# SeungheonOh/voxtral.c

Measured on AMD Instinct MI355X. Metric: decoder tokens/sec + encoder RTF, Voxtral-4B bf16 at 1/2/4/8 MI355X, higher is better.
Workload: dtype f32

## Files before the change

include/voxtral_hip.h:

```cpp
#ifndef VOXTRAL_HIP_H
#define VOXTRAL_HIP_H

#include <stddef.h>
#include <stdint.h>

#ifdef __cplusplus
extern "C" {
#endif

int vox_hip_init(void);
int vox_hip_available(void);
void vox_hip_shutdown(void);
size_t vox_hip_memory_used(void);
const char *vox_hip_last_error(void);
void vox_hip_clear_error(void);
int vox_hip_set_device(int device);

typedef struct {
    int enc_dim, enc_layers, enc_heads, enc_kv_heads, enc_head_dim, enc_hidden, enc_window;
    int dec_dim, dec_layers, dec_heads, dec_kv_heads, dec_head_dim, dec_hidden, dec_window;
    int vocab, mel_bins, downsample, ada_dim;
    float rope_theta, enc_eps, dec_eps;
    int gelu_erf;
} vox_hip_config_t;

void vox_hip_config_voxtral_4b(vox_hip_config_t *cfg);

typedef struct {
    const float *conv0_w, *conv0_b, *conv1_w, *conv1_b;
    const uint16_t **enc_wq, **enc_wk, **enc_wv, **enc_wo, **enc_w1, **enc_w2, **enc_w3;
    const float **enc_wq_b, **enc_wv_b, **enc_wo_b, **enc_w2_b, **enc_attn_norm, **enc_ffn_norm;
    const float *enc_norm;
    const uint16_t *ad0, *ad1;
    const uint16_t *tok_emb;
    const uint16_t **dec_wq, **dec_wk, **dec_wv, **dec_wo, **dec_w1, **dec_w2, **dec_w3;
    const float **dec_attn_norm, **dec_ffn_norm, **dec_ada_down, **dec_ada_up;
    const float *dec_norm;
    const float **enc_wq_s, **enc_wk_s, **enc_wv_s, **enc_wo_s, **enc_w1_s, **enc_w2_s, **enc_w3_s;
    const float *ad0_s, *ad1_s, *tok_emb_s;
    const float **dec_wq_s, **dec_wk_s, **dec_wv_s, **dec_wo_s, **dec_w1_s, **dec_w2_s, **dec_w3_s;
} vox_hip_weights_t;

typedef struct vox_hip_model vox_hip_model_t;
typedef struct vox_hip_stream vox_hip_stream_t;

vox_hip_model_t *vox_hip_model_create(const vox_hip_config_t *cfg, const vox_hip_weights_t *w,
                                      int delay_tokens);
void vox_hip_model_free(vox_hip_model_t *m);
int vox_hip_model_set_delay(vox_hip_model_t *m, int delay_tokens);
int vox_hip_model_ada_scale(vox_hip_model_t *m, float *out);
int vox_hip_model_set_kv_fp16(vox_hip_model_t *m, int on);
int vox_hip_model_set_kv_dtype(vox_hip_model_t *m, int dtype);
int vox_hip_model_set_enc_kv_fp16(vox_hip_model_t *m, int on);
int vox_hip_model_set_kv_grow(vox_hip_model_t *m, int slots0);
typedef struct {
    int packed_tensors;
    int raw_tensors;
    long long packed_bytes;
    long long packed_raw_bytes;
    long long raw_bytes;
    double pack_ms;
} vox_hip_wpack_stats_t;
int vox_hip_model_wpack_stats(const vox_hip_model_t *m, vox_hip_wpack_stats_t *out);
int vox_hip_gemv_wpack(int rows, int K, const uint16_t *W, const float *x, float *y, int packed);
int vox_hip_set_wmx4(int mode);
int vox_hip_wmx4(void);
typedef struct {
    int wmx4_tensors;
    int refused_tensors;
    long long plane_bytes;
    long long bf16_bytes;
    double bits_per_weight;
    double scan_ms;
    double round_ms;
    double pack_ms;
} vox_hip_wmx4_stats_t;
int vox_hip_model_wmx4_stats(const vox_hip_model_t *m, vox_hip_wmx4_stats_t *out);
int vox_hip_set_wmx4_batch(int on);
int vox_hip_wmx4_batch(void);
int vox_hip_model_wmx4_batch_stats(const vox_hip_model_t *m, long long out4[4]);
int vox_hip_skinny_wmx4(int N, int K, const uint16_t *W, const float *x, int nb, float *y, int fmt, int head);
int vox_hip_set_gemm_planes(int planes);
int vox_hip_gemm_planes(void);
int vox_hip_set_gemmf_wait(int ticks);
int vox_hip_set_gemmf_q8(int on);
int vox_hip_gemmf_q8(void);
int vox_hip_model_gemmf_q8_stats(const vox_hip_model_t *m, long long out4[4]);
int vox_hip_gemmf_q8_rows(int M, int N, int K, const float *x, const int8_t *Wq, const float *scales, float *y,
                          int fmt);

vox_hip_stream_t *vox_hip_stream_create(vox_hip_model_t *m);
void vox_hip_stream_free(vox_hip_stream_t *s);
int vox_hip_stream_kv_fp16(const vox_hip_stream_t *s);
int vox_hip_stream_kv_dtype(const vox_hip_stream_t *s);
int vox_hip_stream_enc_kv_fp16(const vox_hip_stream_t *s);
int vox_hip_stream_enc_paths(const vox_hip_stream_t *s, long long out5[5]);
long long vox_hip_stream_enc_kv_bytes(const vox_hip_stream_t *s);
int vox_hip_stream_kv_slots(const vox_hip_stream_t *s);
long long vox_hip_stream_kv_bytes(const vox_hip_stream_t *s);
int vox_hip_stream_kv_grow_stats(const vox_hip_stream_t *s, long long out3[3]);
int vox_hip_stream_reserve_kv(vox_hip_stream_t *s, int positions);
int vox_hip_stream_read_kv(vox_hip_stream_t *s, int layer, int first_logical_pos, int n, void *k_out, void *v_out);
int vox_hip_stream_read_enc_kv(vox_hip_stream_t *s, int layer, int first_logical_pos, int n, void *k_out, void *v_out);
int vox_hip_kv8_convert(const float *x, int n, uint8_t *codes, float *back);
int vox_hip_stream_reset(vox_hip_stream_t *s);
int vox_hip_stream_reset_decoder(vox_hip_stream_t *s);
#define VOX_HIP_MAX_DELAY_TOKENS 30
int vox_hip_stream_set_delay(vox_hip_stream_t *s, int delay_tokens);
int vox_hip_stream_delay(const vox_hip_stream_t *s);
int vox_hip_stream_ada_scale(vox_hip_stream_t *s, float *out);

int vox_hip_stream_encode_mel(vox_hip_stream_t *s, const float *mel, int n_frames,
                              int mel_on_device);
int vox_hip_stream_adapter_tokens(vox_hip_stream_t *s);
int vox_hip_set_adapter_rows0(int rows);
int vox_hip_stream_adapter_stats(const vox_hip_stream_t *s, long long out3[3]);
int vox_hip_stream_set_async_encode(vox_hip_stream_t *s, int on);
int vox_hip_stream_encode_mel_batch(vox_hip_stream_t *const *streams, const float *const *mels,
                                    const int *n_frames, int B, int mel_on_device, int *added);

typedef struct vox_hip_mel vox_hip_mel_t;
vox_hip_mel_t *vox_hip_mel_create(vox_hip_stream_t *s, int left_pad_samples);
int vox_hip_mel_feed(vox_hip_mel_t *m, const float *samples, int n_samples);
int vox_hip_mel_finish(vox_hip_mel_t *m, int right_pad_samples);
int vox_hip_mel_frames(const vox_hip_mel_t *m, int *frame_offset);
const float *vox_hip_mel_frame_ptr(const vox_hip_mel_t *m, int global_frame);
int vox_hip_mel_discard_before(vox_hip_mel_t *m, int keep_from_frame);
int vox_hip_mel_read(vox_hip_mel_t *m, int global_first, int n, float *out);
void vox_hip_mel_free(vox_hip_mel_t *m);
int vox_hip_mel_reset(vox_hip_mel_t *m, int left_pad_samples);
int vox_hip_stream_read_adapter(vox_hip_stream_t *s, int first, int n, float *out);

int vox_hip_stream_decode(vox_hip_stream_t *s, int max_steps, int stop_at_eos,
                          int *tokens_out, float *logits_out);
#define VOX_HIP_MAX_ALT 4
int vox_hip_stream_set_alt(vox_hip_stream_t *s, int n_alt, float cutoff);
int vox_hip_stream_read_alts(vox_hip_stream_t *s, int first, int n, int *ids_out, float *probs_out);
#define VOX_HIP_BATCH_MAX_SLOTS 128
typedef struct vox_hip_batch vox_hip_batch_t;
vox_hip_batch_t *vox_hip_batch_create(vox_hip_model_t *m, int max_streams);
void vox_hip_batch_free(vox_hip_batch_t *b);
int vox_hip_batch_decode(vox_hip_batch_t *b, vox_hip_stream_t **streams, int n, int max_steps,
                         int stop_at_eos, int *tokens_out, int *counts_out);
int vox_hip_batch_decode_rows(vox_hip_batch_t *b, vox_hip_stream_t **streams, int n, const int *rows,
                              int max_steps, int stop_at_eos, int *tokens_out, int *counts_out);
int vox_hip_batch_begin_rows(vox_hip_batch_t *b, vox_hip_stream_t **streams, int n, const int *rows,
                             int max_steps, int stop_at_eos, int *tokens_out, int *counts_out);
int vox_hip_batch_finish(vox_hip_batch_t *b);
int vox_hip_batch_read_logits(vox_hip_batch_t *b, vox_hip_stream_t *s, float *out);
int vox_hip_batch_stats(const vox_hip_batch_t *b, long long *out6);
int vox_hip_batch_kv_grow_stats(const vox_hip_batch_t *b, long long out3[3]);
int vox_hip_batch_set_prefill_kv(vox_hip_batch_t *b, int on);
int vox_hip_batch_set_gemv_rows(vox_hip_batch_t *b, int max_rows);
int vox_hip_batch_set_gemv_rows_q8(vox_hip_batch_t *b, int max_rows);
int vox_hip_batch_gemv_stats(const vox_hip_batch_t *b, long long *out4);
int vox_hip_batch_set_gemv_wmx4(vox_hip_batch_t *b, int on);
int vox_hip_batch_gemv_wmx4_stats(const vox_hip_batch_t *b, long long out4[4]);
int vox_hip_batch_set_wmx4(vox_hip_batch_t *b, int on);
int vox_hip_gemv_rows(int rows, int K, const uint16_t *W, const float *x, int R, float *y, int packed);
int vox_hip_gemv_rows_q8(int rows, int K, const int8_t *W, const float *scales, const float *x, int R, float *y);
int vox_hip_gemv_q8(int rows, int K, const int8_t *W, const float *scales, const float *x, float *y);
int vox_hip_stream_state(vox_hip_stream_t *s, int *out6);

void vox_hip_sgemm_bf16(int M, int N, int K, const float *A, const uint16_t *B_bf16, float *C);
void vox_hip_sgemm_q8(int M, int N, int K, const float *A, const int8_t *B_q8, const float *scales,
                      float *C);
void vox_hip_fused_qkv_bf16(int M, int K, const float *input,
                            const uint16_t *wq_bf16, int Nq, const uint16_t *wk_bf16, int Nk,
                            const uint16_t *wv_bf16, int Nv, float *q, float *k, float *v);
void vox_hip_fused_ffn_bf16(int M, int dim, int hidden, const float *input,
                            const uint16_t *w1_bf16, const uint16_t *w3_bf16,
                            const uint16_t *w2_bf16, float *output);
// ... 24 lines not shown
```

voxtral.c_amd/csrc/vox_hip.hip:

```cpp
#include "../../include/voxtral_hip.h"
#include "vox_hip_internal.h"
#include "vox_wmx4.h"
#include "vox_wpack.h"

#include <hip/hip_runtime.h>
#include <math.h>
#include <stdarg.h>
#include <stdio.h>
#include <stdlib.h>
#include <string.h>

#include <stddef.h>
#include <algorithm>
#include <atomic>
#include <chrono>
#include <mutex>
#include <string>
#include <thread>
#include <unordered_map>
#include <vector>

using namespace vox;

#define TOKEN_BOS 1
// ... 1561 lines not shown
            if (l == 0) s->enc_paths[4] += ns > 1;
            SklFused o = f;
            o.x = x;
            o.bias = L.bo;
            o.ssq_out = s->essq;
            o.planes = xa;
            o.nw = L.ffn_norm;
            CK(launch_gemm_sklx(SKX_PRO_PLANES, SKX_EPI_RESID, xq, EQ, F.wo, ED, n, o, st));
            SklFused u = f;
            u.ssq_in = s->essq;
            u.nsl = nsl_wo;
            u.planes = xq;
            CK(launch_gemm_sklx(SKX_PRO_SCALE, SKX_EPI_SWIGLU, xa, ED, F.w13, 2 * EH, n, u, st));
            SklFused d = f;
            d.x = x;
            d.bias = L.b2;
            d.ssq_out = s->essq;
            if (l + 1 < c.enc_layers) {
                d.planes = xa;
                d.nw = m->enc[l + 1].attn_norm;
            }
            CK(launch_gemm_sklx(SKX_PRO_PLANES, SKX_EPI_RESID, xq, EH, F.w2, ED, n, d, st));
        }
        CK(launch_rmsnorm_rows(x, ED, x, ED, m->enc_norm, nullptr, n, ED, c.enc_eps, st));
        return 0;
    }
    s->enc_paths[2]++;
    for (int l = 0; l < c.enc_layers; l++) {
        const EncLayerD& L = m->enc[l];
        const DecFragD& F = m->efrag[l];
        float* Kc = enc_ring(s, s->ek, l);
        float* Vc = enc_ring(s, s->ev, l);
        CK(launch_rmsnorm_fplanes(x, n, ED, L.attn_norm, nullptr, c.enc_eps, xp, l ? sl : nullptr,
                                  l ? skl_splits(EH, ED) : 0, st, l ? m->enc[l - 1].b2 : nullptr));
        CK(launch_gemm_skl(xp, ED, F.wqkv, L.sqkv, NQKV, n, sl, st));
        CK(launch_slabs_rope_kv(sl, skl_splits(ED, NQKV), n, L.bqkv, EQ, EKV, hd, rope, (int)pos0, s->q, Kc, Vc, s->ecap, st,
                                s->ekvt));
        CK(launch_attn_rows_mf(hd, s->q, EQ, Kc, Vc, s->ecap, s->att, EQ, n, H, KVH, (int)pos0, 0, c.enc_window, scale, st,
                             s->gws, s->gws_n, xp, s->ekvt));
        CK(launch_gemm_skl(xp, EQ, F.wo, L.so, ED, n, sl, st));
        CK(launch_rmsnorm_fplanes(x, n, ED, L.ffn_norm, nullptr, c.enc_eps, xp, sl, skl_splits(EQ, ED), st, L.bo));
        CK(launch_gemm_skl(xp, ED, F.w13, L.s13, 2 * EH, n, sl, st));
        CK(launch_swiglu_fplanes(sl, skl_splits(ED, 2 * EH), EH, n, xp, st));
        CK(launch_gemm_skl(xp, EH, F.w2, L.s2, ED, n, sl, st));
    }
    CK(launch_resid_slabs(x, n, ED, sl, skl_splits(EH, ED), m->enc[c.enc_layers - 1].b2, st));
    CK(launch_rmsnorm_rows(x, ED, x, ED, m->enc_norm, nullptr, n, ED, c.enc_eps, st));
    return 0;
}

static int enc_gemmf_env() {
    static const int v = env_on("VOX_HIP_GEMMF");
    return v;
}

template <class Layer>
static bool gemmf_fmt_ok(const vox_hip_model_t* m, const std::vector<Layer>& layers) {
    if (m->gemmf_q8) return true;
    for (const Layer& L : layers)
        if (L.sqkv || L.so || L.s13 || L.s2) return false;
    return true;
}

static bool enc_gemmf_ok(const vox_hip_model_t* m, int n) {
    const vox_hip_config_t& c = m->c;
    const int ED = c.enc_dim, EQ = c.enc_heads * c.enc_head_dim, EKV = c.enc_kv_heads * c.enc_head_dim;
    return enc_gemmf_env() && gemmf_fmt_ok(m, m->enc) && gemmf_ok(n, EQ + 2 * EKV, ED) && gemmf_ok(n, ED, EQ) &&
           gemmf_ok(n, 2 * c.enc_hidden, ED) && gemmf_ok(n, ED, c.enc_hidden) && c.enc_hidden % 64 == 0 &&
           ED <= 4 * 512;
}

struct GemmfQ {
    hipStream_t st;
    float* ws;
    size_t ws_n;
    int* flags;
    int* epoch;
    long long* n_q8;
    const int* epoch_dev;
    int* step_q8;
};

static int gemmf_on(const GemmfQ& q, int epi, const uint16_t* xs, int K, int n, const uint8_t* W, const float* wscale,
                    int N, const float* bias, float* C, int ldc, uint16_t* xo) {
    if (!q.epoch_dev) {
        hipStreamCaptureStatus cs = hipStreamCaptureStatusNone;
        CK(hipStreamIsCapturing(q.st, &cs));
        if (cs != hipStreamCaptureStatusNone) return set_err("k_gemmf launch while the stream is capturing");
    }
    if (++*q.epoch <= 0) *q.epoch = 1;
    if (!gemmf_ok(n, N, K) || !q.ws || !q.flags)
        return set_err("k_gemmf: unsupported shape M %d N %d K %d (ws %p flags %p)", n, N, K, (void*)q.ws, (void*)q.flags);
    if (!q.epoch_dev) {
        const hipError_t pend = hipGetLastError();
        if (pend != hipSuccess) return set_err("k_gemmf: HIP error pending before the launch: %s", hipGetErrorString(pend));
    }
    CK(launch_gemmf(epi, gemm_planes_np(), xs, K, n, W, N, bias, C, ldc, xo, q.ws, q.ws_n, q.flags, *q.epoch, q.st,
                    q.epoch_dev, q.epoch_dev ? gemmf_wide_rb(n, N, K) : 0, wscale));
    if (wscale) {
        ++*q.n_q8;
        if (q.step_q8) ++*q.step_q8;
    }
    return 0;
}

static GemmfQ stream_gemmfq(vox_hip_stream_t* s) {
    return GemmfQ{s->st, s->gws, s->gws_n, s->gflags, &s->gepoch, &s->m->n_gemmf_q8, nullptr, nullptr};
}

struct RowsLayer {
    const uint8_t *wqkv, *wo, *w13, *w2;
    const uint8_t *fqkv, *fo, *f13, *f2;
    const float *sqkv, *so, *s13, *s2;
    const float *bqkv, *bo, *b2;
    const float *attn_norm, *ffn_norm, *ada;
};
struct RowsStack {
    int D, Q, KV, hidden, layers;
    float eps;
    RowsLayer (*layer)(const vox_hip_model_t* m, int l);
};
struct RowsScratch {
    float *x, *qkv, *xn, *att, *hid;
    uint16_t *pa, *pc;
};
struct RowsAda {
    const float* table = nullptr;
    const BatchSlot* slots = nullptr;
};

static RowsLayer enc_rows_layer(const vox_hip_model_t* m, int l) {
    const EncLayerD& L = m->enc[l];
    const DecFragD F = m->efrag.empty() ? DecFragD{} : m->efrag[l];
    return RowsLayer{L.wqkv, L.wo, L.w13, L.w2, F.wqkv, F.wo, F.w13, F.w2, L.sqkv, L.so, L.s13, L.s2,
                     L.bqkv, L.bo, L.b2, L.attn_norm, L.ffn_norm, nullptr};
}
static RowsLayer dec_rows_layer(const vox_hip_model_t* m, int l) {
    const DecLayerD& L = m->dec[l];
    const DecFragD F = m->dfrag.empty() ? DecFragD{} : m->dfrag[l];
    return RowsLayer{L.wqkv, L.wo, L.w13, L.w2, F.wqkv, F.wo, F.w13, F.w2, L.sqkv, L.so, L.s13, L.s2,
                     nullptr, nullptr, nullptr, L.attn_norm, L.ffn_norm, m->ada_scale + (size_t)l * m->c.dec_dim};
}
static RowsStack enc_rows_stack(const vox_hip_config_t& c) {
    return RowsStack{c.enc_dim, c.enc_heads * c.enc_head_dim, c.enc_kv_heads * c.enc_head_dim, c.enc_hidden, c.enc_layers,
                     c.enc_eps, enc_rows_layer};
}
static RowsStack dec_rows_stack(const vox_hip_config_t& c) {
    return RowsStack{c.dec_dim, c.dec_heads * c.dec_head_dim, c.dec_kv_heads * c.dec_head_dim, c.dec_hidden, c.dec_layers,
                     c.dec_eps, dec_rows_layer};
}

template <class Attn>
static int rows_layers(const vox_hip_model_t* m, const RowsStack& S, const RowsScratch& B, const GemmfQ& q, bool gf, int n,
                       Attn attn, const RowsAda& ada = RowsAda{}) {
    const int D = S.D, NQKV = S.Q + 2 * S.KV, HID = S.hidden;
    hipStream_t st = q.st;
    for (int l = 0; l < S.layers; l++) {
        RowsLayer L = S.layer(m, l);
        if (ada.table) L.ada = ada.table + (size_t)l * D;
        if (gf) {
            CK(launch_rmsnorm_fplanes(B.x, n, D, L.attn_norm, nullptr, S.eps, B.pa, nullptr, 0, st));
            if (gemmf_on(q, EPI_STORE, B.pa, D, n, L.fqkv, L.sqkv, NQKV, L.bqkv, B.qkv, NQKV, nullptr)) return -1;
        } else {
            CK(launch_rmsnorm_rows(B.x, D, B.xn, D, L.attn_norm, nullptr, n, D, S.eps, st));
            CK(launch_gemm(EPI_STORE, 3, B.xn, D, L.wqkv, L.sqkv, D, n, NQKV, L.bqkv, B.qkv, NQKV, st, q.ws, q.ws_n));
        }
        if (attn(l, gf ? B.pa : nullptr)) return -1;
        if (gf) {
            if (gemmf_on(q, EPI_RESID, B.pa, S.Q, n, L.fo, L.so, D, L.bo, B.x, D, nullptr)) return -1;
            if (ada.slots) CK(launch_rmsnorm_fplanes_slots(B.x, n, D, L.ffn_norm, ada.slots, (size_t)l * D, S.eps, B.pa, st));
            else CK(launch_rmsnorm_fplanes(B.x, n, D, L.ffn_norm, L.ada, S.eps, B.pa, nullptr, 0, st));
            if (gemmf_on(q, EPI_SWIGLU, B.pa, D, n, L.f13, L.s13, 2 * HID, nullptr, nullptr, HID, B.pc)) return -1;
            if (gemmf_on(q, EPI_RESID, B.pc, HID, n, L.f2, L.s2, D, L.b2, B.x, D, nullptr)) return -1;
        } else {
            CK(launch_gemm(EPI_RESID, 3, B.att, S.Q, L.wo, L.so, S.Q, n, D, L.bo, B.x, D, st, q.ws, q.ws_n));
            if (ada.slots) CK(launch_rmsnorm_rows_slots(B.x, D, B.xn, D, L.ffn_norm, ada.slots, (size_t)l * D, n, D, S.eps, st));
            else CK(launch_rmsnorm_rows(B.x, D, B.xn, D, L.ffn_norm, L.ada, n, D, S.eps, st));
            CK(launch_gemm(EPI_SWIGLU, 3, B.xn, D, L.w13, L.s13, D, n, 2 * HID, nullptr, B.hid, HID, st, q.ws, q.ws_n));
            CK(launch_gemm(EPI_RESID, 3, B.hid, HID, L.w2, L.s2, HID, n, D, L.b2, B.x, D, st, q.ws, q.ws_n));
        }
    }
    return 0;
}

static int stream_enc_planes(vox_hip_stream_t* s) {
    const vox_hip_config_t& c = s->m->c;
    if (model_enc_frag(s->m)) return -1;
    if (!s->gpa) {
        const size_t rb = PLANE_MAX_ROWS / SK_ROWS;
        CK(dalloc(&s->gpa, rb * 3 * SK_ROWS * std::max(c.enc_dim, c.enc_heads * c.enc_head_dim)));
        CK(dalloc(&s->gpc, rb * 3 * SK_ROWS * c.enc_hidden));
    }
    if (!s->gflags) CK(dalloc(&s->gflags, gemmf_flag_ints()));
    return 0;
}
static RowsScratch enc_rows_scratch(vox_hip_stream_t* s, float* x) {
    return RowsScratch{x, s->qkv, s->xn, s->att, s->gate, s->gpa, s->gpc};
}

static bool enc_gemv_ok(const vox_hip_model_t* m) {
    const vox_hip_config_t& c = m->c;
    const int ED = c.enc_dim, EQ = c.enc_heads * c.enc_head_dim, EKV = c.enc_kv_heads * c.enc_head_dim;
    const bool q8 = m->enc[0].sqkv != nullptr;
    return gemv_ok(EQ + 2 * EKV, ED, q8) && gemv_ok(ED, EQ, q8) && gemv_ok(2 * c.enc_hidden, ED, q8) &&
           gemv_ok(ED, c.enc_hidden, q8) && c.enc_head_dim % 2 == 0 && c.enc_hidden % 16 == 0;
}

static int run_encoder_row_gemv(vox_hip_stream_t* s, float* x, long long pos0, const float* rope) {
    vox_hip_model_t* m = s->m;
    const vox_hip_config_t& c = m->c;
    const int ED = c.enc_dim, H = c.enc_heads, KVH = c.enc_kv_heads, hd = c.enc_head_dim;
    const int EQ = H * hd, EKV = KVH * hd, EH = c.enc_hidden;
    const float scale = 1.0f / sqrtf((float)hd);
    hipStream_t st = s->st;
    for (int l = 0; l < c.enc_layers; l++) {
        const EncLayerD& L = m->enc[l];
        float* Kc = enc_ring(s, s->ek, l);
        float* Vc = enc_ring(s, s->ev, l);
        GemvArgs a;
        memset(&a, 0, sizeof a);
        a.x = x; a.K = ED; a.W = L.wqkv; a.wscale = L.sqkv; a.rows = EQ + 2 * EKV; a.bias = L.bqkv;
        a.norm_w = L.attn_norm; a.eps = c.enc_eps; a.y = s->q;
        a.qd = EQ; a.kvd = EKV; a.hd = hd; a.pos = (int)pos0; a.rope = rope - (size_t)pos0 * hd;
        a.Kc = Kc; a.Vc = Vc; a.cap = s->ecap; a.kvt = s->ekvt;
        CK(launch_gemv(PRO_NORM, EPI_QKV_BIAS, a, st));
        CK(launch_attn_rows_mf(hd, s->q, EQ, Kc, Vc, s->ecap, s->att, EQ, 1, H, KVH, (int)pos0, 0, c.enc_window, scale,
                               st, s->gws, s->gws_n, nullptr, s->ekvt));
        memset(&a, 0, sizeof a);
        a.x = s->att; a.K = EQ; a.W = L.wo; a.wscale = L.so; a.rows = ED; a.bias = L.bo; a.y = x;
        CK(launch_gemv(PRO_NONE, EPI_RESID, a, st));
        memset(&a, 0, sizeof a);
        a.x = x; a.K = ED; a.W = L.w13; a.wscale = L.s13; a.rows = 2 * EH; a.norm_w = L.ffn_norm; a.eps = c.enc_eps;
        a.y = s->gate;
        CK(launch_gemv(PRO_NORM, EPI_SWIGLU, a, st));
        memset(&a, 0, sizeof a);
        a.x = s->gate; a.K = EH; a.W = L.w2; a.wscale = L.s2; a.rows = ED; a.bias = L.b2; a.y = x;
        CK(launch_gemv(PRO_NONE, EPI_RESID, a, st));
    }
    CK(launch_rmsnorm_rows(x, ED, x, ED, m->enc_norm, nullptr, 1, ED, c.enc_eps, st));
    return 0;
}

static int enc_skinny_env() {
    static const int v = env_on("VOX_HIP_ENC_SKINNY");
    return v;
}

static int run_encoder_rows(vox_hip_stream_t* s, float* x, int n, long long pos0, const float* rope) {
    vox_hip_model_t* m = s->m;
    const vox_hip_config_t& c = m->c;
    const int ED = c.enc_dim, H = c.enc_heads, KVH = c.enc_kv_heads, hd = c.enc_head_dim;
    const int EQ = H * hd, EKV = KVH * hd;
    const float scale = 1.0f / sqrtf((float)hd);
    hipStream_t st = s->st;
    if (n > ENC_SUB) return set_err("encoder pass of %d rows > %d", n, ENC_SUB);
    if (n == 1 && enc_gemv_ok(m)) {
        s->enc_paths[0]++;
        return run_encoder_row_gemv(s, x, pos0, rope);
    }
    if (n <= enc_skinny_rows() && enc_skinny_env() && enc_skinny_ok(c)) return run_encoder_rows_skinny(s, x, n, pos0, rope);
    s->enc_paths[3]++;
    const bool gf = enc_gemmf_ok(m, n);
    if (gf && stream_enc_planes(s)) return -1;
    if (rows_layers(m, enc_rows_stack(c), enc_rows_scratch(s, x), stream_gemmfq(s), gf, n, [&](int l, uint16_t* planes) -> int {
            float* Kc = enc_ring(s, s->ek, l);
            float* Vc = enc_ring(s, s->ev, l);
            CK(launch_rope_kv(s->qkv, n, EQ, EKV, hd, rope, (int)pos0, s->q, Kc, Vc, s->ecap, st, s->ekvt));
            CK(launch_attn_rows_mf(hd, s->q, EQ, Kc, Vc, s->ecap, s->att, EQ, n, H, KVH, (int)pos0, 0, c.enc_window, scale,
                                   st, s->gws, s->gws_n, planes, s->ekvt));
            return 0;
        }))
        return -1;
    CK(launch_rmsnorm_rows(x, ED, x, ED, m->enc_norm, nullptr, n, ED, c.enc_eps, st));
    return 0;
}

static int ensure_rope(vox_hip_stream_t* s, long long last_pos) {
    vox_hip_model_t* m = s->m;
    if (last_pos < m->rope_positions) return 0;
    int p = m->rope_positions;
    while (p <= last_pos) p *= 2;
    CK(hipDeviceSynchronize());
    if (model_rope_tables(m, p)) return -1;
    s->graph_ready = 0;
    return 0;
}

static int enc_prefix(vox_hip_stream_t* s, const float* mel, int n, int mel_on_device, int* T1o, float** xino) {
    vox_hip_model_t* m = s->m;
    const vox_hip_config_t& c = m->c;
    const int MB = c.mel_bins, ED = c.enc_dim;
    hipStream_t st = s->st;
    *T1o = 0;
    *xino = nullptr;
    if (n <= 0) return 0;
    if (stream_alloc_frames(s, n + 4)) return -1;
    CK(hipMemcpyAsync(s->mel_p, s->mel_tail, (size_t)2 * MB * 4, hipMemcpyDeviceToDevice, st));
    CK(hipMemcpyAsync(s->mel_p + (size_t)2 * MB, mel, (size_t)n * MB * 4,
                      mel_on_device ? hipMemcpyDeviceToDevice : hipMemcpyHostToDevice, st));
    CK(launch_mel_tail(s->mel_p, n, MB, s->mel_tail, st));
    CK(hipMemcpyAsync(s->c0_p, s->c0_tail, (size_t)2 * ED * 4, hipMemcpyDeviceToDevice, st));
    if (s->res_count)
        CK(hipMemcpyAsync(s->c0_p + (size_t)2 * ED, s->c0_res, (size_t)ED * 4, hipMemcpyDeviceToDevice, st));
    float* c0_new = s->c0_p + (size_t)(2 + s->res_count) * ED;
    CK(launch_im2col3(s->mel_p, MB, n, 1, 0, s->im2col, st));
    CK(launch_gemm(c.gelu_erf ? EPI_GELU_ERF : EPI_GELU, 3, s->im2col, MB * 3, m->conv0_w, nullptr, MB * 3, n, ED,
                   m->conv0_b, c0_new, ED, st, s->gws, s->gws_n));
    const int total = s->res_count + n;
    const int new_res = total & 1;
    const int feed = total - new_res;
    if (new_res)
        CK(hipMemcpyAsync(s->c0_res, s->c0_p + (size_t)(2 + total - 1) * ED, (size_t)ED * 4,
                          hipMemcpyDeviceToDevice, st));
    s->res_count = new_res;
    if (feed <= 0) return 0;
    const int T1 = feed / 2;
    float* xin = s->x_enc + (size_t)4 * ED;
    CK(launch_im2col3(s->c0_p, ED, T1, 2, 1, s->im2col, st));
    CK(launch_gemm(c.gelu_erf ? EPI_GELU_ERF : EPI_GELU, 3, s->im2col, ED * 3, m->conv1_w, nullptr, ED * 3, T1, ED,
                   m->conv1_b, xin, ED, st, s->gws, s->gws_n));
    CK(hipMemcpyAsync(s->c0_tail, s->c0_p + (size_t)(2 + feed - 2) * ED, (size_t)2 * ED * 4,
                      hipMemcpyDeviceToDevice, st));
    if (ensure_rope(s, s->enc_pos + T1 + 1)) return -1;
    *T1o = T1;
    *xino = xin;
    return 0;
}

static const int CS_ROWS = 2 * ENC_SUB + 5 * VOX_MAX_BATCH;
static bool enc_prefix_batch_fits(vox_hip_stream_t* const* ss, const int* n, int B) {
    long long r0 = 0, r1 = 0;
    for (int b = 0; b < B; b++)
        if (n[b] > 0) {
            r0 += 2 + ss[b]->res_count + n[b];
            r1 += (ss[b]->res_count + n[b]) / 2;
        }
    return r0 <= CS_ROWS && r1 <= ENC_SUB;
}

static int enc_prefix_batch(vox_hip_stream_t* lead, vox_hip_stream_t* const* ss, const float* const* mels,
                            const int* n, int B, int mel_on_device, float* X, int* T1, int* off) {
    vox_hip_model_t* m = lead->m;
    const vox_hip_config_t& c = m->c;
    const int MB = c.mel_bins, ED = c.enc_dim;
    hipStream_t st = lead->st;
    if (!lead->cs_im) {
        CK(dalloc(&lead->cs_im, std::max((size_t)CS_ROWS * MB * 3, (size_t)ENC_SUB * ED * 3)));
        CK(dalloc(&lead->cs_c0, (size_t)CS_ROWS * ED));
    }
    std::vector<int> seg(B, 0), res(B, 0), tot(B, 0);
    int R0 = 0, N = 0;
    for (int b = 0; b < B; b++) {
        T1[b] = 0;
        off[b] = N;
// ... 81 lines not shown
    s->enc_res_count = left;
    return added;
}

static int enc_suffix_batch(vox_hip_stream_t* lead, const float* X, vox_hip_stream_t* const* ss, const int* T1,
                            const int* off, int B, int* added) {
    vox_hip_model_t* m = lead->m;
    const vox_hip_config_t& c = m->c;
    const int ED = c.enc_dim, D = c.dec_dim;
    hipStream_t st = lead->st;
    const size_t ain_rows = (size_t)ENC_SUB + 4 * VOX_MAX_BATCH;
    if (!lead->abatch) {
        CK(dalloc(&lead->abatch, ain_rows * ED));
        CK(dalloc(&lead->abatch_out, ain_rows / 4 * D));
    }
    std::vector<int> aoff(B, 0), n4v(B, 0);
    int NA = 0;
    for (int b = 0; b < B; b++)
        if (T1[b] > 0) {
            const int tot = ss[b]->enc_res_count + T1[b];
            if (ss[b]->total_adapter + tot / 4 > ss[b]->adapter_cap) return set_err("enc_suffix_batch: adapter buffer");
            NA += tot / 4;
        }
    if ((size_t)NA * 4 > ain_rows) return set_err("enc_suffix_batch: %d adapter rows", NA);
    NA = 0;
    for (int b = 0; b < B; b++) {
        added[b] = 0;
        if (T1[b] <= 0) continue;
        vox_hip_stream_t* s = ss[b];
        s->enc_pos += T1[b];
        const int R = s->enc_res_count, tot = R + T1[b], usable = (tot / 4) * 4, left = tot - usable;
        const float* xb = X + (size_t)off[b] * ED;
        if (usable > 0) {
            float* dst = lead->abatch + (size_t)NA * 4 * ED;
            if (R) CK(hipMemcpyAsync(dst, s->enc_res, (size_t)R * ED * 4, hipMemcpyDeviceToDevice, st));
            CK(hipMemcpyAsync(dst + (size_t)R * ED, xb, (size_t)(usable - R) * ED * 4, hipMemcpyDeviceToDevice, st));
            if (left)
                CK(hipMemcpyAsync(s->enc_res, xb + (size_t)(usable - R) * ED, (size_t)left * ED * 4,
                                  hipMemcpyDeviceToDevice, st));
            aoff[b] = NA;
            n4v[b] = usable / 4;
            NA += usable / 4;
        } else {
            CK(hipMemcpyAsync(s->enc_res + (size_t)R * ED, xb, (size_t)T1[b] * ED * 4, hipMemcpyDeviceToDevice, st));
        }
        s->enc_res_count = left;
    }
    for (int r0 = 0; r0 < NA; r0 += ENC_SUB / 4) {
        const int nr = std::min(ENC_SUB / 4, NA - r0);
        CK(launch_gemm(c.gelu_erf ? EPI_GELU_ERF : EPI_GELU, 3, lead->abatch + (size_t)r0 * 4 * ED, 4 * ED, m->ad0,
                       m->ad0_s, 4 * ED, nr, D, nullptr, lead->ad_mid, D, st, lead->gws, lead->gws_n));
        CK(launch_gemm(EPI_STORE, 3, lead->ad_mid, D, m->ad1, m->ad1_s, D, nr, D, nullptr,
                       lead->abatch_out + (size_t)r0 * D, D, st, lead->gws, lead->gws_n));
    }
    for (int b = 0; b < B; b++) {
        if (!n4v[b]) continue;
        vox_hip_stream_t* s = ss[b];
        CK(hipMemcpyAsync(s->adapter + (size_t)s->total_adapter * D, lead->abatch_out + (size_t)aoff[b] * D,
                          (size_t)n4v[b] * D * 4, hipMemcpyDeviceToDevice, st));
        s->total_adapter += n4v[b];
        added[b] = n4v[b];
    }
    return 0;
}

static int run_encoder_rows_batch(vox_hip_stream_t* lead, float* X, int N, vox_hip_stream_t* const* ss,
                                  const int* off, const int* nr, const long long* pos0, int B) {
    vox_hip_model_t* m = lead->m;
    const vox_hip_config_t& c = m->c;
    const int ED = c.enc_dim, H = c.enc_heads, KVH = c.enc_kv_heads, hd = c.enc_head_dim;
    const int EQ = H * hd, EKV = KVH * hd;
    const float scale = 1.0f / sqrtf((float)hd);
    hipStream_t st = lead->st;
    const bool gf = enc_gemmf_ok(m, N);
    if (gf && stream_enc_planes(lead)) return -1;
    EncRows er;
    memset(&er, 0, sizeof er);
    er.B = B;
    for (int b = 0; b < B; b++) {
        er.off[b] = off[b];
        er.nr[b] = nr[b];
        er.pos0[b] = (int)pos0[b];
    }
    if (rows_layers(m, enc_rows_stack(c), enc_rows_scratch(lead, X), stream_gemmfq(lead), gf, N, [&](int l, uint16_t* planes) -> int {
            for (int b = 0; b < B; b++) {
                er.Kc[b] = enc_ring(ss[b], ss[b]->ek, l);
                er.Vc[b] = enc_ring(ss[b], ss[b]->ev, l);
            }
            CK(launch_rope_kv_rows(lead->qkv, N, EQ, EKV, hd, m->rope_enc, er, lead->q, lead->ecap, st, lead->ekvt));
            CK(launch_attn_rows(hd, lead->q, er, N, lead->ecap, lead->att, H, KVH, c.enc_window, scale, lead->gws,
                                lead->gws_n, st, planes, lead->ekvt));
            return 0;
        }))
        return -1;
    CK(launch_rmsnorm_rows(X, ED, X, ED, m->enc_norm, nullptr, N, ED, c.enc_eps, st));
    return 0;
}

static int encode_mel_batch_pass(vox_hip_stream_t* const* ss, const float* const* mels, const int* n, int B,
                                 int mel_on_device, int* added, bool sync = true) {
    vox_hip_stream_t* lead = ss[0];
    const vox_hip_config_t& c = lead->m->c;
    const int ED = c.enc_dim;
    std::vector<int> T1(B), off(B);
    std::vector<float*> xin(B);
    std::vector<long long> pos0(B);
    int N = 0;
    bool all_async = true;
    int active = 0;
    for (int b = 0; b < B; b++) {
        all_async = all_async && ss[b]->enc_async;
        if (n[b] > 0) {
            const int tot = ss[b]->res_count + n[b];
            active += tot - (tot & 1) > 0;
        }
    }
    static const int stem_batch = env_on("VOX_HIP_ENC_STEM_BATCH");
    const bool stacked = stem_batch && active > 1 && enc_prefix_batch_fits(ss, n, B);
    if (stacked) {
        if (!lead->xbatch) CK(dalloc(&lead->xbatch, (size_t)ENC_SUB * ED));
        N = enc_prefix_batch(lead, ss, mels, n, B, mel_on_device, lead->xbatch, T1.data(), off.data());
        if (N < 0) return -1;
        for (int b = 0; b < B; b++) pos0[b] = ss[b]->enc_pos;
    } else {
        for (int b = 0; b < B; b++) {
            if (enc_prefix(ss[b], mels[b], n[b], mel_on_device, &T1[b], &xin[b])) return -1;
            off[b] = N;
            pos0[b] = ss[b]->enc_pos;
            N += T1[b];
        }
    }
    if (!stacked && (N > ENC_SUB || active <= 1)) {
        for (int b = 0; b < B; b++) {
            added[b] = 0;
            if (T1[b] <= 0) continue;
            for (int r0 = 0; r0 < T1[b]; r0 += ENC_SUB) {
                const int nrr = std::min(ENC_SUB, T1[b] - r0);
                const long long p0 = ss[b]->enc_pos + r0;
                if (run_encoder_rows(ss[b], xin[b] + (size_t)r0 * ED, nrr, p0, lead->m->rope_enc + (size_t)p0 * c.enc_head_dim))
                    return -1;
            }
            added[b] = enc_suffix(ss[b], xin[b], T1[b]);
            if (added[b] < 0) return -1;
        }
    } else {
        if (!stacked) {
            if (!lead->xbatch) CK(dalloc(&lead->xbatch, (size_t)ENC_SUB * ED));
            for (int b = 1; b < B; b++) {
                CK(hipEventRecord(ss[b]->sev, ss[b]->st));
                CK(hipStreamWaitEvent(lead->st, ss[b]->sev, 0));
            }
            for (int b = 0; b < B; b++)
                if (T1[b] > 0)
                    CK(hipMemcpyAsync(lead->xbatch + (size_t)off[b] * ED, xin[b], (size_t)T1[b] * ED * 4,
                                      hipMemcpyDeviceToDevice, lead->st));
        }
        for (int b = 0; b < B; b++)
            if (T1[b] > 0 && stream_alloc_adapter(ss[b], ss[b]->total_adapter + (ss[b]->enc_res_count + T1[b]) / 4))
                return -1;
        if (run_encoder_rows_batch(lead, lead->xbatch, N, ss, off.data(), T1.data(), pos0.data(), B)) return -1;
        if (enc_suffix_batch(lead, lead->xbatch, ss, T1.data(), off.data(), B, added)) return -1;
        CK(hipEventRecord(lead->sev, lead->st));
        for (int b = 1; b < B; b++) CK(hipStreamWaitEvent(ss[b]->st, lead->sev, 0));
    }
    if (sync && !all_async)
        for (int b = 0; b < B; b++) CK(hipStreamSynchronize(ss[b]->st));
    return 0;
// ... 44 lines not shown
        for (int r0 = 0; r0 < T1; r0 += ENC_SUB) {
            int nr = std::min(ENC_SUB, T1 - r0);
            long long p0 = s->enc_pos + r0;
            if (run_encoder_rows(s, xin + (size_t)r0 * c.enc_dim, nr, p0,
                                 s->m->rope_enc + (size_t)p0 * c.enc_head_dim))
                return -1;
        }
        added = enc_suffix(s, xin, T1);
        if (added < 0) return -1;
    }
    if (!s->enc_async) CK(hipStreamSynchronize(s->st));
    return added;
}

extern "C" int vox_hip_stream_set_async_encode(vox_hip_stream_t* s, int on) {
    if (!s) return set_err("null stream");
    if (s->enc_async && !on) CK(hipStreamSynchronize(s->st));
    s->enc_async = on ? 1 : 0;
    return 0;
}

extern "C" int vox_hip_stream_adapter_tokens(vox_hip_stream_t* s) { return s->total_adapter; }

extern "C" int vox_hip_stream_adapter_stats(const vox_hip_stream_t* s, long long out3[3]) {
    if (!s || !out3) return set_err("stream_adapter_stats: null argument");
    out3[0] = s->adapter_cap;
    out3[1] = s->ad_grows;
    out3[2] = s->ad_grows_held;
    return 0;
}

extern "C" int vox_hip_stream_read_adapter(vox_hip_stream_t* s, int first, int n, float* out) {
    const int D = s->m->c.dec_dim;
    if (first < 0 || first + n > s->total_adapter) return set_err("adapter rows out of range");
    CK(hipMemcpyAsync(out, s->adapter + (size_t)first * D, (size_t)n * D * 4, hipMemcpyDeviceToHost, s->st));
    CK(hipStreamSynchronize(s->st));
    return 0;
}

static int stream_prefilled(vox_hip_stream_t* s, hipStream_t q) {
    const int np = 32 + stream_delay(s);
    const int st4[4] = {np, np, TOKEN_STREAMING_PAD, s->n_generated};
    CK(hipMemcpyAsync(s->state, st4, sizeof st4, hipMemcpyHostToDevice, q));
    s->h_state[0] = np;
    s->h_state[1] = np;
    s->h_state[2] = TOKEN_STREAMING_PAD;
    s->h_state[3] = s->n_generated;
    s->started = 1;
    return 0;
}

static int dec_gemmf_env() {
    static const int v = env_on("VOX_HIP_PREFILL_GEMMF");
    return v;
}

static bool dec_gemmf_ok(const vox_hip_model_t* m, int n) {
    const vox_hip_config_t& c = m->c;
    const int DD = c.dec_dim, DQ = c.dec_heads * c.dec_head_dim, DKV = c.dec_kv_heads * c.dec_head_dim;
    return enc_gemmf_env() && dec_gemmf_env() && gemmf_fmt_ok(m, m->dec) && n >= 1 && n <= PLANE_MAX_ROWS && gemmf_ok(n, DQ + 2 * DKV, DD) &&
           gemmf_ok(n, DD, DQ) && gemmf_ok(n, 2 * c.dec_hidden, DD) && gemmf_ok(n, DD, c.dec_hidden) &&
           c.dec_hidden % 64 == 0;
}

static int stream_dec_planes(vox_hip_stream_t* s, int rows) {
    if (rows <= s->dp_rows) return 0;
    const vox_hip_config_t& c = s->m->c;
    const int DD = c.dec_dim, DQ = c.dec_heads * c.dec_head_dim;
    const int r = (rows + 127) / 128 * 128;
    dfree(s->dpa);
    dfree(s->dpc);
    s->dp_rows = 0;
    CK(dalloc(&s->dpa, (size_t)r * 3 * std::max(DD, DQ)));
    CK(dalloc(&s->dpc, (size_t)r * 3 * c.dec_hidden));
    if (!s->gflags) CK(dalloc(&s->gflags, gemmf_flag_ints()));
    s->dp_rows = r;
    return 0;
}

static RowsScratch dec_rows_scratch(vox_hip_stream_t* s, float* x) {
    return RowsScratch{x, s->qkvd, s->xnd, s->attd, s->gated, s->dpa, s->dpc};
}

static int run_decoder_rows(vox_hip_stream_t* s, float* x, int n, int pos0, const float* rope) {
    vox_hip_model_t* m = s->m;
    const vox_hip_config_t& c = m->c;
    const int H = c.dec_heads, KVH = c.dec_kv_heads, hd = c.dec_head_dim;
    const int DQ = H * hd, DKV = KVH * hd;
    const float scale = 1.0f / sqrtf((float)hd);
    hipStream_t st = s->st;
    if (stream_alloc_dec_rows(s, n)) return -1;
    if (n > DEC_SLACK + 1 && pos0 > 0) return set_err("prefill of %d rows on a non-empty cache", n);
    bool gf = n > 1 && dec_gemmf_ok(m, n);
    if (gf && (model_frag(m) || stream_dec_planes(s, n))) {
        vox_hip_clear_error();
        (void)hipGetLastError();
        gf = false;
    }
    return rows_layers(m, dec_rows_stack(c), dec_rows_scratch(s, x), stream_gemmfq(s), gf, n, [&](int l, uint16_t* planes) -> int {
        float* Kc = dec_ring(s, s->dk, l);
        float* Vc = dec_ring(s, s->dv, l);
        CK(launch_rope_kv(s->qkvd, n, DQ, DKV, hd, rope, pos0, s->qd_, Kc, Vc, s->dcap, st, s->kvt));
        CK(launch_attn_rows_mf(hd, s->qd_, DQ, Kc, Vc, s->dcap, s->attd, DQ, n, H, KVH, pos0, 0, c.dec_window, scale, st,
                               s->gws, s->gws_n, planes, s->kvt));
        return 0;
    }, RowsAda{s->delay < 0 ? nullptr : stream_ada(s), nullptr});
}

enum { T_QKV, T_WO, T_W13, T_W2 };
struct StepTensor {
    const uint8_t* W;
    const float* wscale;
    int rows, K, pro, epi;
    const float *norm_w, *ada;
    const WPackD* pack;
    const WMx4D* mx;
};
static StepTensor dec_step_tensor(const vox_hip_model_t* m, int l, int which) {
    const vox_hip_config_t& c = m->c;
    const int DD = c.dec_dim, DQ = c.dec_heads * c.dec_head_dim, DKV = c.dec_kv_heads * c.dec_head_dim, DH = c.dec_hidden;
    if (l == (int)m->dec.size())
        return StepTensor{m->tok_emb, m->tok_emb_s, c.vocab, DD, PRO_NORM, EPI_STORE, m->dec_norm, nullptr, &m->plm, &m->mlm};
    const DecLayerD& L = m->dec[l];
    switch (which) {
    case T_QKV: return StepTensor{L.wqkv, L.sqkv, DQ + 2 * DKV, DD, PRO_NORM, EPI_QKV, L.attn_norm, nullptr, &L.pqkv, &L.mqkv};
    case T_WO: return StepTensor{L.wo, L.so, DD, DQ, PRO_NONE, EPI_RESID, nullptr, nullptr, &L.po, &L.mo};
    case T_W13:
        return StepTensor{L.w13, L.s13, 2 * DH, DD, PRO_NORM_ADA, EPI_SWIGLU, L.ffn_norm, m->ada_scale + (size_t)l * DD,
                          &L.p13, &L.m13};
    default: return StepTensor{L.w2, L.s2, DD, DH, PRO_NONE, EPI_RESID, nullptr, nullptr, &L.p2, &L.m2};
    }
}
template <class F>
static bool all_step_tensors(const vox_hip_model_t* m, F f) {
    const int nl = (int)m->dec.size();
    for (int l = 0; l <= nl; l++)
        for (int w = 0; w < (l < nl ? 4 : 1); w++)
            if (!f(dec_step_tensor(m, l, w))) return false;
    return true;
}
static void step_tensor_args(GemvArgs& a, const StepTensor& t, const float* x, float* y, float eps, int wmx4) {
    memset(&a, 0, sizeof a);
    a.x = x; a.K = t.K; a.W = t.W; a.wscale = t.wscale; a.rows = t.rows; a.y = y;
    a.norm_w = t.norm_w; a.ada = t.ada; a.eps = t.norm_w ? eps : 0.f;
    wpack_args(a, *t.pack);
    if (wmx4) wmx4_args(a, *t.mx);
}

static int enqueue_lm_head(vox_hip_stream_t* s, const int* state);

static int enqueue_step_layers(vox_hip_stream_t* s, const int* state, int pos, const float* rope_row,
                               int splits) {
    vox_hip_model_t* m = s->m;
    const vox_hip_config_t& c = m->c;
    const int H = c.dec_heads, KVH = c.dec_kv_heads, hd = c.dec_head_dim;
    const float scale = 1.0f / sqrtf((float)hd);
    hipStream_t st = s->st;
    for (int l = 0; l < c.dec_layers; l++) {
        float* Kc = dec_ring(s, s->dk, l);
        float* Vc = dec_ring(s, s->dv, l);
        GemvArgs a;
        StepTensor t = dec_step_tensor(m, l, T_QKV);
        step_tensor_args(a, t, s->xd, s->qd_, c.dec_eps, 1);
        a.qd = H * hd; a.kvd = KVH * hd; a.hd = hd;
        a.state = state; a.pos = pos;
        a.rope = state ? m->rope_dec : rope_row - (size_t)pos * hd;
        a.Kc = Kc; a.Vc = Vc; a.cap = s->dcap; a.kvt = s->kvt;
        CK(launch_gemv(t.pro, t.epi, a, st));
        CK(launch_attn_decode(hd, s->qd_, Kc, Vc, s->dcap, state, pos, c.dec_window, scale, H, KVH,
                              s->part, s->attd, splits, st, s->kvt));
        t = dec_step_tensor(m, l, T_WO);
        step_tensor_args(a, t, s->attd, s->xd, c.dec_eps, 1);
        CK(launch_gemv(t.pro, t.epi, a, st));
        t = dec_step_tensor(m, l, T_W13);
        if (s->delay >= 0) t.ada = stream_ada(s) + (size_t)l * c.dec_dim;
        step_tensor_args(a, t, s->xd, s->gated, c.dec_eps, 1);
        const bool gprof = s->profiling && state && !s->capturing && (int)s->pev.size() == 2 * c.dec_layers;
        if (gprof) CK(launch_gemv_timed(t.pro, t.epi, a, s->pev[2 * l], s->pev[2 * l + 1], st));
        else CK(launch_gemv(t.pro, t.epi, a, st));
        t = dec_step_tensor(m, l, T_W2);
        step_tensor_args(a, t, s->gated, s->xd, c.dec_eps, 1);
        CK(launch_gemv(t.pro, t.epi, a, st));
    }
    return enqueue_lm_head(s, state);
}

static int enqueue_lm_head(vox_hip_stream_t* s, const int* state) {
    vox_hip_model_t* m = s->m;
    const StepTensor t = dec_step_tensor(m, m->c.dec_layers, 0);
// ... 35 lines not shown
    s->capturing = 1;
    int rc = enqueue_graph_step(s, graph_splits(s, gi));
    s->capturing = 0;
    hipError_t e = hipStreamEndCapture(s->st, &g);
    if (rc || e != hipSuccess) {
        if (g) hipGraphDestroy(g);
        return set_err("graph capture failed: %s", hipGetErrorString(e));
    }
    e = hipGraphInstantiate(&s->step_exec[gi], g, nullptr, nullptr, 0);
    hipGraphDestroy(g);
    if (e != hipSuccess) return set_err("graph instantiate failed: %s", hipGetErrorString(e));
    s->graph_ready |= 1 << gi;
    s->graph_alt = s->n_alt > 1;
    s->graph_rope_gen = s->m->rope_gen;
    return 0;
}

static int collect_graph_profile(vox_hip_stream_t* s) {
    if (!s->profiling || !s->graph_prof) return 0;
    const vox_hip_config_t& c = s->m->c;
    for (int l = 0; l < c.dec_layers; l++) {
        float ms = 0.f;
        CK(hipEventElapsedTime(&ms, s->pev[2 * l], s->pev[2 * l + 1]));
        s->prof_ms += ms;
        s->prof_bytes += (double)2 * c.dec_hidden * c.dec_dim * 2;
        s->prof_launches++;
    }
    return 0;
}

static int use_graphs() {
    static const int v = env_on("VOX_HIP_GRAPH");
    return v;
}

static int run_steps(vox_hip_stream_t* s, int n, int pos0) {
    const vox_hip_config_t& c = s->m->c;
    const int gi = graph_index(s, std::min(pos0 + n, c.dec_window));
    const int splits = graph_splits(s, gi);
    if (s->profiling && use_graphs() && n > 1) {
        s->profiling = 0;
        const int rc = run_steps(s, n - 1, pos0);
        s->profiling = 1;
        if (rc) return -1;
        pos0 += n - 1;
        n = 1;
    }
    if (!use_graphs() || s->profiling) {
        if (s->profiling && s->pev.empty()) {
            s->pev.resize(2 * c.dec_layers);
            for (auto& e : s->pev) CK(hipEventCreate(&e));
        }
        s->graph_prof = s->profiling;
        for (int i = 0; i < n; i++)
            if (enqueue_graph_step(s, splits)) return -1;
        return 0;
    }
    if (s->graph_ready && (s->graph_alt != (s->n_alt > 1) || s->graph_rope_gen != s->m->rope_gen)) s->graph_ready = 0;
    if (!(s->graph_ready & (1 << gi)) && build_step_graph(s, gi)) return -1;
    for (int i = 0; i < n; i++) CK(hipGraphLaunch(s->step_exec[gi], s->st));
    return 0;
}

template <class T>
static int ring_read(const T* ring, int cap, int rec, long long first, int n, T* out, hipStream_t st) {
    while (n > 0) {
        const int slot = (int)(first % cap);
        const int k = std::min(n, cap - slot);
        CK(hipMemcpyAsync(out, ring + (size_t)slot * rec, (size_t)k * rec * sizeof(T), hipMemcpyDeviceToHost, st));
        out += (size_t)k * rec;
        first += k;
        n -= k;
    }
    return 0;
}

static int stream_prefill(vox_hip_stream_t* s) {
    vox_hip_model_t* m = s->m;
    const int np = 32 + stream_delay(s);
    if (stream_alloc_dec_rows(s, np)) return -1;
    if (ensure_rope(s, np + 2)) return -1;
    CK(launch_embed_rows(s->adapter, m->tok_emb, m->tok_emb_s, 0, np, TOKEN_BOS, TOKEN_STREAMING_PAD, m->c.dec_dim,
                         s->xd, s->st));
    if (run_decoder_rows(s, s->xd, np, 0, m->rope_dec)) return -1;
    return stream_prefilled(s, s->st);
}

extern "C" int vox_hip_stream_decode(vox_hip_stream_t* s, int max_steps, int stop_at_eos,
                                     int* tokens_out, float* logits_out) {
    vox_hip_model_t* m = s->m;
    const vox_hip_config_t& c = m->c;
    const int D = c.dec_dim, V = c.vocab, hd = c.dec_head_dim;
    const int prompt_len = 1 + 32 + stream_delay(s);
    int produced = 0;
    if (s->held) return set_err("stream_decode: %s", HELD_MSG);
    if (max_steps <= 0 || s->eos_seen) return 0;
    if (!s->started && s->total_adapter < prompt_len) return 0;
    if (s->dslots0) {
        const int pos = s->started ? s->h_state[0] : prompt_len - 1;
        const int left = s->total_adapter - (s->started ? s->h_state[1] : prompt_len - 1);
        if (stream_grow_dec(s, pos + std::max(0, std::min(max_steps, left)))) return -1;
    }
    if (!s->started && stream_prefill(s)) return -1;
    const int step_base = s->n_generated;
    int avail = s->total_adapter - (s->h_state[1] > 0 ? s->h_state[1] : prompt_len - 1);
    {
        int st4[4];
        CK(hipMemcpyAsync(st4, s->state, sizeof st4, hipMemcpyDeviceToHost, s->st));
        CK(hipStreamSynchronize(s->st));
        memcpy(s->h_state, st4, sizeof st4);
        avail = s->total_adapter - st4[1];
    }
    if (ensure_rope(s, (long long)s->h_state[0] + avail + 1)) return -1;
    if (avail > 0) CK(launch_embed_step(s->adapter, m->tok_emb, m->tok_emb_s, s->state, D, s->xd, s->st));
    int todo = std::min(max_steps, avail);
    std::vector<int> tok;
    while (produced < todo) {
        int b = std::min(STEP_BATCH, todo - produced);
        if (logits_out) b = 1;
        if (run_steps(s, b, s->h_state[0] + produced)) return -1;
        tok.resize(produced + b);
        if (ring_read(s->tokens, s->tokens_cap, 1, (long long)step_base + produced, b, tok.data() + produced, s->st))
            return -1;
        if (logits_out)
            CK(hipMemcpyAsync(logits_out + (size_t)produced * V, s->logits, (size_t)V * 4, hipMemcpyDeviceToHost, s->st));
        CK(hipStreamSynchronize(s->st));
        if (collect_graph_profile(s)) return -1;
        int eos_at = -1;
        if (stop_at_eos)
            for (int i = produced; i < produced + b; i++)
                if (tok[i] == TOKEN_EOS) { eos_at = i; break; }
        if (eos_at >= 0) {
            produced = eos_at + 1;
            s->eos_seen = 1;
            break;
        }
        produced += b;
    }
    if (tokens_out) memcpy(tokens_out, tok.data(), (size_t)produced * 4);
    s->n_generated += produced;
    s->h_state[0] += produced;
    s->h_state[1] += produced;
    if (produced) s->h_state[2] = tok[produced - 1];
    s->h_state[3] = s->n_generated;
    (void)hd;
    return produced;
}

extern "C" int vox_hip_stream_set_alt(vox_hip_stream_t* s, int n_alt, float cutoff) {
    if (!s) return -1;
    if (s->held) return set_err("stream_set_alt: %s", HELD_MSG);
    if (n_alt < 1) n_alt = 1;
    if (n_alt > VOX_HIP_MAX_ALT) n_alt = VOX_HIP_MAX_ALT;
    if (cutoff < 0) cutoff = 0;
    if (cutoff > 1) cutoff = 1;
    s->n_alt = n_alt;
    s->alt_cutoff = cutoff;
    return 0;
}

extern "C" int vox_hip_stream_read_alts(vox_hip_stream_t* s, int first, int n, int* ids_out,
                                        float* probs_out) {
    if (!s || first < 0 || n < 0 || first + n > s->n_generated || first < s->n_generated - s->tokens_cap)
        return set_err("alt range out of bounds (the last %d steps are kept)", s->tokens_cap);
    if (n == 0) return 0;
    std::vector<float> rec((size_t)n * ALT_REC);
    std::vector<int> tok(n);
// ... 408 lines not shown
            CK(dalloc(&dW, (size_t)N * K * 2));
            if (upload(dW, W, (size_t)N * K * 2) || frag_copy(&dF, dW, N, K, 0)) return -1;
        }
        CK(dalloc(&dx, (size_t)nb * K));
        CK(dalloc(&dxs, (size_t)Z * 3 * SK_ROWS * K));
        CK(dalloc(&dout, nout));
        if (upload(dx, x, (size_t)nb * K * 4)) return -1;
        CK(launch_split_fplanes(dx, nb, K, dxs, g_twin_st));
        if (!head)
            CK(launch_gemm_skl(dxs, K, dF, nullptr, N, nb, dout, g_twin_st, nullptr, 0, 0.f, 1, fmt));
        else if (nb > SK_ROWS)
            CK(launch_gemm_skf2(dxs, K, dF, nullptr, N, nb, dout, N, g_twin_st, fmt));
        else
            CK(launch_gemm_skf(dxs, K, dF, nullptr, N, nb, dout, N, g_twin_st, fmt));
        CK(hipStreamSynchronize(g_twin_st));
        CK(hipMemcpy(out.data(), dout, nout * 4, hipMemcpyDeviceToHost));
        return 0;
    };
    const int rc = run();
    dfree(dW); dfree(dF); dfree(dx); dfree(dxs); dfree(dout);
    if (rc) return -1;
    for (int j = 0; j < nb; j++) {
        float* yr = y + (size_t)j * N;
        if (head) {
            memcpy(yr, out.data() + (size_t)j * N, (size_t)N * 4);
            continue;
        }
        const float* p = out.data() + (size_t)(j >> 4) * S * SK_ROWS * N + (size_t)(j & 15) * N;
        for (int n = 0; n < N; n++) {
            float v = p[n];
            for (int sp = 1; sp < S; sp++) v += p[(size_t)sp * SK_ROWS * N + n];
            yr[n] = v;
        }
    }
    return 0;
}

extern "C" int vox_hip_gemmf_q8_rows(int M, int N, int K, const float* x, const int8_t* Wq, const float* scales, float* y,
                                     int fmt) {
    std::lock_guard<std::mutex> lk(g_twin_mu);
    if (!x || !Wq || !y || (fmt && !scales)) return set_err("gemmf_q8_rows: null argument");
    if (fmt != 0 && fmt != 1) return set_err("gemmf_q8_rows: fmt is 0 or 1");
    if (!gemmf_ok(M, N, K) || M > PLANE_MAX_ROWS)
        return set_err("gemmf_q8_rows: k_gemmf does not take M %d N %d K %d (M 1..1024, N %% 128, K %% 64)", M, N, K);
    if (twin_init()) return -1;
    uint8_t *dW = nullptr, *dF = nullptr;
    float *dx = nullptr, *dy = nullptr, *ds = nullptr, *dws = nullptr;
    uint16_t* dxs = nullptr;
    int* dflags = nullptr;
    auto run = [&]() -> int {
        const size_t n = (size_t)N * K;
        if (fmt) {
            CK(dalloc(&dW, n));
            CK(dalloc(&ds, (size_t)N));
            if (upload(dW, Wq, n) || upload(ds, scales, (size_t)N * 4) || frag_copy(&dF, dW, N, K, 1)) return -1;
        } else {
            std::vector<uint16_t> wb(n);
            for (size_t i = 0; i < n; i++) {
                const float f = (float)Wq[i];
                uint32_t u;
                memcpy(&u, &f, 4);
                wb[i] = (uint16_t)(u >> 16);
            }
            CK(dalloc(&dW, n * 2));
            if (upload(dW, wb.data(), n * 2) || frag_copy(&dF, dW, N, K, 0)) return -1;
        }
        const size_t rows = (size_t)(M + 127) / 128 * 128;
        const size_t ws_n = gemmf_ws_floats(gemmf_grid());
        CK(dalloc(&dx, (size_t)M * K));
        CK(dalloc(&dxs, rows * 3 * K));
        CK(dalloc(&dy, (size_t)M * N));
        CK(dalloc(&dws, ws_n));
        CK(dalloc(&dflags, gemmf_flag_ints()));
        if (upload(dx, x, (size_t)M * K * 4)) return -1;
        CK(launch_split_fplanes(dx, M, K, dxs, g_twin_st));
        CK(launch_gemmf(EPI_STORE, gemm_planes_np(), dxs, K, M, dF, N, nullptr, dy, N, nullptr, dws, ws_n, dflags, 1,
                        g_twin_st, nullptr, 0, fmt ? ds : nullptr));
        CK(hipStreamSynchronize(g_twin_st));
        CK(hipMemcpy(y, dy, (size_t)M * N * 4, hipMemcpyDeviceToHost));
        return 0;
    };
    const int rc = run();
    dfree(dW); dfree(dF); dfree(dx); dfree(dxs); dfree(dy); dfree(ds); dfree(dws); dfree(dflags);
    return rc ? -1 : 0;
}

extern "C" void vox_hip_sgemm_bf16(int M, int N, int K, const float* A, const uint16_t* B, float* C) {
    std::lock_guard<std::mutex> lk(g_twin_mu);
    twin_sgemm(M, N, K, A, B, nullptr, C);
}

extern "C" void vox_hip_sgemm_q8(int M, int N, int K, const float* A, const int8_t* B, const float* scales,
                                 float* C) {
    std::lock_guard<std::mutex> lk(g_twin_mu);
    if (!scales) { set_err("sgemm_q8: null scales"); return; }
    twin_sgemm(M, N, K, A, B, scales, C);
}

extern "C" void vox_hip_fused_qkv_bf16(int M, int K, const float* input, const uint16_t* wq, int Nq,
                                       const uint16_t* wk, int Nk, const uint16_t* wv, int Nv,
                                       float* q, float* k, float* v) {
    std::lock_guard<std::mutex> lk(g_twin_mu);
    if (M <= 0) return;
    if (twin_init()) return;
    const TwinW* W[3] = {twin_weight(wq, nullptr, Nq, K), twin_weight(wk, nullptr, Nk, K),
                         twin_weight(wv, nullptr, Nv, K)};
    if (!W[0] || !W[1] || !W[2]) return;
    float* outs[3] = {q, k, v};
    float* dO[3] = {nullptr, nullptr, nullptr};
    size_t* caps[3] = {&g_tQ_n, &g_tK_n, &g_tV_n};
    float** bufs[3] = {&g_tQ, &g_tK, &g_tV};
    if (twin_put_rows(&g_tA, &g_tA_n, input, M, K, W[0]->Kp)) return;
    for (int i = 0; i < 3; i++) {
        if (twin_buf(bufs[i], caps[i], (size_t)M * W[i]->Np) || twin_gemm_dev(M, g_tA, *W[i], *bufs[i])) return;
        dO[i] = *bufs[i];
    }
    for (int i = 0; i < 3; i++)
        if (twin_get_rows(outs[i], dO[i], M, W[i]->N, W[i]->Np)) return;
    if (hipStreamSynchronize(g_twin_st) != hipSuccess) set_err("fused_qkv: sync failed");
}

__global__ void k_silu_mul(float* g, const float* u, size_t n) {
    size_t i = (size_t)blockIdx.x * 256 + threadIdx.x;
    if (i < n) {
        float v = g[i];
        g[i] = v / (1.0f + expf(-v)) * u[i];
    }
}

extern "C" void vox_hip_fused_ffn_bf16(int M, int dim, int hidden, const float* input,
                                       const uint16_t* w1, const uint16_t* w3, const uint16_t* w2,
                                       float* output) {
    std::lock_guard<std::mutex> lk(g_twin_mu);
    if (M <= 0) return;
    if (twin_init()) return;
    const TwinW* d1 = twin_weight(w1, nullptr, hidden, dim);
    const TwinW* d3 = twin_weight(w3, nullptr, hidden, dim);
    const TwinW* d2 = twin_weight(w2, nullptr, dim, hidden);
    if (!d1 || !d3 || !d2) return;
    const int Hp = d1->Np;
    if (d2->Kp != Hp) { set_err("fused_ffn: padded hidden %d != %d", d2->Kp, Hp); return; }
    if (twin_put_rows(&g_tA, &g_tA_n, input, M, dim, d1->Kp) || twin_buf(&g_tQ, &g_tQ_n, (size_t)M * Hp) ||
        twin_buf(&g_tK, &g_tK_n, (size_t)M * Hp) || twin_buf(&g_tC, &g_tC_n, (size_t)M * d2->Np) ||
        twin_gemm_dev(M, g_tA, *d1, g_tQ) || twin_gemm_dev(M, g_tA, *d3, g_tK))
        return;
    const size_t n = (size_t)M * Hp;
    hipLaunchKernelGGL(k_silu_mul, dim3((unsigned)((n + 255) / 256)), dim3(256), 0, g_twin_st, g_tQ, g_tK, n);
    if (hipGetLastError() != hipSuccess) { set_err("fused_ffn: silu_mul launch failed"); return; }
    if (twin_gemm_dev(M, g_tQ, *d2, g_tC) || twin_get_rows(output, g_tC, M, dim, d2->Np)) return;
    if (hipStreamSynchronize(g_twin_st) != hipSuccess) set_err("fused_ffn: sync failed");
}

static int twin_attention(float* out, const float* Q, const float* K, const float* V, int seq_q, int seq_k,
                          int n_heads, int n_kv_heads, int head_dim, float scale, int window_size, int q_offset) {
    if (twin_init()) return -1;
    if (seq_q <= 0) return 0;
    if (!out || !Q || !K || !V) return set_err("encoder_attention: null pointer");
    if (q_offset < 0 || q_offset + seq_q > seq_k) return set_err("encoder_attention: queries beyond keys");
    if (n_kv_heads <= 0 || n_heads % n_kv_heads) return set_err("encoder_attention: heads %d / kv heads %d", n_heads, n_kv_heads);
    const size_t qn = (size_t)seq_q * n_heads * head_dim, kn = (size_t)seq_k * n_kv_heads * head_dim;
    if (twin_buf(&g_tQ, &g_tQ_n, qn) || twin_buf(&g_tK, &g_tK_n, kn) || twin_buf(&g_tV, &g_tV_n, kn) ||
        twin_buf(&g_tO, &g_tO_n, qn))
        return -1;
    CK(hipMemcpyAsync(g_tQ, Q, qn * 4, hipMemcpyHostToDevice, g_twin_st));
    CK(hipMemcpyAsync(g_tK, K, kn * 4, hipMemcpyHostToDevice, g_twin_st));
    CK(hipMemcpyAsync(g_tV, V, kn * 4, hipMemcpyHostToDevice, g_twin_st));
// ... 539 lines not shown
    if (!b) return set_err("batch_set_gemv_rows_q8: null batch");
    return batch_set_gemv_rows_q8(b, max_rows);
}

static int batch_set_gemv_wmx4(vox_hip_batch_t* b, int on, bool quiet) {
    if (b->call.active) return quiet ? -1 : set_err("batch_set_gemv_wmx4: a begun call was not finished");
    if (on) {
        const vox_hip_model_t* m = b->m;
        long long with = 0, without = 0;
        model_gemv_wmx4_count(m, &with, &without);
        if (!with)
            return quiet ? -1
                         : set_err("batch_set_gemv_wmx4: the model has no wmx4 GEMV plane (vox_hip_set_wmx4 before its creation; "
                                   "not Q8, not VOX_HIP_WPACK=0)");
        if (!model_gemvr_ok(m, 1))
            return quiet ? -1 : set_err("batch_set_gemv_wmx4: no wmx4 k_gemvr instance for this model's shapes");
    }
    b->gemv_wmx4 = on ? 1 : 0;
    return 0;
}

extern "C" int vox_hip_batch_set_gemv_wmx4(vox_hip_batch_t* b, int on) {
    if (!b) return set_err("batch_set_gemv_wmx4: null batch");
    return batch_set_gemv_wmx4(b, on, false);
}

extern "C" int vox_hip_batch_gemv_wmx4_stats(const vox_hip_batch_t* b, long long out4[4]) {
    if (!b || !out4) return set_err("batch_gemv_wmx4_stats: null argument");
    out4[0] = b->gemv_wmx4;
    out4[1] = b->n_gemv_wmx4_replays;
    model_gemv_wmx4_count(b->m, &out4[2], &out4[3]);
    return 0;
}

extern "C" int vox_hip_batch_set_wmx4(vox_hip_batch_t* b, int on) {
    if (!b) return set_err("batch_set_wmx4: null batch");
    if (b->call.active) return set_err("batch_set_wmx4: a begun call was not finished");
    if (on && !b->m->fstats[0])
        return set_err("batch_set_wmx4: the model has no wmx4 fragment planes (vox_hip_set_wmx4_batch before its creation)");
    b->wmx4 = on ? 1 : 0;
    return 0;
}

extern "C" int vox_hip_batch_set_prefill_kv(vox_hip_batch_t* b, int on) {
    if (!b) return set_err("batch_set_prefill_kv: null batch");
    if (b->call.active) return set_err("batch_set_prefill_kv: a begun call was not finished");
    b->prefill_kv = on ? 1 : 0;
    return 0;
}

extern "C" int vox_hip_batch_gemv_stats(const vox_hip_batch_t* b, long long* out4) {
    if (!b || !out4) return set_err("batch_gemv_stats: null argument");
    out4[0] = b->gemv_rows;
    out4[1] = b->n_gemv_replays;
    out4[2] = b->n_gemv_rows;
    out4[3] = b->n_gemv_captures;
    return 0;
}

static int batch_step_wide(vox_hip_batch_t* b, int nb, int splits, int kvt, int mixed, int ragged) {
    vox_hip_model_t* m = b->m;
    const vox_hip_config_t& c = m->c;
    const int DD = c.dec_dim, H = c.dec_heads, KVH = c.dec_kv_heads, hd = c.dec_head_dim;
    const int DQ = H * hd, DKV = KVH * hd, QKV = DQ + 2 * DKV;
    const float scale = 1.0f / sqrtf((float)hd);
    const int cap = c.dec_window + DEC_SLACK;
    const size_t ring_layer = (size_t)cap * DKV * kv_esize(kvt);
    hipStream_t st = b->st;
    const bool gf = dec_gemmf_ok(m, nb);
    const bool lm_gf = (!m->tok_emb_s || m->gemmf_q8) && enc_gemmf_env() && dec_gemmf_env() && gemmf_ok(nb, c.vocab, DD);
    int launches = 0;
    b->wide_q8 = 0;
    const GemmfQ q{st, b->pgws, GEMM_WS_ELEMS, b->wflags, &launches, &m->n_gemmf_q8, b->wepoch, &b->wide_q8};
    AttnSlotsRag ap;
    ap.q = nullptr; ap.q_ld = 0;
    ap.part = b->apart; ap.part_ld = b->apart_n;
    ap.out = gf ? nullptr : b->att; ap.out_ld = DQ;
    ap.slots = b->slots;
    ap.ring_off = 0;
    ap.caps = b->dcaps; ap.layer = 0;
    AttnFuse af;
    af.qkv = b->wqkv; af.S = 1; af.N = QKV; af.rope = m->rope_dec; af.xs = b->wpa;
    if (rows_layers(m, dec_rows_stack(c), RowsScratch{b->x, b->wqkv, b->wxn, b->att, b->whid, b->wpa, b->wpc}, q, gf, nb,
                    [&](int l, uint16_t*) -> int {
                        ap.ring_off = (size_t)l * ring_layer;
                        ap.layer = l;
                        if (ragged) CK(launch_attn_batch_wide_rag(hd, ap, af, nb, c.dec_window, scale, H, KVH, splits, st, kvt));
                        else CK(launch_attn_batch_wide(hd, ap, af, nb, cap, c.dec_window, scale, H, KVH, splits, st, kvt));
                        return 0;
                    }, RowsAda{nullptr, mixed ? b->slots : nullptr}))
        return -1;
    if (lm_gf) {
        CK(launch_rmsnorm_fplanes(b->x, nb, DD, m->dec_norm, nullptr, c.dec_eps, b->wpa, nullptr, 0, st));
        if (gemmf_on(q, EPI_STORE, b->wpa, DD, nb, m->lm_frag, m->tok_emb_s, c.vocab, nullptr, b->logits, c.vocab, nullptr)) return -1;
    } else {
        CK(launch_rmsnorm_rows(b->x, DD, b->wxn, DD, m->dec_norm, nullptr, nb, DD, c.dec_eps, st));
        CK(launch_gemm(EPI_STORE, 3, b->wxn, DD, m->tok_emb, m->tok_emb_s, DD, nb, c.vocab, nullptr, b->logits, c.vocab, st,
                       b->pgws, GEMM_WS_ELEMS));
    }
    CK(launch_argmax_batch(b->logits, nb, c.vocab, b->pval, b->pidx, b->palt, b->slots, TOKENS_CAP, slot_toklog(b->slots, b->rows),
                           m->tok_emb, m->tok_emb_s, DD, b->x, st));
    if (launches) CK(launch_gemmf_epoch_bump(b->wepoch, launches + 1, st));
    return 0;
}


static int slot_bucket(int n, int* g) {
    int k = 0;
    while ((1 << k) < n) k++;
    *g = k;
    return 1 << k;
}

static int batch_run(vox_hip_batch_t* b, int nb, int gb, int gi, int splits, int kvt, int steps, int gemv, int mixed,
                     int ragged) {
    const int wmx4 = b->wmx4;
    const int gwmx4 = b->gemv_wmx4;
    const bool wide = nb > VOX_MAX_BATCH;
    auto step = [&]() {
        return wide ? batch_step_wide(b, nb, splits, kvt, mixed, ragged)
               : gemv ? batch_step_gemv(b, nb, splits, kvt, gwmx4) : batch_step(b, nb, splits, kvt, wmx4, mixed, ragged);
    };
    if (ragged) b->n_ragged_replays += steps;
    if (gemv) b->n_gemv_replays += steps;
    if (gemv && gwmx4) b->n_gemv_wmx4_replays += steps;
    if (!use_graphs()) {
        for (int k = 0; k < steps; k++)
            if (step()) return -1;
        b->n_replays += steps;
        return 0;
    }
    if (b->grope_gen != b->m->rope_gen) {
        batch_drop_graphs(b);
        b->grope_gen = b->m->rope_gen;
    }
    const int mr = mixed + 2 * ragged;
    hipGraphExec_t& ge = wide ? b->gwexec[mr][kvt][gb - 6][gi]
                         : gemv ? b->gvexec[3 * gwmx4 + kvt][gb][gi] : b->gexec[mr][3 * wmx4 + kvt][gb][gi];
    if (!ge) {
        hipGraph_t g = nullptr;
        CK(hipStreamBeginCapture(b->st, hipStreamCaptureModeThreadLocal));
        const int rc = step();
        hipError_t e = hipStreamEndCapture(b->st, &g);
        if (rc || e != hipSuccess) {
            if (g) hipGraphDestroy(g);
            return set_err("batch graph capture failed: %s", hipGetErrorString(e));
        }
        e = hipGraphInstantiate(&ge, g, nullptr, nullptr, 0);
        hipGraphDestroy(g);
        if (e != hipSuccess) {
            ge = nullptr;
            return set_err("batch graph instantiate failed: %s", hipGetErrorString(e));
        }
        b->n_captures++;
        if (ragged) b->n_ragged_captures++;
        if (gemv) b->n_gemv_captures++;
    }
    for (int k = 0; k < steps; k++) CK(hipGraphLaunch(ge, b->st));
    if (wide) b->m->n_gemmf_q8 += (long long)steps * b->wide_q8;
    b->n_replays += steps;
    return 0;
}

static void stream_steps_done(vox_hip_stream_t* s, int produced, int last_token) {
    s->n_generated += produced;
    s->h_state[0] += produced;
    s->h_state[1] += produced;
    if (produced) s->h_state[2] = last_token;
    s->h_state[3] = s->n_generated;
}

static int batch_prefill(vox_hip_batch_t* b, vox_hip_stream_t* const* ss, int B, bool bounded) {
    vox_hip_model_t* m = b->m;
    const vox_hip_config_t& c = m->c;
    const int np = 32 + stream_delay(ss[0]);
    const int per = std::max(1, ENC_SUB / np);
    const int kvt = ss[0]->kvt;
    const bool one_by_one = kvt != KV_F32 && !b->prefill_kv;
    if (B > per && !one_by_one) {
        for (int i0 = 0; i0 < B; i0 += per)
            if (batch_prefill(b, ss + i0, std::min(per, B - i0), bounded)) return -1;
        return 0;
    }
    if ((B == 1 && !bounded) || one_by_one || B * np > ENC_SUB) {
        for (int i = 0; i < B; i++) {
            if (stream_prefill(ss[i])) return -1;
            CK(hipStreamSynchronize(ss[i]->st));
        }
        b->n_prefill_passes += B;
        b->n_prefilled += B;
        return 0;
    }
    const int DD = c.dec_dim, H = c.dec_heads, KVH = c.dec_kv_heads, hd = c.dec_head_dim;
    const int DQ = H * hd, DKV = KVH * hd;
    const float scale = 1.0f / sqrtf((float)hd);
    vox_hip_stream_t* lead = ss[0];
    const int N = B * np, cap = lead->dcap;
    hipStream_t st = b->st;
    if (stream_alloc_dec_rows(lead, N)) return -1;
    if (ensure_rope(lead, np + 2)) return -1;
    if (!b->pgws) CK(dalloc(&b->pgws, GEMM_WS_ELEMS));
    float* gws = b->pgws;
    const size_t gws_n = GEMM_WS_ELEMS;
    float* X = lead->xd;
    for (int i = 0; i < B; i++)
        CK(launch_embed_rows(ss[i]->adapter, m->tok_emb, m->tok_emb_s, 0, np, TOKEN_BOS, TOKEN_STREAMING_PAD, DD,
                             X + (size_t)i * np * DD, st));
    EncRows er;
    memset(&er, 0, sizeof er);
    er.B = B;
    for (int i = 0; i < B; i++) {
        er.off[i] = i * np;
        er.nr[i] = np;
        er.pos0[i] = 0;
    }
    const bool gf = dec_gemmf_ok(m, N);
    if (gf) {
        if (!b->gflags) CK(dalloc(&b->gflags, gemmf_flag_ints()));
        if (model_frag(m) || stream_dec_planes(lead, N)) return -1;
    }
    if (rows_layers(m, dec_rows_stack(c), dec_rows_scratch(lead, X),
                    GemmfQ{st, gws, gws_n, b->gflags, &b->gepoch, &m->n_gemmf_q8, nullptr, nullptr}, gf, N,
                    [&](int l, uint16_t* planes) -> int {
                        for (int i = 0; i < B; i++) {
                            er.Kc[i] = dec_ring(ss[i], ss[i]->dk, l);
                            er.Vc[i] = dec_ring(ss[i], ss[i]->dv, l);
                        }
                        CK(launch_rope_kv_rows(lead->qkvd, N, DQ, DKV, hd, m->rope_dec, er, lead->qd_, cap, st, kvt));
                        CK(launch_attn_rows(hd, lead->qd_, er, N, cap, lead->attd, H, KVH, c.dec_window, scale, gws, gws_n, st,
                                            planes, kvt));
                        return 0;
                    }, RowsAda{lead->delay < 0 ? nullptr : stream_ada(lead), nullptr}))
        return -1;
    for (int i = 0; i < B; i++)
        if (stream_prefilled(ss[i], st)) return -1;
    b->n_prefill_passes++;
    b->n_prefilled += B;
    return 0;
}

static int batch_begin(vox_hip_batch_t* b, vox_hip_stream_t** streams, int n, const int* rows, int max_steps,
                       int stop_at_eos, int* tokens_out, int* counts_out) {
    if (!b || n < 1 || n > b->cap || n > VOX_MAX_SLOTS || max_steps < 0) return set_err("bad batch arguments");
    if (b->call.active) return set_err("batch: a begun call was not finished");
    vox_hip_model_t* m = b->m;
    const vox_hip_config_t& c = m->c;
    int mixed = 0;
    for (int i = 0; i < n; i++) {
        if (!streams[i] || streams[i]->m != m) return set_err("batch streams must share the batch's model");
        if (streams[i]->held) return set_err("batch streams[%d]: %s", i, HELD_MSG);
        mixed |= streams[i]->delay >= 0;
        if (streams[i]->kvt != streams[0]->kvt)
            return set_err("batch streams must share the decoder KV element type (vox_hip_model_set_kv_dtype)");
        for (int j = 0; j < i; j++)
            if (streams[j] == streams[i]) return set_err("stream listed twice in a batch");
        counts_out[i] = 0;
    }
    const int kvt = streams[0]->kvt;
    b->n_calls++;
    b->lnb = 0;
    int avail[VOX_MAX_SLOTS];
    for (int i = 0; i < n; i++) {
        if (rows) {
            if (rows[i] < 0 || rows[i] > streams[i]->total_adapter) return set_err("batch rows[%d] out of range", i);
            avail[i] = rows[i];
        } else {
            CK(hipStreamSynchronize(streams[i]->st));
            avail[i] = streams[i]->total_adapter;
        }
    }
    if (max_steps == 0) return 1;
    int ragged = 0;
    {
        bool grows = false;
        for (int i = 0; i < n; i++) grows = grows || streams[i]->dslots0;
        if (grows) {
            std::vector<DecGrow> gr(n);
            for (int i = 0; i < n; i++) {
                vox_hip_stream_t* s = streams[i];
                const int np = 32 + stream_delay(s);
                const bool joins = !s->started && !s->eos_seen && avail[i] >= 1 + np;
                int need = 0;
                if (s->started && !s->eos_seen) need = s->h_state[0] + std::max(0, std::min(avail[i] - s->h_state[1], max_steps));
                else if (joins) need = np + std::max(0, std::min(avail[i] - np, max_steps));
                if (dec_grow_alloc(s, need, true, &gr[i])) {
                    dec_grow_drop(gr.data(), i);
                    return -1;
                }
            }
            for (int i = 0; i < n; i++) ragged |= (gr[i].cap ? gr[i].cap : streams[i]->dcap) != dec_ring_full(streams[i]);
            if (ragged && !b->hcaps) {
                hipError_t e = b->dcaps ? hipSuccess : dalloc(&b->dcaps, (size_t)b->rows);
                if (e == hipSuccess) e = hipHostMalloc((void**)&b->hcaps, sizeof(int) * b->rows, hipHostMallocDefault);
                if (e != hipSuccess) {
                    b->hcaps = nullptr;
                    dec_grow_drop(gr.data(), n);
                    return set_err("batch: per-slot ring capacity table: %s", hipGetErrorString(e));
                }
            }
            if (dec_grow_commit(gr.data(), n, b->st)) return -1;
        }
        b->n_ragged_calls += ragged;
    }
    {
        vox_hip_stream_t* pre[VOX_MAX_SLOTS];
        int np = 0, longest_delay = 0;
// ... 223 lines not shown
```

voxtral.c_amd/csrc/vox_hip_dev.h:

```cpp
#pragma once
#include <hip/hip_runtime.h>
#include <stdint.h>

#include "vox_hip_internal.h"

namespace vox {

typedef __attribute__((ext_vector_type(8))) __bf16 bf16x8;
typedef __attribute__((ext_vector_type(4))) float f32x4;
typedef __attribute__((ext_vector_type(2))) float f32x2;
typedef __attribute__((ext_vector_type(4))) unsigned int u32x4;
typedef __attribute__((ext_vector_type(2))) unsigned int u32x2;

__device__ __forceinline__ uint4 ldnt(const uint4* p) {
    u32x4 v = __builtin_nontemporal_load(reinterpret_cast<const u32x4*>(p));
    return make_uint4(v.x, v.y, v.z, v.w);
}

__device__ __forceinline__ float bf2f(uint32_t bits16) { return __uint_as_float(bits16 << 16); }
__device__ __forceinline__ float bflo(uint32_t w) { return __uint_as_float(w << 16); }
__device__ __forceinline__ float bfhi(uint32_t w) { return __uint_as_float(w & 0xffff0000u); }

__device__ __forceinline__ uint32_t f2bf(float f) {
    const __bf16 b = (__bf16)f;
// ... 117 lines not shown
__device__ __forceinline__ float hlo(uint32_t w) { return (float)__builtin_bit_cast(_Float16, (unsigned short)(w & 0xffffu)); }
__device__ __forceinline__ float hhi(uint32_t w) { return (float)__builtin_bit_cast(_Float16, (unsigned short)(w >> 16)); }
__device__ __forceinline__ float dot8h(uint4 w, uint32_t sd, int q, float4 a, float4 b, float acc) {
    const uint32_t HM = 0xfff8fff8u, SM = 0x00070007u;
    const uint32_t t = (w.x & SM) | ((w.y & SM) << 3) | ((w.z & SM) << 6);
    const uint32_t p3 = (t << 3) | ((sd << (4 * q)) & 0xf000f000u);
    const uint32_t p0 = w.x & HM, p1 = w.y & HM, p2 = w.z & HM;
    acc = fmaf(hlo(p0), a.x, acc);
    acc = fmaf(hhi(p0), a.y, acc);
    acc = fmaf(hlo(p1), a.z, acc);
    acc = fmaf(hhi(p1), a.w, acc);
    acc = fmaf(hlo(p2), b.x, acc);
    acc = fmaf(hhi(p2), b.y, acc);
    acc = fmaf(hlo(p3), b.z, acc);
    acc = fmaf(hhi(p3), b.w, acc);
    return acc;
}

typedef float f32x2 __attribute__((ext_vector_type(2)));
__device__ __forceinline__ float dot8m4(uint32_t w, uint32_t scale_byte, float4 a, float4 b, float acc) {
    const float sc = __uint_as_float(scale_byte << 23);
    const f32x2 p0 = __builtin_amdgcn_cvt_scalef32_pk_f32_fp4(w, sc, 0);
    const f32x2 p1 = __builtin_amdgcn_cvt_scalef32_pk_f32_fp4(w, sc, 1);
    const f32x2 p2 = __builtin_amdgcn_cvt_scalef32_pk_f32_fp4(w, sc, 2);
    const f32x2 p3 = __builtin_amdgcn_cvt_scalef32_pk_f32_fp4(w, sc, 3);
    acc = fmaf(p0.x, a.x, acc);
    acc = fmaf(p0.y, a.y, acc);
    acc = fmaf(p1.x, a.z, acc);
    acc = fmaf(p1.y, a.w, acc);
    acc = fmaf(p2.x, b.x, acc);
    acc = fmaf(p2.y, b.y, acc);
    acc = fmaf(p3.x, b.z, acc);
    acc = fmaf(p3.y, b.w, acc);
    return acc;
}

struct f32x8 {
    f32x2 p[4];
};
__device__ __forceinline__ f32x8 dec8m4(uint32_t w, uint32_t scale_byte) {
    const float sc = __uint_as_float(scale_byte << 23);
    f32x8 d;
    d.p[0] = __builtin_amdgcn_cvt_scalef32_pk_f32_fp4(w, sc, 0);
    d.p[1] = __builtin_amdgcn_cvt_scalef32_pk_f32_fp4(w, sc, 1);
    d.p[2] = __builtin_amdgcn_cvt_scalef32_pk_f32_fp4(w, sc, 2);
    d.p[3] = __builtin_amdgcn_cvt_scalef32_pk_f32_fp4(w, sc, 3);
    return d;
}
__device__ __forceinline__ float dot8f(const f32x8& d, float4 a, float4 b, float acc) {
    acc = fmaf(d.p[0].x, a.x, acc);
    acc = fmaf(d.p[0].y, a.y, acc);
    acc = fmaf(d.p[1].x, a.z, acc);
    acc = fmaf(d.p[1].y, a.w, acc);
    acc = fmaf(d.p[2].x, b.x, acc);
    acc = fmaf(d.p[2].y, b.y, acc);
    acc = fmaf(d.p[3].x, b.z, acc);
    acc = fmaf(d.p[3].y, b.w, acc);
    return acc;
}

__device__ __forceinline__ float i8f(uint32_t w, int b) { return (float)((int32_t)(w << (24 - 8 * b)) >> 24); }
__device__ __forceinline__ float dot16q(uint4 w, const float4 (&x)[4], float acc) {
    const uint32_t d[4] = {w.x, w.y, w.z, w.w};
#pragma unroll
    for (int k = 0; k < 4; k++) {
        acc = fmaf(i8f(d[k], 0), x[k].x, acc);
        acc = fmaf(i8f(d[k], 1), x[k].y, acc);
        acc = fmaf(i8f(d[k], 2), x[k].z, acc);
        acc = fmaf(i8f(d[k], 3), x[k].w, acc);
    }
    return acc;
}

__device__ __forceinline__ bf16x8 i8x8_bf16(uint32_t lo, uint32_t hi) {
    uint32_t h[8];
#pragma unroll
    for (int b = 0; b < 4; b++) {
        h[b] = __float_as_uint(i8f(lo, b)) >> 16;
        h[4 + b] = __float_as_uint(i8f(hi, b)) >> 16;
    }
    return __builtin_bit_cast(bf16x8, make_uint4(h[0] | (h[1] << 16), h[2] | (h[3] << 16), h[4] | (h[5] << 16), h[6] | (h[7] << 16)));
}

}
```

voxtral.c_amd/csrc/vox_hip_gemmf.hip:

```cpp
#include "vox_hip_internal.h"
#include "vox_hip_dev.h"

#include <hip/hip_runtime.h>
#include <stdint.h>

#include <algorithm>
#include <stdlib.h>

namespace vox {

#ifndef VOX_GF_DIAG
#define VOX_GF_DIAG 0
#endif

typedef __attribute__((address_space(3))) void lds_void_t;
typedef __attribute__((address_space(1))) void g_void_t;

template <int N>
__device__ __forceinline__ void wait_vm() {
    static_assert(N >= 0 && N < 64, "vmcnt range");
    __builtin_amdgcn_s_waitcnt((N & 15) | ((N >> 4) << 14) | (7 << 4) | (15 << 8));
}

struct GemmfArgs {
    const uint16_t* xs;
    int K, M;
    const uint8_t* W;
    int N;
    const float* wscale;
    const float* bias;
    float* C;
    int ldc;
    uint16_t* xo;
    float* ws;
    int* flags;
    int* recomputes;
    int wait_ticks;
    int epoch;
    const int* epoch_dev;
    int S, NT, T;
    long long U;
    int MT;
    int colmajor;
};


constexpr int GF_TIMEOUT_TICKS = 5000;
static int g_gemmf_wait = GF_TIMEOUT_TICKS;

template <int NP, int RB, int NG, int WR, int WF = WF_BF16>
struct GfCfg {
    static_assert(WF == WF_BF16 || WF == WF_Q8, "k_gemmf streams bf16 or int8 fragments");
    static constexpr int NWV = 4 * WR;
    static constexpr int RBW = RB / WR;
    static constexpr int CH = RB * NP * 2;
    static constexpr int CW = 4 * NG * (WF == WF_Q8 ? 1 : 2);
    static constexpr int NA = CH / NWV;
    static constexpr int NB = CW / NWV;
    static constexpr int SLOT = (CH + CW) * 512;
    static_assert(CH % NWV == 0 && CW % NWV == 0 && RB % WR == 0, "chunks must split over the waves");
};

template <int NP, int RB, int NG, int WR, int SL, int WF = WF_BF16>
__device__ __forceinline__ void gf_issue(const uint16_t* xb, size_t plane, const uint8_t* wt, int KB, int s,
                                         uint16_t* lds, int wave, int lane) {
    using C = GfCfg<NP, RB, NG, WR, WF>;
    if (VOX_GF_DIAG == 2) return;
    uint16_t* dst = lds + SL * C::SLOT;
#pragma unroll
    for (int i = 0; i < C::NA; i++) {
        const int c = wave + C::NWV * i;
        const int rb = c / (NP * 2), p = (c >> 1) % NP, t = c & 1;
        const uint16_t* src = xb + ((size_t)rb * 3 + p) * plane + (size_t)(s * 2 + t) * 512 + lane * 8;
        __builtin_amdgcn_global_load_lds((g_void_t*)src, (lds_void_t*)(dst + c * 512), 16, 0, 0);
    }
#pragma unroll
    for (int i = 0; i < C::NB; i++) {
        const int j = wave + C::NWV * i;
        const uint8_t* src = WF == WF_Q8 ? wt + ((size_t)j * KB + s) * 1024 + lane * 16
                                         : wt + ((size_t)(j >> 1) * KB + s) * 2048 + (j & 1) * 1024 + lane * 16;
        __builtin_amdgcn_global_load_lds((g_void_t*)src, (lds_void_t*)(dst + (C::CH + j) * 512), 16, 0, 0);
    }
}

template <int NP, int RB, int NG, int WR, int WF = WF_BF16>
struct GfHalf {
    bf16x8 w[NG];
    bf16x8 x[RB / WR][NP];
};

template <int NG, int WF>
struct GfRaw {
    u32x4 q[WF == WF_Q8 ? NG : 1];
};

template <int NP, int RB, int NG, int WR, int SL, int T, int WF = WF_BF16>
__device__ __forceinline__ void gf_read(const uint16_t* lds, int wave, int lane, GfHalf<NP, RB, NG, WR, WF>& f,
                                        GfRaw<NG, WF>& raw) {
    using C = GfCfg<NP, RB, NG, WR, WF>;
    const uint16_t* src = lds + SL * C::SLOT;
    const int wc = wave & 3, r0 = (wave >> 2) * C::RBW;
    if constexpr (WF == WF_Q8) {
        if (T == 0) {
#pragma unroll
            for (int g = 0; g < NG; g++)
                raw.q[g] = *reinterpret_cast<const u32x4*>(src + (C::CH + wc * NG + g) * 512 + lane * 8);
        }
    } else {
#pragma unroll
        for (int g = 0; g < NG; g++)
            f.w[g] = *reinterpret_cast<const bf16x8*>(src + (C::CH + (wc * NG + g) * 2 + T) * 512 + lane * 8);
    }
#pragma unroll
    for (int i = 0; i < C::RBW; i++)
#pragma unroll
        for (int p = 0; p < NP; p++)
            f.x[i][p] = *reinterpret_cast<const bf16x8*>(src + (((r0 + i) * NP + p) * 2 + T) * 512 + lane * 8);
}

template <int NP, int RB, int NG, int WR, int T, int WF>
__device__ __forceinline__ void gf_cvt(const GfRaw<NG, WF>& raw, GfHalf<NP, RB, NG, WR, WF>& f) {
    if constexpr (WF == WF_Q8) {
#pragma unroll
        for (int g = 0; g < NG; g++) f.w[g] = T ? i8x8_bf16(raw.q[g][2], raw.q[g][3]) : i8x8_bf16(raw.q[g][0], raw.q[g][1]);
    }
}
// ... 6 lines not shown
    }
#pragma unroll
    for (int i = 0; i < RB / WR; i++)
#pragma unroll
        for (int p = 0; p < NP; p++)
#pragma unroll
            for (int g = 0; g < NG; g++)
                acc[i][g] = __builtin_amdgcn_mfma_f32_16x16x32_bf16(f.w[g], f.x[i][p], acc[i][g], 0, 0, 0);
}

__device__ __forceinline__ void wait_lgkm0() { __builtin_amdgcn_s_waitcnt(15 | (3 << 14) | (7 << 4)); }

template <int NP, int RB, int NG, int WR, int WF = WF_BF16>
__device__ __forceinline__ void gf_stages(const GemmfArgs& a, uint16_t* lds, int mt, int nt, int s0, int s1,
                                          f32x4 (&acc)[RB / WR][NG]) {
    using C = GfCfg<NP, RB, NG, WR, WF>;
    const int lane = threadIdx.x & 63, wave = __builtin_amdgcn_readfirstlane(threadIdx.x >> 6);
    const int KB = a.K >> 6;
    const size_t plane = (size_t)SK_ROWS * a.K;
    const uint16_t* xb = a.xs + (size_t)(mt * RB) * 3 * plane;
    const uint8_t* wt = a.W + (size_t)nt * 4 * NG * KB * (WF == WF_Q8 ? 1024 : 2048);
    GfHalf<NP, RB, NG, WR, WF> H0, H1;
    GfRaw<NG, WF> raw;
    gf_issue<NP, RB, NG, WR, 0, WF>(xb, plane, wt, KB, s0, lds, wave, lane);
    if (s0 + 1 < s1) gf_issue<NP, RB, NG, WR, 1, WF>(xb, plane, wt, KB, s0 + 1, lds, wave, lane);
    if (s0 + 2 < s1) gf_issue<NP, RB, NG, WR, 2, WF>(xb, plane, wt, KB, s0 + 2, lds, wave, lane);
    if (VOX_GF_DIAG == 2) {
    } else if (s0 + 2 < s1) wait_vm<2 * (C::NA + C::NB)>();
    else if (s0 + 1 < s1) wait_vm<C::NA + C::NB>();
    else wait_vm<0>();
    asm volatile("" ::: "memory");
    __builtin_amdgcn_s_barrier();
    asm volatile("" ::: "memory");
    gf_read<NP, RB, NG, WR, 0, 0, WF>(lds, wave, lane, H0, raw);
    wait_lgkm0();
    gf_cvt<NP, RB, NG, WR, 0, WF>(raw, H0);
#define GF_STAGE(J)                                                                                              \
    if (s + J < s1) {                                                                                            \
        gf_read<NP, RB, NG, WR, J, 1, WF>(lds, wave, lane, H1, raw);                                             \
        gf_cvt<NP, RB, NG, WR, 1, WF>(raw, H1);                                                                  \
        __builtin_amdgcn_sched_barrier(0);                                                                       \
        gf_mma<NP, RB, NG, WR, WF>(H0, acc);                                                                     \
        __builtin_amdgcn_sched_barrier(0);                                                                       \
        wait_lgkm0();                                                                                            \
        if (s + J + 1 < s1) {                                                                                    \
            if (VOX_GF_DIAG == 2) {                                                                              \
            } else if (s + J + 2 < s1) wait_vm<C::NA + C::NB>();                                                 \
            else wait_vm<0>();                                                                                   \
            asm volatile("" ::: "memory");                                                                       \
            __builtin_amdgcn_s_barrier();                                                                        \
            asm volatile("" ::: "memory");                                                                       \
            if (s + J + 3 < s1) gf_issue<NP, RB, NG, WR, J, WF>(xb, plane, wt, KB, s + J + 3, lds, wave, lane);  \
            gf_read<NP, RB, NG, WR, (J + 1) % 3, 0, WF>(lds, wave, lane, H0, raw);                               \
        }                                                                                                        \
        __builtin_amdgcn_sched_barrier(0);                                                                       \
        gf_mma<NP, RB, NG, WR, WF>(H1, acc);                                                                     \
        __builtin_amdgcn_sched_barrier(0);                                                                       \
        wait_lgkm0();                                                                                            \
        if (s + J + 1 < s1) gf_cvt<NP, RB, NG, WR, 0, WF>(raw, H0);                                              \
    }
    for (int s = s0; s < s1; s += 3) {
        GF_STAGE(0)
        GF_STAGE(1)
        GF_STAGE(2)
    }
#undef GF_STAGE
    __builtin_amdgcn_s_barrier();
}

__device__ __forceinline__ long long gf_bound(long long U, int G, int b) { return U * b / G; }

__device__ __forceinline__ f32x4 gf_scaled(const f32x4& v, const float* sc) {
    const float4 s = *reinterpret_cast<const float4*>(sc);
    f32x4 r = {v[0] * s.x, v[1] * s.y, v[2] * s.z, v[3] * s.w};
#pragma unroll
    for (int e = 0; e < 4; e++) {
        float t = r[e];
        asm volatile("" : "+v"(t));
        r[e] = t;
    }
    return r;
}

template <int EPI, int WF = WF_BF16>
__device__ __forceinline__ void gf_out(const GemmfArgs& a, int m, int gg, int lane, const f32x4& w0, const f32x4& w1) {
    const int nq = gg * 16 + (lane >> 4) * 4;
    const f32x4 v0 = WF == WF_Q8 ? gf_scaled(w0, a.wscale + nq) : w0;
    if (EPI == EPI_SWIGLU) {
        const f32x4 v1 = WF == WF_Q8 ? gf_scaled(w1, a.wscale + nq + 16) : w1;
        const int h0 = (gg >> 1) * 16 + (lane >> 4) * 4;
        float v[4];
#pragma unroll
        for (int e = 0; e < 4; e++) v[e] = silu(v0[e]) * v1[e];
        if (a.xo) {
            const int H = a.N >> 1;
            uint32_t hp[2], mp[2], lq[2];
#pragma unroll
            for (int e = 0; e < 4; e += 2) {
                uint16_t h_0, m_0, l_0, h_1, m_1, l_1;
                split3(v[e], h_0, m_0, l_0);
                split3(v[e + 1], h_1, m_1, l_1);
                hp[e / 2] = h_0 | ((uint32_t)h_1 << 16);
                mp[e / 2] = m_0 | ((uint32_t)m_1 << 16);
                lq[e / 2] = l_0 | ((uint32_t)l_1 << 16);
            }
            *reinterpret_cast<uint2*>(a.xo + frag_at(m, H, 0, h0)) = make_uint2(hp[0], hp[1]);
            *reinterpret_cast<uint2*>(a.xo + frag_at(m, H, 1, h0)) = make_uint2(mp[0], mp[1]);
            *reinterpret_cast<uint2*>(a.xo + frag_at(m, H, 2, h0)) = make_uint2(lq[0], lq[1]);
        } else {
            *reinterpret_cast<float4*>(a.C + (size_t)m * a.ldc + h0) = make_float4(v[0], v[1], v[2], v[3]);
        }
        return;
    }
    const int n = gg * 16 + (lane >> 4) * 4;
    float4 v = make_float4(v0[0], v0[1], v0[2], v0[3]);
    if (a.bias) {
        const float4 bb = *reinterpret_cast<const float4*>(a.bias + n);
        v.x += bb.x; v.y += bb.y; v.z += bb.z; v.w += bb.w;
    }
    float4* cp = reinterpret_cast<float4*>(a.C + (size_t)m * a.ldc + n);
    if (EPI == EPI_RESID) {
        const float4 o = *cp;
        v.x += o.x; v.y += o.y; v.z += o.z; v.w += o.w;
    } else if (EPI == EPI_GELU) {
        v.x = gelu_tanh(v.x); v.y = gelu_tanh(v.y); v.z = gelu_tanh(v.z); v.w = gelu_tanh(v.w);
    } else if (EPI == EPI_GELU_ERF) {
        v.x = gelu_erf(v.x); v.y = gelu_erf(v.y); v.z = gelu_erf(v.z); v.w = gelu_erf(v.w);
    }
    *cp = v;
}

template <int EPI, int NP, int RB, int NG, int WR, int WF = WF_BF16>
__global__ __launch_bounds__(256 * WR, 1) void k_gemmf(const GemmfArgs a) {
    using C = GfCfg<NP, RB, NG, WR, WF>;
    constexpr int RBW = C::RBW;
    extern __shared__ __attribute__((aligned(16))) uint16_t gf_lds[];
    unsigned long long* s_okm = reinterpret_cast<unsigned long long*>(gf_lds + 3 * C::SLOT);
    const int tid = threadIdx.x, lane = tid & 63, wave = __builtin_amdgcn_readfirstlane(tid >> 6);
    const int wc = wave & 3, r0 = (wave >> 2) * RBW;
    const int G = gridDim.x, b = blockIdx.x;
    const int epoch = a.epoch_dev ? a.epoch + *a.epoch_dev : a.epoch;
    const long long u0 = gf_bound(a.U, G, b), u1 = gf_bound(a.U, G, b + 1);
    constexpr int TILE = C::NWV * RBW * NG * 256;
    const int rbm = (a.M + 15) >> 4;
    const __amdgpu_buffer_rsrc_t Ws = __builtin_amdgcn_make_buffer_rsrc(a.ws, 0, 0x7fffffff, 0x00020000);
    auto poff = [&](int slotb, int i, int g) {
        return (int)(((size_t)slotb * TILE + ((size_t)(wave * RBW + i) * NG + g) * 256 + lane * 4) * 4);
    };
    long long u = u0;
    while (u < u1) {
        const int t = (int)(u / a.S), s0 = (int)(u % a.S);
        const int s1 = (int)min((long long)a.S, s0 + (u1 - u));
        const int mt = a.colmajor ? t % a.MT : t / a.NT, nt = a.colmajor ? t / a.MT : t % a.NT;
        f32x4 acc[RBW][NG];
#pragma unroll
        for (int i = 0; i < RBW; i++)
#pragma unroll
            for (int g = 0; g < NG; g++) acc[i][g] = f32x4{0.f, 0.f, 0.f, 0.f};
        gf_stages<NP, RB, NG, WR, WF>(a, gf_lds, mt, nt, s0, s1, acc);
        u += s1 - s0;
        if (s0 > 0) {
#pragma unroll
            for (int i = 0; i < RBW; i++)
#pragma unroll
                for (int g = 0; g < NG; g++)
                    __builtin_amdgcn_raw_buffer_store_b128(__builtin_bit_cast(u32x4, acc[i][g]), Ws, poff(b, i, g), 0, 16);
            asm volatile("s_waitcnt vmcnt(0)" ::: "memory");
            __syncthreads();
            if (tid == 0) __hip_atomic_store(&a.flags[b], epoch, __ATOMIC_RELAXED, __HIP_MEMORY_SCOPE_AGENT);
            continue;
        }
        const long long tend = (long long)(t + 1) * a.S;
        int npb = 0;
        while (b + 1 + npb < G && gf_bound(a.U, G, b + 1 + npb) < tend) npb++;
        if (npb > 0) {
            if (wave == 0) {
                const bool mine = lane < npb;
                bool ok = !mine;
                const unsigned long long t0 = __builtin_amdgcn_s_memrealtime();
                while (a.wait_ticks >= 0) {
                    if (!ok) ok = __hip_atomic_load(&a.flags[b + 1 + lane], __ATOMIC_RELAXED, __HIP_MEMORY_SCOPE_AGENT) == epoch;
                    if (__builtin_amdgcn_ballot_w64(!ok) == 0) break;
                    if (__builtin_amdgcn_s_memrealtime() - t0 > (unsigned long long)a.wait_ticks) break;
                    __builtin_amdgcn_s_sleep(2);
                }
                if (mine && !ok) __hip_atomic_fetch_add(a.recomputes, 1, __ATOMIC_RELAXED, __HIP_MEMORY_SCOPE_AGENT);
                const unsigned long long okm = __builtin_amdgcn_ballot_w64(mine && ok);
                if (lane == 0) *s_okm = okm;
            }
            __syncthreads();
            const unsigned long long okm = *s_okm;
            __syncthreads();
            for (int k = 0; k < npb; k++) {
                const int pb = b + 1 + k;
                f32x4 part[RBW][NG];
                if ((okm >> k) & 1) {
#pragma unroll
                    for (int i = 0; i < RBW; i++)
#pragma unroll
                        for (int g = 0; g < NG; g++)
                            part[i][g] = __builtin_bit_cast(f32x4, __builtin_amdgcn_raw_buffer_load_b128(Ws, poff(pb, i, g), 0, 16));
// ... 6 lines not shown
                    const int q1 = (int)(min(gf_bound(a.U, G, pb + 1), tend) - (long long)t * a.S);
                    gf_stages<NP, RB, NG, WR, WF>(a, gf_lds, mt, nt, q0, q1, part);
                }
#pragma unroll
                for (int i = 0; i < RBW; i++)
#pragma unroll
                    for (int g = 0; g < NG; g++) acc[i][g] += part[i][g];
            }
        }
#pragma unroll
        for (int i = 0; i < RBW; i++) {
            const int rb = mt * RB + r0 + i;
            if (rb >= rbm) break;
            const int m = rb * 16 + (lane & 15);
            if (m >= a.M) continue;
#pragma unroll
            for (int g = 0; g < NG; g += (EPI == EPI_SWIGLU ? 2 : 1))
                gf_out<EPI, WF>(a, m, (nt * 4 + wc) * NG + g, lane, acc[i][g], acc[i][EPI == EPI_SWIGLU ? g + 1 : g]);
        }
    }
}

static int g_cus = 0;
int g_gemmf_blocks = -1;
int g_gemmf_rb = -1;
VOX_KB_KNOB(g_gemmf_minu, 0);
int g_gemmf_order = -1;
int g_gemmf_wr = -1;

template <int EPI, int NP, int RB, int NG, int WR, int WF = WF_BF16>
static hipError_t gemmf_launch(const GemmfArgs& a, int G, hipStream_t st) {
    using C = GfCfg<NP, RB, NG, WR, WF>;
    static bool attr = false;
    const size_t lds = (size_t)3 * C::SLOT * 2 + 16;
    if (!attr) {
        hipError_t e = hipFuncSetAttribute(reinterpret_cast<const void*>(&k_gemmf<EPI, NP, RB, NG, WR, WF>),
                                           hipFuncAttributeMaxDynamicSharedMemorySize, (int)lds);
        if (e != hipSuccess) return e;
        attr = true;
    }
    hipLaunchKernelGGL((k_gemmf<EPI, NP, RB, NG, WR, WF>), dim3(G), dim3(256 * WR), lds, st, a);
    return hipGetLastError();
}

size_t gemmf_ws_floats(int blocks) { return (size_t)blocks * (8 * 2 * 4 * 256); }

int gemmf_grid() {
    if (!g_cus) {
        int dev = 0;
        if (hipGetDevice(&dev) != hipSuccess ||
            hipDeviceGetAttribute(&g_cus, hipDeviceAttributeMultiprocessorCount, dev) != hipSuccess || g_cus <= 0)
            g_cus = 256;
    }
    if (g_gemmf_blocks < 0) {
        const char* e = getenv("VOX_HIP_GEMMF_BLOCKS");
        const int v = e ? atoi(e) : 0;
        g_gemmf_blocks = v > 0 && v <= 4 * g_cus ? v : 0;
    }
    return g_gemmf_blocks ? g_gemmf_blocks : g_cus;
}

size_t gemmf_flag_ints() { return (size_t)gemmf_grid() + 1; }
int set_gemmf_wait(int ticks) {
    const int old = g_gemmf_wait;
    g_gemmf_wait = ticks;
    return old;
}

__global__ void k_gemmf_epoch_bump(int* w, int by) {
    const int v = *w;
    *w = v > (1 << 30) ? 1 : v + by;
}

hipError_t launch_gemmf_epoch_bump(int* epoch_dev, int by, hipStream_t st) {
    if (!epoch_dev || by < 1) return hipErrorInvalidValue;
    hipLaunchKernelGGL(k_gemmf_epoch_bump, dim3(1), dim3(1), 0, st, epoch_dev, by);
    return hipGetLastError();
}

int gemmf_wide_rb(int M, int N, int) { return (M > 64 && N / 128 >= gemmf_grid()) ? 8 : 4; }

bool gemmf_ok(int M, int N, int K) { return M > 0 && M <= 1024 && K % 64 == 0 && N % 128 == 0; }

hipError_t launch_gemmf(int epi, int np, const uint16_t* xs, int K, int M, const void* Wf, int N, const float* bias,
                        float* C, int ldc, uint16_t* xo, float* ws, size_t ws_floats, int* flags, int epoch,
                        hipStream_t st, const int* epoch_dev, int rb, const float* wscale) {
    constexpr int NG = 2, WR = 2;
    if (g_gemmf_rb < 0) {
        const char* e = getenv("VOX_HIP_GEMMF_RB");
        const int v = e ? atoi(e) : 0;
        g_gemmf_rb = (v == 4 || v == 8) ? v : 0;
    }
    if (!gemmf_ok(M, N, K) || (np != 2 && np != 3) || !ws || !flags || (g_gemmf_rb && g_gemmf_rb != 4 && g_gemmf_rb != 8) ||
        (rb && rb != 4 && rb != 8))
        return hipErrorInvalidValue;
    const int NGx = NG;
    const int t8 = ((M + 127) / 128) * (N / (64 * NG));
    const int RB = np == 3 ? 4 : g_gemmf_rb ? g_gemmf_rb : rb ? rb : (t8 >= gemmf_grid() ? 8 : 4);
    GemmfArgs a;
    a.xs = xs; a.K = K; a.M = M; a.W = static_cast<const uint8_t*>(Wf); a.N = N; a.wscale = wscale; a.bias = bias; a.C = C; a.ldc = ldc;
    a.xo = xo; a.ws = ws; a.flags = flags; a.epoch = epoch; a.epoch_dev = epoch_dev;
    a.recomputes = flags + gemmf_grid();
    a.wait_ticks = g_gemmf_wait;
    a.S = K / 64;
    a.NT = N / (64 * NGx);
    a.MT = (M + 16 * RB - 1) / (16 * RB);
    a.T = a.MT * a.NT;
    if (g_gemmf_order < 0) {
        const char* e = getenv("VOX_HIP_GEMMF_ORDER");
        const int v = e ? atoi(e) : 0;
        g_gemmf_order = (v == 1 || v == 2) ? v : 0;
    }
    a.colmajor = g_gemmf_order ? g_gemmf_order == 1 : (np == 3 && a.MT > 4 && (a.MT % 4 != 0 || K > 2048));
    a.U = (long long)a.T * a.S;
    const long long minu = g_gemmf_minu ? g_gemmf_minu
                           : a.MT <= 2 ? std::max(6, a.S / 8) : std::max(4, (a.S + 1) / 2);
    if ((a.S + minu - 1) / minu + 2 > 64) return hipErrorInvalidConfiguration;
    int G = gemmf_grid();
    if ((long long)G * minu > a.U) G = (int)std::max(1LL, a.U / minu);
    if ((size_t)G * 4 * RB * NGx * 256 > ws_floats) return hipErrorInvalidConfiguration;
#define GF_EPI(E)                                                                               \
    if (epi == E)                                                                               \
        return wscale ? (np == 3   ? gemmf_launch<E, 3, 4, NG, WR, WF_Q8>(a, G, st)             \
                         : RB == 8 ? gemmf_launch<E, 2, 8, NG, WR, WF_Q8>(a, G, st)             \
                                   : gemmf_launch<E, 2, 4, NG, WR, WF_Q8>(a, G, st))            \
               : np == 3 ? gemmf_launch<E, 3, 4, NG, WR>(a, G, st)                              \
               : g_gemmf_wr == 4 ? (RB == 8 ? gemmf_launch<E, 2, 8, NG, 4>(a, G, st)             \
                                            : gemmf_launch<E, 2, 4, NG, 4>(a, G, st))            \
               : RB == 8 ? gemmf_launch<E, 2, 8, NG, WR>(a, G, st) : gemmf_launch<E, 2, 4, NG, WR>(a, G, st);
    if (g_gemmf_wr < 0) {
        const char* e = getenv("VOX_HIP_GEMMF_WR");
        g_gemmf_wr = (e && atoi(e) == 2) ? 2 : 4;
    }

    GF_EPI(EPI_STORE) GF_EPI(EPI_RESID) GF_EPI(EPI_GELU) GF_EPI(EPI_GELU_ERF) GF_EPI(EPI_SWIGLU)
#undef GF_EPI
    return hipErrorInvalidValue;
}

}
```

voxtral.c_amd/csrc/vox_hip_internal.h:

```cpp
#pragma once
#include <hip/hip_runtime.h>
#include <stdint.h>

namespace vox {

enum { EPI_STORE = 0, EPI_RESID = 1, EPI_GELU = 2, EPI_GELU_ERF = 3, EPI_SWIGLU = 4, EPI_QKV = 5, EPI_LOGITS = 6,
       EPI_LOGITS_ALT = 7,
       EPI_PARTIAL = 8,
       EPI_QKV_BIAS = 9 };
constexpr int ALT_TEXT_MIN = 1000;
constexpr int ALT_PART = 10;
constexpr int ALT_REC = 8;
enum { PRO_NONE = 0, PRO_NORM = 1, PRO_NORM_ADA = 2 };
enum { WF_BF16 = 0, WF_Q8 = 1, WF_P13 = 2, WF_MX4 = 3 };

constexpr int GEMV_MAX_BLOCKS = 1024;

struct GemvArgs {
    const float* x;
    int K;
    const void* W;
    const float* wscale;
    const void* wp_main = nullptr;
    const void* wp_side = nullptr;
    int wp_d = 0;
    const void* wm_plane = nullptr;
    int rows;
    const float* norm_w;
    const float* ada;
    float eps;
    float* y;
    const float* bias;
    int qd, kvd, hd;
    const float* rope;
    const int* state;
    int pos;
    float* Kc;
    float* Vc;
    int cap;
    int kvt = 0;
    float* part_val;
    int* part_idx;
    float* part_alt;
};

enum { KV_F32 = 0, KV_F16 = 1, KV_FP8 = 2 };
static inline size_t kv_esize(int kvt) { return kvt == KV_FP8 ? 1 : kvt == KV_F16 ? 2 : 4; }

constexpr int VOX_MAX_BATCH = 32;
constexpr int VOX_MAX_SLOTS = 128;

struct BatchSlot {
    int* state;
    int* tokens;
    const float* adapter;
    char* Kc;
    char* Vc;
    float* alts;
    int adapter_rows;
    int left;
    int stop_tok;
    int live;
    int pos;
    int produced;
    const float* ada;
};
static_assert(sizeof(BatchSlot) == 80, "BatchSlot layout");
constexpr int GEMVR_MAX_ROWS = 8;
struct GemvRArgs {
    GemvArgs g;
    int ldx, ldy;
    const BatchSlot* slots;
    size_t ring_off;
};
constexpr int BATCH_TOKLOG = 64;

struct AttnPtrs {
    const float* q[VOX_MAX_BATCH];
    const float* Kc[VOX_MAX_BATCH];
    const float* Vc[VOX_MAX_BATCH];
    const int* state[VOX_MAX_BATCH];
    float* part[VOX_MAX_BATCH];
    float* out[VOX_MAX_BATCH];
    const BatchSlot* slots = nullptr;
    size_t ring_off = 0;
};
struct AttnSlots {
    const float* q;
    float* part;
    float* out;
    size_t q_ld, part_ld, out_ld;
    const BatchSlot* slots;
// ... 84 lines not shown
hipError_t launch_attn_batch_dbg(const AttnPtrs& p, const AttnFuse& f, int nb, int cap, int window, float scale, int H,
                                 int KVH, int splits, hipStream_t st);
hipError_t launch_attn_dbg(int dbg, const float* q, const float* Kc, const float* Vc, int cap,
                           const int* state, float* part, float* out, hipStream_t st);
hipError_t launch_embed_step(const float* adapter, const void* emb, const float* esc, const int* state,
                             int D, float* x, hipStream_t st);
hipError_t launch_embed_rows(const float* adapter, const void* emb, const float* esc, int row0, int n,
                             int first_tok, int rest_tok, int D, float* x, hipStream_t st);
hipError_t launch_argmax_final(const float* pv, const int* pi, int n, int* state, int* tokens,
                               int cap, const float* adapter, int adapter_rows,
                               const void* emb, const float* esc, int D, float* x,
                               const float* part_alt, float* alts, int V, hipStream_t st);
hipError_t launch_embed_batch(const BatchSlot* slots, int nb, const void* emb, const float* esc, int D, float* x,
                              hipStream_t st);
hipError_t launch_argmax_batch(const float* logits, int nb, int V, float* pval, int* pidx, float* palt,
                               BatchSlot* slots, int tokens_cap, int* toklog, const void* emb, const float* esc, int D,
                               float* x, hipStream_t st);
#ifdef VOX_KBENCH
#define VOX_KB_KNOB(name, v) int name = v
#else
#define VOX_KB_KNOB(name, v) constexpr int name = v
#endif
constexpr int SK_ROWS = 16;
constexpr int SK_MAX_ROWS = 96;
constexpr int PLANE_MAX_ROWS = 1024;
hipError_t launch_frag_pack(const void* src, int N, int K, int q8, void* dst, hipStream_t st);
hipError_t launch_rmsnorm_fplanes(float* x, int nb, int D, const float* w, const float* ada, float eps,
                                  uint16_t* xs, const float* part, int S, hipStream_t st, const float* bias = nullptr);
hipError_t launch_rmsnorm_fplanes_slots(float* x, int nb, int D, const float* w, const BatchSlot* slots, size_t ada_off,
                                        float eps, uint16_t* xs, hipStream_t st);
hipError_t launch_resid_slabs(float* x, int nb, int D, const float* part, int S, const float* bias, hipStream_t st);
hipError_t launch_slabs_rows(const float* part, int S, int nb, int N, const float* bias, float* out, int ldo,
                             hipStream_t st);
hipError_t launch_split_fplanes(const float* x, int nb, int K, uint16_t* xs, hipStream_t st);
hipError_t launch_swiglu_fplanes(const float* part, int S, int H, int nb, uint16_t* xs, hipStream_t st);
hipError_t launch_gemm_skf(const uint16_t* xs, int K, const void* Wf, const float* wscale, int N, int nb, float* C,
                           int ldc, hipStream_t st, int mx4 = 0);
hipError_t launch_gemm_skf2(const uint16_t* xs, int K, const void* Wf, const float* wscale, int N, int nb, float* C,
                            int ldc, hipStream_t st, int mx4 = 0);
int skl_splits(int K, int N = 0);
constexpr int SKL_MAX_SLICES = 12;
hipError_t launch_gemm_skl(const uint16_t* xs, int K, const void* Wf, const float* wscale, int N, int nb,
                           float* part, hipStream_t st, const float* ssq = nullptr, int nsl = 0, float eps = 0.f,
                           int pair = 0, int mx4 = 0);
hipError_t launch_gemm_skl_cfg(int nw, int ks, const uint16_t* xs, int K, const void* Wf, int N, int nb, float* part,
                               hipStream_t st);
hipError_t launch_gemm_skl2_cfg(int nw, int ks, const uint16_t* xs, int K, const void* Wf, int N, int nb, float* part,
                                hipStream_t st);
hipError_t launch_resid_xw_fplanes(float* x, int nb, int D, const float* w, const float* ada, uint16_t* xs,
                                   const float* part, int S, const float* bias, float* ssq, hipStream_t st);
hipError_t launch_resid_xw_fplanes_slots(float* x, int nb, int D, const float* w, const BatchSlot* slots, size_t ada_off,
                                         uint16_t* xs, const float* part, int S, const float* bias, float* ssq,
                                         hipStream_t st);
enum { SKX_PRO_PLANES = 0, SKX_PRO_SCALE = 1 };
enum { SKX_EPI_QKV = 1, SKX_EPI_RESID = 2, SKX_EPI_SWIGLU = 3 };
struct SklFused {
    const float* ssq_in = nullptr;
    int nsl = 0;
    float eps = 0.f;
    float* part = nullptr;
    int* ticket = nullptr;
    const float* bias = nullptr;
    float* x = nullptr;
    float* ssq_out = nullptr;
    uint16_t* planes = nullptr;
    const float* nw = nullptr;
    const float* ada = nullptr;
    const float* rope = nullptr;
    int qd = 0, kvd = 0, hd = 0, pos0 = 0, cap = 0;
    float* q = nullptr;
    float* Kc = nullptr;
    float* Vc = nullptr;
    int kvt = 0;
};
int sklx_slices(int N, int K);
constexpr int SKX_TICKETS = 4 * 1024;
hipError_t launch_gemm_sklx(int pro, int epi, const uint16_t* xs, int K, const void* Wf, int N, int nb,
                            const SklFused& f, hipStream_t st, int mx4 = 0);
bool gemmf_ok(int M, int N, int K);
int gemmf_grid();
size_t gemmf_flag_ints();
int set_gemmf_wait(int ticks);
size_t gemmf_ws_floats(int blocks);
hipError_t launch_gemmf(int epi, int np, const uint16_t* xs, int K, int M, const void* Wf, int N, const float* bias,
                        float* C, int ldc, uint16_t* xo, float* ws, size_t ws_floats, int* flags, int epoch,
                        hipStream_t st, const int* epoch_dev = nullptr, int rb = 0, const float* wscale = nullptr);
hipError_t launch_gemmf_epoch_bump(int* epoch_dev, int by, hipStream_t st);
int gemmf_wide_rb(int M, int N, int K);
int gemm_planes_np();
int set_gemm_planes(int np);
hipError_t launch_im2col3(const float* src, int C, int T, int stride, int off, float* A,
                          hipStream_t st);
hipError_t launch_mel_tail(const float* melp, int n_new, int MB, float* tail, hipStream_t st);
hipError_t launch_mel_frames(const float* samples, long long start0, int nframes, const float* window,
                             const float* dcosT, const float* dsinT, const float* filtT, float log_min, float* mel,
                             hipStream_t st);
hipError_t launch_mel_reflect(float* buf, long long n, long long real_end, int len, hipStream_t st);

}
```

voxtral.c_amd/csrc/vox_hip_kernels.hip:

```cpp
#include "vox_hip_internal.h"
#include "vox_hip_dev.h"

#include <hip/hip_runtime.h>
#include <hip/hip_ext.h>
#include <stdint.h>
#include <algorithm>
#include <type_traits>
#include <string.h>
#include <stdlib.h>

namespace vox {

typedef _Float16 kvh_t;
typedef _Float16 h16x4 __attribute__((ext_vector_type(4)));
typedef _Float16 h16x2 __attribute__((ext_vector_type(2)));
__device__ __forceinline__ float kv8_clamp(float v) { return v > 448.f ? 448.f : v < -448.f ? -448.f : v; }
__device__ __forceinline__ unsigned kv8_fix_nan(float v, unsigned code) {
    return v != v ? (0x7fu | ((__float_as_uint(v) >> 24) & 0x80u)) : code;
}
__device__ __forceinline__ unsigned kv8_enc2(float a, float b) {
    const unsigned w = (unsigned)__builtin_amdgcn_cvt_pk_fp8_f32(kv8_clamp(a), kv8_clamp(b), 0, false);
    return kv8_fix_nan(a, w & 0xffu) | (kv8_fix_nan(b, (w >> 8) & 0xffu) << 8);
}
struct kv8_t {
    uint8_t b;
    kv8_t() = default;
    __device__ __forceinline__ explicit kv8_t(float v) : b((uint8_t)(kv8_enc2(v, v) & 0xffu)) {}
    __device__ __forceinline__ explicit operator float() const {
        return __builtin_amdgcn_cvt_pk_f32_fp8((int)b, false)[0];
    }
};
static_assert(sizeof(kv8_t) == 1, "kv8_t: one byte per ring element");
template <class T> __device__ __forceinline__ float4 kv_ld4(const T* p) {
    if constexpr (sizeof(T) == 4) {
        return *reinterpret_cast<const float4*>(p);
    } else if constexpr (sizeof(T) == 2) {
        const h16x4 h = *reinterpret_cast<const h16x4*>(p);
        return make_float4((float)h[0], (float)h[1], (float)h[2], (float)h[3]);
    } else {
        const int w = *reinterpret_cast<const int*>(p);
        const auto lo = __builtin_amdgcn_cvt_pk_f32_fp8(w, false), hi = __builtin_amdgcn_cvt_pk_f32_fp8(w, true);
        return make_float4(lo[0], lo[1], hi[0], hi[1]);
    }
}
template <class T> __device__ __forceinline__ float2 kv_ld2(const T* p) {
    if constexpr (sizeof(T) == 4) {
        return *reinterpret_cast<const float2*>(p);
    } else if constexpr (sizeof(T) == 2) {
        const h16x2 h = *reinterpret_cast<const h16x2*>(p);
        return make_float2((float)h[0], (float)h[1]);
    } else {
        const auto v = __builtin_amdgcn_cvt_pk_f32_fp8((int)*reinterpret_cast<const uint16_t*>(p), false);
        return make_float2(v[0], v[1]);
    }
}
template <class T> __device__ __forceinline__ float kv_round(float v) { return (float)(T)v; }
template <class T> __device__ __forceinline__ void kv_st2(T* p, float a, float b) {
    if constexpr (sizeof(T) == 4) {
        *reinterpret_cast<float2*>(p) = make_float2(a, b);
    } else if constexpr (sizeof(T) == 2) {
        *reinterpret_cast<h16x2*>(p) = h16x2{(T)a, (T)b};
    } else {
        *reinterpret_cast<uint16_t*>(p) = (uint16_t)kv8_enc2(a, b);
    }
}
__device__ __forceinline__ float kv_f32(float v) {
    asm volatile("" : "+v"(v));
    return v;
}
__device__ __forceinline__ void kv_st2_rt(float* base, size_t e, float a, float b, int kvt) {
    if (kvt == KV_FP8) kv_st2(reinterpret_cast<kv8_t*>(base) + e, a, b);
    else if (kvt == KV_F16) kv_st2(reinterpret_cast<kvh_t*>(base) + e, a, b);
    else kv_st2(base + e, a, b);
}

__global__ __launch_bounds__(256) void k_rmsnorm_rows(const float* __restrict__ x, int ldx,
                                                      float* __restrict__ y, int ldy,
                                                      const float* __restrict__ w,
                                                      const float* __restrict__ ada, int D,
                                                      float eps) {
    __shared__ float red[4];
    const float* xr = x + (size_t)blockIdx.x * ldx;
    float* yr = y + (size_t)blockIdx.x * ldy;
    float ss = 0.f;
    for (int i = threadIdx.x; i < D; i += 256) ss = fmaf(xr[i], xr[i], ss);
    ss = wave_sum(ss);
    if ((threadIdx.x & 63) == 0) red[threadIdx.x >> 6] = ss;
    __syncthreads();
    float tot = red[0] + red[1] + red[2] + red[3];
    float inv = 1.0f / sqrtf(tot / (float)D + eps);
    for (int i = threadIdx.x; i < D; i += 256) {
        float v = xr[i] * inv * w[i];
        if (ada) v *= (1.0f + ada[i]);
        yr[i] = v;
    }
}

__global__ __launch_bounds__(256) void k_rmsnorm_rows_slot(const float* __restrict__ x, int ldx,
                                                           float* __restrict__ y, int ldy,
                                                           const float* __restrict__ w,
                                                           const BatchSlot* __restrict__ slots, size_t ada_off,
                                                           int D, float eps) {
    __shared__ float red[4];
    const float* xr = x + (size_t)blockIdx.x * ldx;
    float* yr = y + (size_t)blockIdx.x * ldy;
    float ss = 0.f;
    for (int i = threadIdx.x; i < D; i += 256) ss = fmaf(xr[i], xr[i], ss);
    ss = wave_sum(ss);
    if ((threadIdx.x & 63) == 0) red[threadIdx.x >> 6] = ss;
    __syncthreads();
    float tot = red[0] + red[1] + red[2] + red[3];
    float inv = 1.0f / sqrtf(tot / (float)D + eps);
    const float* ab = slots[blockIdx.x].ada;
    const float* ada = ab ? ab + ada_off : nullptr;
    for (int i = threadIdx.x; i < D; i += 256) {
        float v = xr[i] * inv * w[i];
        if (ada) v *= (1.0f + ada[i]);
        yr[i] = v;
    }
}

#define G2_M 128
#define G2_N 128
#define G2_K 64
#define G2_LDS (G2_K + 8)
#ifndef VOX_G2_DIAG
#define VOX_G2_DIAG 0
#endif

template <int AV>
struct G2Regs {
    float4 a[AV];
    uint4 w[4];
};

template <int WQ8, int AV>
__device__ __forceinline__ void g2_load(G2Regs<AV>& r, const float* __restrict__ Ap, const uint16_t* __restrict__ Wp,
                                        const int8_t* __restrict__ Wq, int ko) {
    const float4* a = reinterpret_cast<const float4*>(Ap + ko);
#pragma unroll
    for (int i = 0; i < AV; i++) r.a[i] = a[i];
    if (WQ8) {
        const uint4* q = reinterpret_cast<const uint4*>(Wq + ko);
        r.w[0] = q[0];
        r.w[1] = q[1];
    } else {
        const uint4* w = reinterpret_cast<const uint4*>(Wp + ko);
#pragma unroll
        for (int i = 0; i < 4; i++) r.w[i] = w[i];
    }
}

template <int WQ8, int NP, int AV>
__device__ __forceinline__ void g2_store(const G2Regs<AV>& r, uint16_t* base, int srow, int sk, int wrow, int wk,
                                         float amask) {
    constexpr int PLANE = 128 * (64 + 8);
    const float4* ra = r.a;
// ... 4190 lines not shown
```

voxtral.c_amd/vox_hip.py:

```python
from __future__ import annotations

import ctypes
import os

import numpy as np

from vox_weights import (VoxConfig, Weights, build_weights_struct, config_struct_class,
                         weights_struct_class)

_HERE = os.path.dirname(os.path.abspath(__file__))
LIB_PATH = os.environ.get("VOX_HIP_LIB") or os.path.join(_HERE, "libvoxtral_hip.so")

TOKEN_BOS, TOKEN_EOS, TOKEN_STREAMING_PAD = 1, 2, 32
STREAM_FIRST_CHUNK_MIN_MEL = 312
STREAM_DEFAULT_INTERVAL = 2.0
RAW_AUDIO_LENGTH_PER_TOK = 1280
OFFLINE_STREAMING_BUFFER_TOKENS = 10

ConfigC = config_struct_class()
WeightsC = weights_struct_class()

class WPackStatsC(ctypes.Structure):
    _fields_ = [("packed_tensors", ctypes.c_int), ("raw_tensors", ctypes.c_int),
                ("packed_bytes", ctypes.c_longlong), ("packed_raw_bytes", ctypes.c_longlong),
                ("raw_bytes", ctypes.c_longlong), ("pack_ms", ctypes.c_double)]


class WMx4StatsC(ctypes.Structure):
    _fields_ = [("wmx4_tensors", ctypes.c_int), ("refused_tensors", ctypes.c_int),
                ("plane_bytes", ctypes.c_longlong), ("bf16_bytes", ctypes.c_longlong),
                ("bits_per_weight", ctypes.c_double), ("scan_ms", ctypes.c_double),
                ("round_ms", ctypes.c_double), ("pack_ms", ctypes.c_double)]


def gemv_wpack(W_bf16, x, packed):
    init()
    W = np.ascontiguousarray(W_bf16, np.uint16)
    xv = np.ascontiguousarray(x, np.float32)
    rows, K = W.shape
    assert xv.shape == (K,)
    y = np.empty(rows, np.float32)
    rc = lib().vox_hip_gemv_wpack(rows, K, W.ctypes.data, fptr(xv), fptr(y), int(packed))
    if rc < 0:
        _err("gemv_wpack")
    return y, (rc if int(packed) == 2 else bool(rc))


def gemv_rows(W_bf16, x, packed):
    init()
    W = np.ascontiguousarray(W_bf16, np.uint16)
    xv = np.ascontiguousarray(x, np.float32)
    rows, K = W.shape
    assert xv.ndim == 2 and xv.shape[1] == K
    R = xv.shape[0]
    y = np.empty((R, rows), np.float32)
    rc = lib().vox_hip_gemv_rows(rows, K, W.ctypes.data, fptr(xv), R, fptr(y), int(packed))
    if rc < 0:
        _err("gemv_rows")
    return y, rc


def _q8_args(W_i8, scales, x):
    W = np.ascontiguousarray(W_i8, np.int8)
    sc = np.ascontiguousarray(scales, np.float32)
    xv = np.ascontiguousarray(x, np.float32)
    rows, K = W.shape
    assert sc.shape == (rows,) and xv.shape[-1] == K
    return W, sc, xv, rows, K


def gemv_rows_q8(W_i8, scales, x):
    init()
    W, sc, xv, rows, K = _q8_args(W_i8, scales, x)
    assert xv.ndim == 2
    R = xv.shape[0]
    y = np.empty((R, rows), np.float32)
    if lib().vox_hip_gemv_rows_q8(rows, K, W.ctypes.data, fptr(sc), fptr(xv), R, fptr(y)) < 0:
        _err("gemv_rows_q8")
    return y


def gemv_q8(W_i8, scales, x):
    init()
    W, sc, xv, rows, K = _q8_args(W_i8, scales, x)
    assert xv.ndim == 1
    y = np.empty(rows, np.float32)
    if lib().vox_hip_gemv_q8(rows, K, W.ctypes.data, fptr(sc), fptr(xv), fptr(y)) < 0:
        _err("gemv_q8")
    return y


EXPORTS = [
    "vox_hip_init", "vox_hip_available", "vox_hip_shutdown", "vox_hip_memory_used",
    "vox_hip_last_error", "vox_hip_clear_error", "vox_hip_set_device", "vox_hip_config_voxtral_4b",
    "vox_hip_model_create", "vox_hip_model_free", "vox_hip_model_set_delay",
    "vox_hip_model_ada_scale", "vox_hip_model_set_kv_fp16", "vox_hip_stream_kv_fp16",
    "vox_hip_model_set_kv_dtype", "vox_hip_stream_kv_dtype", "vox_hip_stream_read_kv", "vox_hip_kv8_convert",
    "vox_hip_model_set_enc_kv_fp16", "vox_hip_stream_enc_kv_fp16", "vox_hip_stream_read_enc_kv",
    "vox_hip_stream_enc_kv_bytes", "vox_hip_stream_enc_paths",
    "vox_hip_model_set_kv_grow", "vox_hip_stream_kv_slots", "vox_hip_stream_kv_bytes",
    "vox_hip_stream_kv_grow_stats", "vox_hip_stream_reserve_kv", "vox_hip_batch_kv_grow_stats",
    "vox_hip_model_wpack_stats", "vox_hip_gemv_wpack",
    "vox_hip_set_wmx4", "vox_hip_wmx4", "vox_hip_model_wmx4_stats",
    "vox_hip_set_wmx4_batch", "vox_hip_wmx4_batch", "vox_hip_model_wmx4_batch_stats", "vox_hip_batch_set_wmx4",
    "vox_hip_skinny_wmx4",
    "vox_hip_set_gemm_planes", "vox_hip_gemm_planes", "vox_hip_set_gemmf_wait",
    "vox_hip_set_gemmf_q8", "vox_hip_gemmf_q8", "vox_hip_model_gemmf_q8_stats", "vox_hip_gemmf_q8_rows",
    "vox_hip_stream_create", "vox_hip_stream_free",
    "vox_hip_stream_reset", "vox_hip_stream_reset_decoder", "vox_hip_stream_encode_mel",
    "vox_hip_stream_set_delay", "vox_hip_stream_delay", "vox_hip_stream_ada_scale",
    "vox_hip_stream_adapter_tokens", "vox_hip_stream_read_adapter", "vox_hip_stream_decode",
    "vox_hip_set_adapter_rows0", "vox_hip_stream_adapter_stats",
    "vox_hip_batch_create", "vox_hip_batch_free", "vox_hip_batch_decode", "vox_hip_batch_decode_rows",
    "vox_hip_batch_begin_rows", "vox_hip_batch_finish",
    "vox_hip_batch_read_logits",
    "vox_hip_batch_stats", "vox_hip_batch_set_gemv_rows", "vox_hip_batch_gemv_stats", "vox_hip_gemv_rows",
    "vox_hip_batch_set_gemv_wmx4", "vox_hip_batch_gemv_wmx4_stats", "vox_hip_batch_set_prefill_kv",
    "vox_hip_batch_set_gemv_rows_q8", "vox_hip_gemv_rows_q8", "vox_hip_gemv_q8",
    "vox_hip_stream_state", "vox_hip_stream_set_alt", "vox_hip_stream_read_alts", "vox_hip_sgemm_bf16", "vox_hip_sgemm_q8", "vox_hip_fused_qkv_bf16",
    "vox_hip_fused_ffn_bf16", "vox_hip_encoder_attention", "vox_hip_encoder_full_step",
    "vox_hip_decoder_prefill_step", "vox_hip_decoder_start", "vox_hip_decoder_end",
    "vox_hip_decoder_full_step", "vox_hip_stream_set_profiling", "vox_hip_stream_profile",
    "vox_hip_stream_sync", "vox_hip_stream_set_async_encode", "vox_hip_stream_encode_mel_batch", "vox_hip_device_upload", "vox_hip_device_free",
    "vox_hip_mel_create", "vox_hip_mel_feed", "vox_hip_mel_finish", "vox_hip_mel_frames",
    "vox_hip_mel_frame_ptr", "vox_hip_mel_discard_before", "vox_hip_mel_read", "vox_hip_mel_free", "vox_hip_mel_reset",
]

_lib = None


def lib():
    global _lib
    if _lib is not None:
        return _lib
    if not os.path.exists(LIB_PATH):
        raise RuntimeError(f"{LIB_PATH} not built (run __graft_entry__.build())")
    L = ctypes.CDLL(LIB_PATH)
    P, I, F = ctypes.c_void_p, ctypes.c_int, ctypes.c_float
    fp = ctypes.POINTER(ctypes.c_float)
    ip = ctypes.POINTER(ctypes.c_int)
    sig = {
        "vox_hip_init": (I, []), "vox_hip_available": (I, []), "vox_hip_shutdown": (None, []),
        "vox_hip_memory_used": (ctypes.c_size_t, []), "vox_hip_last_error": (ctypes.c_char_p, []),
        "vox_hip_clear_error": (None, []),
        "vox_hip_set_device": (I, [I]),
        "vox_hip_config_voxtral_4b": (None, [P]),
        "vox_hip_model_create": (P, [P, P, I]), "vox_hip_model_free": (None, [P]),
        "vox_hip_model_set_delay": (I, [P, I]), "vox_hip_model_ada_scale": (I, [P, fp]),
        "vox_hip_model_set_kv_fp16": (I, [P, I]), "vox_hip_stream_kv_fp16": (I, [P]),
        "vox_hip_model_set_kv_dtype": (I, [P, I]), "vox_hip_stream_kv_dtype": (I, [P]),
        "vox_hip_stream_read_kv": (I, [P, I, I, I, P, P]),
        "vox_hip_model_set_enc_kv_fp16": (I, [P, I]), "vox_hip_stream_enc_kv_fp16": (I, [P]),
        "vox_hip_stream_read_enc_kv": (I, [P, I, I, I, P, P]),
        "vox_hip_stream_enc_kv_bytes": (ctypes.c_longlong, [P]),
        "vox_hip_stream_enc_paths": (I, [P, ctypes.POINTER(ctypes.c_longlong)]),
        "vox_hip_model_set_kv_grow": (I, [P, I]), "vox_hip_stream_kv_slots": (I, [P]),
        "vox_hip_stream_kv_bytes": (ctypes.c_longlong, [P]),
        "vox_hip_stream_kv_grow_stats": (I, [P, ctypes.POINTER(ctypes.c_longlong)]),
        "vox_hip_stream_reserve_kv": (I, [P, I]),
        "vox_hip_batch_kv_grow_stats": (I, [P, ctypes.POINTER(ctypes.c_longlong)]),
        "vox_hip_kv8_convert": (I, [fp, I, P, fp]),
        "vox_hip_model_wpack_stats": (I, [P, P]),
        "vox_hip_gemv_wpack": (I, [I, I, P, fp, fp, I]),
        "vox_hip_set_wmx4": (I, [I]), "vox_hip_wmx4": (I, []), "vox_hip_model_wmx4_stats": (I, [P, P]),
        "vox_hip_set_wmx4_batch": (I, [I]), "vox_hip_wmx4_batch": (I, []),
        "vox_hip_model_wmx4_batch_stats": (I, [P, ctypes.POINTER(ctypes.c_longlong)]),
        "vox_hip_batch_set_wmx4": (I, [P, I]),
        "vox_hip_skinny_wmx4": (I, [I, I, P, fp, I, fp, I, I]),
        "vox_hip_set_gemm_planes": (I, [I]), "vox_hip_gemm_planes": (I, []),
        "vox_hip_set_gemmf_wait": (I, [I]),
        "vox_hip_set_gemmf_q8": (I, [I]), "vox_hip_gemmf_q8": (I, []),
        "vox_hip_model_gemmf_q8_stats": (I, [P, ctypes.POINTER(ctypes.c_longlong)]),
        "vox_hip_gemmf_q8_rows": (I, [I, I, I, fp, P, fp, fp, I]),
        "vox_hip_stream_create": (P, [P]), "vox_hip_stream_free": (None, [P]),
        "vox_hip_stream_reset": (I, [P]), "vox_hip_stream_reset_decoder": (I, [P]),
        "vox_hip_stream_set_delay": (I, [P, I]), "vox_hip_stream_delay": (I, [P]),
        "vox_hip_stream_ada_scale": (I, [P, fp]),
        "vox_hip_stream_encode_mel": (I, [P, P, I, I]),
        "vox_hip_stream_adapter_tokens": (I, [P]),
        "vox_hip_set_adapter_rows0": (I, [I]),
        "vox_hip_stream_adapter_stats": (I, [P, ctypes.POINTER(ctypes.c_longlong)]),
        "vox_hip_stream_read_adapter": (I, [P, I, I, fp]),
        "vox_hip_stream_decode": (I, [P, I, I, ip, fp]),
        "vox_hip_stream_state": (I, [P, ip]),
        "vox_hip_batch_create": (P, [P, I]), "vox_hip_batch_free": (None, [P]),
        "vox_hip_batch_decode": (I, [P, ctypes.POINTER(ctypes.c_void_p), I, I, I, ip, ip]),
        "vox_hip_batch_decode_rows": (I, [P, ctypes.POINTER(ctypes.c_void_p), I, ip, I, I, ip, ip]),
        "vox_hip_batch_begin_rows": (I, [P, ctypes.POINTER(ctypes.c_void_p), I, ip, I, I, ip, ip]),
        "vox_hip_batch_finish": (I, [P]),
        "vox_hip_batch_read_logits": (I, [P, P, fp]),
        "vox_hip_batch_stats": (I, [P, ctypes.POINTER(ctypes.c_longlong)]),
        "vox_hip_batch_set_gemv_rows": (I, [P, I]),
        "vox_hip_batch_gemv_stats": (I, [P, ctypes.POINTER(ctypes.c_longlong)]),
        "vox_hip_gemv_rows": (I, [I, I, P, fp, I, fp, I]),
        "vox_hip_batch_set_gemv_wmx4": (I, [P, I]),
        "vox_hip_batch_gemv_wmx4_stats": (I, [P, ctypes.POINTER(ctypes.c_longlong)]),
        "vox_hip_batch_set_prefill_kv": (I, [P, I]),
        "vox_hip_batch_set_gemv_rows_q8": (I, [P, I]),
        "vox_hip_gemv_rows_q8": (I, [I, I, P, fp, fp, I, fp]),
        "vox_hip_gemv_q8": (I, [I, I, P, fp, fp, fp]),
        "vox_hip_stream_set_alt": (I, [P, I, F]),
        "vox_hip_stream_read_alts": (I, [P, I, I, ip, fp]),
        "vox_hip_sgemm_bf16": (None, [I, I, I, fp, P, fp]),
        "vox_hip_sgemm_q8": (None, [I, I, I, fp, P, fp, fp]),
        "vox_hip_fused_qkv_bf16": (None, [I, I, fp, P, I, P, I, P, I, fp, fp, fp]),
        "vox_hip_fused_ffn_bf16": (None, [I, I, I, fp, P, P, P, fp]),
        "vox_hip_encoder_attention": (None, [fp, fp, fp, fp, I, I, I, I, I, F, I, I]),
        "vox_hip_encoder_full_step": (I, [P, fp, I, fp, I]),
        "vox_hip_decoder_prefill_step": (I, [P, fp, I, fp, I]),
        "vox_hip_decoder_start": (None, [P, fp, I]), "vox_hip_decoder_end": (None, [P]),
        "vox_hip_decoder_full_step": (I, [P, fp, I, fp]),
        "vox_hip_stream_set_profiling": (I, [P, I]),
        "vox_hip_stream_profile": (I, [P, ctypes.POINTER(ctypes.c_double)]),
        "vox_hip_stream_sync": (I, [P]),
        "vox_hip_stream_set_async_encode": (I, [P, I]),
        "vox_hip_stream_encode_mel_batch": (I, [P, P, P, I, I, P]),
        "vox_hip_device_upload": (P, [P, ctypes.c_size_t]),
        "vox_hip_device_free": (I, [P]),
        "vox_hip_mel_create": (P, [P, I]), "vox_hip_mel_feed": (I, [P, fp, I]),
        "vox_hip_mel_finish": (I, [P, I]), "vox_hip_mel_frames": (I, [P, ip]),
        "vox_hip_mel_frame_ptr": (P, [P, I]), "vox_hip_mel_discard_before": (I, [P, I]),
        "vox_hip_mel_read": (I, [P, I, I, fp]), "vox_hip_mel_free": (None, [P]), "vox_hip_mel_reset": (I, [P, I]),
    }
    for name, (res, args) in sig.items():
        fn = getattr(L, name)
        fn.restype = res
        fn.argtypes = args
    _lib = L
    return L


def fptr(a: np.ndarray):
    assert a.dtype == np.float32 and a.flags.c_contiguous
    return a.ctypes.data_as(ctypes.POINTER(ctypes.c_float))


def _err(what):
    msg = lib().vox_hip_last_error()
    raise RuntimeError(f"{what}: {msg.decode() if msg else 'unknown error'}")


KV_F32, KV_F16, KV_FP8 = 0, 1, 2
MAX_DELAY_TOKENS = 30
KV_NP_DTYPE = {KV_F32: np.float32, KV_F16: np.float16, KV_FP8: np.uint8}


def kv8_decode(codes) -> np.ndarray:
    c = np.arange(256)
    e, m = (c >> 3) & 15, (c & 7).astype(np.float64)
    v = np.where(e == 0, m * 2.0 ** -9, (8 + m) * 2.0 ** (e - 10.0))
    v[(c & 0x7f) == 0x7f] = np.nan
    lut = np.where(c & 0x80, -v, v).astype(np.float32)
    return lut[np.asarray(codes, np.uint8)]


def kv8_convert(x):
    x = np.ascontiguousarray(x, np.float32).ravel()
    codes = np.empty(x.size, np.uint8)
    back = np.empty(x.size, np.float32)
    if lib().vox_hip_kv8_convert(fptr(x), x.size, codes.ctypes.data, fptr(back)) != 0:
        _err("kv8_convert")
    return codes, back


def set_gemm_planes(planes: int):
    if lib().vox_hip_set_gemm_planes(int(planes)) != 0:
        _err("set_gemm_planes")


def gemm_planes() -> int:
    return lib().vox_hip_gemm_planes()


def set_wmx4(mode: int):
    if lib().vox_hip_set_wmx4(int(mode)) != 0:
        _err("set_wmx4")


def wmx4() -> int:
    return lib().vox_hip_wmx4()


def set_wmx4_batch(on: bool):
    if lib().vox_hip_set_wmx4_batch(int(bool(on))) != 0:
        _err("set_wmx4_batch")


def wmx4_batch() -> int:
    return lib().vox_hip_wmx4_batch()


def skinny_wmx4(W_bf16, x, fmt: int, head: bool = False) -> np.ndarray:
    init()
    W = np.ascontiguousarray(W_bf16, np.uint16)
    xv = np.ascontiguousarray(x, np.float32)
    N, K = W.shape
    assert xv.ndim == 2 and xv.shape[1] == K
    nb = xv.shape[0]
    y = np.empty((nb, N), np.float32)
    if lib().vox_hip_skinny_wmx4(N, K, W.ctypes.data, fptr(xv), nb, fptr(y), int(fmt), int(bool(head))) != 0:
        _err("skinny_wmx4")
    return y


def set_gemmf_wait(ticks: int) -> int:
    return lib().vox_hip_set_gemmf_wait(int(ticks))


def set_gemmf_q8(on: bool):
    if lib().vox_hip_set_gemmf_q8(int(bool(on))) != 0:
        _err("set_gemmf_q8")


def gemmf_q8() -> int:
    return lib().vox_hip_gemmf_q8()


def gemmf_q8_rows(x, W_i8, scales, fmt: int) -> np.ndarray:
    init()
    W, sc, xv, N, K = _q8_args(W_i8, scales, x)
    assert xv.ndim == 2
    M = xv.shape[0]
    y = np.empty((M, N), np.float32)
    if lib().vox_hip_gemmf_q8_rows(M, N, K, fptr(xv), W.ctypes.data, fptr(sc), fptr(y), int(fmt)) != 0:
        _err("gemmf_q8_rows")
    return y


def set_adapter_rows0(rows: int):
    if lib().vox_hip_set_adapter_rows0(int(rows)) != 0:
        _err("set_adapter_rows0")


def init(device: int | None = None):
    L = lib()
    if device is not None and L.vox_hip_set_device(device) != 0:
        _err("set_device")
    if not L.vox_hip_init():
        _err("vox_hip_init (no GPU?)")


class Model:

    def __init__(self, cfg: VoxConfig, weights: Weights, delay_tokens: int = 6):
        init()
        self.cfg = cfg
        self.delay_tokens = delay_tokens
        self._cfg_c = cfg.ctypes_struct(ConfigC)
        wstruct, keep = build_weights_struct(weights, WeightsC)
        self.h = lib().vox_hip_model_create(ctypes.byref(self._cfg_c), ctypes.byref(wstruct), delay_tokens)
        if not self.h:
            _err("vox_hip_model_create")

    def set_delay(self, delay_ms: int):
        delay_ms = min(max(delay_ms, 80), 2400)
        self.delay_tokens = delay_ms // 80
        if lib().vox_hip_model_set_delay(self.h, self.delay_tokens) != 0:
            _err("set_delay")

    def set_kv_fp16(self, on: bool):
        if lib().vox_hip_model_set_kv_fp16(self.h, int(on)) != 0:
            _err("set_kv_fp16")

    def set_kv_dtype(self, dtype: int):
        if lib().vox_hip_model_set_kv_dtype(self.h, int(dtype)) != 0:
            _err("set_kv_dtype")

    def set_enc_kv_fp16(self, on: bool):
        if lib().vox_hip_model_set_enc_kv_fp16(self.h, int(on)) != 0:
            _err("set_enc_kv_fp16")

    def set_kv_grow(self, slots0: int):
        if lib().vox_hip_model_set_kv_grow(self.h, int(slots0)) != 0:
            _err("set_kv_grow")

    def wpack_stats(self) -> dict:
        st = WPackStatsC()
        if lib().vox_hip_model_wpack_stats(self.h, ctypes.byref(st)) != 0:
            _err("wpack_stats")
        return {name: getattr(st, name) for name, _ in WPackStatsC._fields_}

    def wmx4_stats(self) -> dict:
        st = WMx4StatsC()
        if lib().vox_hip_model_wmx4_stats(self.h, ctypes.byref(st)) != 0:
            _err("wmx4_stats")
        return {name: getattr(st, name) for name, _ in WMx4StatsC._fields_}

    def wmx4_batch_stats(self) -> dict:
        out = (ctypes.c_longlong * 4)()
        if lib().vox_hip_model_wmx4_batch_stats(self.h, out) != 0:
            _err("wmx4_batch_stats")
        return dict(zip(("tensors", "plane_bytes", "bf16_bytes", "host_us"), (int(v) for v in out)))

    def gemmf_q8_stats(self) -> list:
        out = (ctypes.c_longlong * 4)()
        if lib().vox_hip_model_gemmf_q8_stats(self.h, out) != 0:
            _err("gemmf_q8_stats")
        return [int(v) for v in out]

    def ada_scale(self):
        c = self.cfg
        out = np.empty(c.dec_layers * c.dec_dim, np.float32)
        lib().vox_hip_model_ada_scale(self.h, fptr(out))
        return out.reshape(c.dec_layers, c.dec_dim)

    def close(self):
        if self.h:
            lib().vox_hip_model_free(self.h)
            self.h = None


# ... 690 lines not shown
```

Before: 750.0.

## Fuse RoPE and KV-ring store into QKV gemmf epilogue; skip last prefill layer tail

Adds an EPI_QKV_ROPE epilogue to the fused gemmf kernel so the QKV projection applies rotary embedding and writes Q plus the K/V ring directly, with no separate rope_kv launch and no qkv round trip through memory. The fused epilogue is gated by VOX_HIP_GEMMF_ROPE and is off by default. Decoder prefill separately gains a kv_tail mode: the last layer stops after writing K/V and skips attention, the output projection and the FFN, because only the KV cache is needed. That skip is on by default unless VOX_HIP_PREFILL_TAIL=1. Test entry points and shared KV helpers moved to a header are also added.

```diff
diff --git a/include/voxtral_hip.h b/include/voxtral_hip.h
--- a/include/voxtral_hip.h
+++ b/include/voxtral_hip.h
@@ -88,6 +88,13 @@
 int vox_hip_model_gemmf_q8_stats(const vox_hip_model_t *m, long long out4[4]);
 int vox_hip_gemmf_q8_rows(int M, int N, int K, const float *x, const int8_t *Wq, const float *scales, float *y,
                           int fmt);
+int vox_hip_set_gemmf_rope(int on);
+int vox_hip_set_prefill_tail(int on);
+int vox_hip_gemmf_rows(int M, int N, int K, const float *x, const uint16_t *W, const float *bias, int epi, float *y,
+                       long long *recomputes);
+int vox_hip_gemmf_rope_rows(int M, int qd, int kvd, int hd, int K, const float *x, const uint16_t *W,
+                            const float *bias, const float *rope, int pos0, int cap, int kvt, int fused,
+                            float *q_out, void *k_out, void *v_out);
 
 vox_hip_stream_t *vox_hip_stream_create(vox_hip_model_t *m);
 void vox_hip_stream_free(vox_hip_stream_t *s);
diff --git a/voxtral.c_amd/csrc/vox_hip.hip b/voxtral.c_amd/csrc/vox_hip.hip
--- a/voxtral.c_amd/csrc/vox_hip.hip
+++ b/voxtral.c_amd/csrc/vox_hip.hip
@@ -1667,7 +1667,7 @@
 };
 
 static int gemmf_on(const GemmfQ& q, int epi, const uint16_t* xs, int K, int n, const uint8_t* W, const float* wscale,
-                    int N, const float* bias, float* C, int ldc, uint16_t* xo) {
+                    int N, const float* bias, float* C, int ldc, uint16_t* xo, const GemmfRope* rope = nullptr) {
     if (!q.epoch_dev) {
         hipStreamCaptureStatus cs = hipStreamCaptureStatusNone;
         CK(hipStreamIsCapturing(q.st, &cs));
@@ -1681,7 +1681,7 @@
         if (pend != hipSuccess) return set_err("k_gemmf: HIP error pending before the launch: %s", hipGetErrorString(pend));
     }
     CK(launch_gemmf(epi, gemm_planes_np(), xs, K, n, W, N, bias, C, ldc, xo, q.ws, q.ws_n, q.flags, *q.epoch, q.st,
-                    q.epoch_dev, q.epoch_dev ? gemmf_wide_rb(n, N, K) : 0, wscale));
+                    q.epoch_dev, q.epoch_dev ? gemmf_wide_rb(n, N, K) : 0, wscale, rope));
     if (wscale) {
         ++*q.n_q8;
         if (q.step_q8) ++*q.step_q8;
@@ -1713,6 +1713,35 @@
     const float* table = nullptr;
     const BatchSlot* slots = nullptr;
 };
+struct RowsRope {
+    const vox_hip_stream_t* s = nullptr;
+    bool enc = false;
+    GemmfRope r{};
+};
+
+static int g_gemmf_rope = -1;
+static int gemmf_rope_on() {
+    if (g_gemmf_rope < 0) g_gemmf_rope = env_on("VOX_HIP_GEMMF_ROPE");
+    return g_gemmf_rope;
+}
+static int g_prefill_tail = -1;
+static int prefill_tail_on() {
+    if (g_prefill_tail < 0) {
+        const char* e = getenv("VOX_HIP_PREFILL_TAIL");
+        g_prefill_tail = e && atoi(e) == 1 ? 1 : 0;
+    }
+    return g_prefill_tail;
+}
+extern "C" int vox_hip_set_gemmf_rope(int on) {
+    const int old = gemmf_rope_on();
+    g_gemmf_rope = on ? 1 : 0;
+    return old;
+}
+extern "C" int vox_hip_set_prefill_tail(int on) {
+    const int old = prefill_tail_on();
+    g_prefill_tail = on ? 1 : 0;
+    return old;
+}
 
 static RowsLayer enc_rows_layer(const vox_hip_model_t* m, int l) {
     const EncLayerD& L = m->enc[l];
@@ -1737,20 +1766,28 @@
 
 template <class Attn>
 static int rows_layers(const vox_hip_model_t* m, const RowsStack& S, const RowsScratch& B, const GemmfQ& q, bool gf, int n,
-                       Attn attn, const RowsAda& ada = RowsAda{}) {
+                       Attn attn, const RowsAda& ada = RowsAda{}, bool kv_tail = false, const RowsRope& rope = RowsRope{}) {
     const int D = S.D, NQKV = S.Q + 2 * S.KV, HID = S.hidden;
     hipStream_t st = q.st;
+    const bool roped = gf && rope.s && gemm_planes_np() == 3;
     for (int l = 0; l < S.layers; l++) {
         RowsLayer L = S.layer(m, l);
         if (ada.table) L.ada = ada.table + (size_t)l * D;
+        const bool kv_only = kv_tail && l == S.layers - 1;
         if (gf) {
             CK(launch_rmsnorm_fplanes(B.x, n, D, L.attn_norm, nullptr, S.eps, B.pa, nullptr, 0, st));
-            if (gemmf_on(q, EPI_STORE, B.pa, D, n, L.fqkv, L.sqkv, NQKV, L.bqkv, B.qkv, NQKV, nullptr)) return -1;
+            if (roped) {
+                GemmfRope r = rope.r;
+                r.Kc = rope.enc ? enc_ring(rope.s, rope.s->ek, l) : dec_ring(rope.s, rope.s->dk, l);
+                r.Vc = rope.enc ? enc_ring(rope.s, rope.s->ev, l) : dec_ring(rope.s, rope.s->dv, l);
+                if (gemmf_on(q, EPI_QKV_ROPE, B.pa, D, n, L.fqkv, L.sqkv, NQKV, L.bqkv, nullptr, NQKV, nullptr, &r)) return -1;
+            } else if (gemmf_on(q, EPI_STORE, B.pa, D, n, L.fqkv, L.sqkv, NQKV, L.bqkv, B.qkv, NQKV, nullptr)) return -1;
         } else {
             CK(launch_rmsnorm_rows(B.x, D, B.xn, D, L.attn_norm, nullptr, n, D, S.eps, st));
             CK(launch_gemm(EPI_STORE, 3, B.xn, D, L.wqkv, L.sqkv, D, n, NQKV, L.bqkv, B.qkv, NQKV, st, q.ws, q.ws_n));
         }
-        if (attn(l, gf ? B.pa : nullptr)) return -1;
+        if (attn(l, gf ? B.pa : nullptr, kv_only, roped)) return -1;
+        if (kv_only) break;
         if (gf) {
             if (gemmf_on(q, EPI_RESID, B.pa, S.Q, n, L.fo, L.so, D, L.bo, B.x, D, nullptr)) return -1;
             if (ada.slots) CK(launch_rmsnorm_fplanes_slots(B.x, n, D, L.ffn_norm, ada.slots, (size_t)l * D, S.eps, B.pa, st));
@@ -1847,14 +1884,20 @@
     s->enc_paths[3]++;
     const bool gf = enc_gemmf_ok(m, n);
     if (gf && stream_enc_planes(s)) return -1;
-    if (rows_layers(m, enc_rows_stack(c), enc_rows_scratch(s, x), stream_gemmfq(s), gf, n, [&](int l, uint16_t* planes) -> int {
+    RowsRope rr;
+    if (gf && gemmf_rope_on() && gemmf_rope_ok(EQ, EKV, hd, s->ekvt)) {
+        rr.s = s;
+        rr.enc = true;
+        rr.r = GemmfRope{EQ, EKV, hd, rope, (int)pos0, s->q, nullptr, nullptr, s->ecap, s->ekvt};
+    }
+    if (rows_layers(m, enc_rows_stack(c), enc_rows_scratch(s, x), stream_gemmfq(s), gf, n, [&](int l, uint16_t* planes, bool, bool roped) -> int {
             float* Kc = enc_ring(s, s->ek, l);
             float* Vc = enc_ring(s, s->ev, l);
-            CK(launch_rope_kv(s->qkv, n, EQ, EKV, hd, rope, (int)pos0, s->q, Kc, Vc, s->ecap, st, s->ekvt));
+            if (!roped) CK(launch_rope_kv(s->qkv, n, EQ, EKV, hd, rope, (int)pos0, s->q, Kc, Vc, s->ecap, st, s->ekvt));
             CK(launch_attn_rows_mf(hd, s->q, EQ, Kc, Vc, s->ecap, s->att, EQ, n, H, KVH, (int)pos0, 0, c.enc_window, scale,
                                    st, s->gws, s->gws_n, planes, s->ekvt));
             return 0;
-        }))
+        }, RowsAda{}, false, rr))
         return -1;
     CK(launch_rmsnorm_rows(x, ED, x, ED, m->enc_norm, nullptr, n, ED, c.enc_eps, st));
     return 0;
@@ -2102,7 +2145,7 @@
         er.nr[b] = nr[b];
         er.pos0[b] = (int)pos0[b];
     }
-    if (rows_layers(m, enc_rows_stack(c), enc_rows_scratch(lead, X), stream_gemmfq(lead), gf, N, [&](int l, uint16_t* planes) -> int {
+    if (rows_layers(m, enc_rows_stack(c), enc_rows_scratch(lead, X), stream_gemmfq(lead), gf, N, [&](int l, uint16_t* planes, bool, bool) -> int {
             for (int b = 0; b < B; b++) {
                 er.Kc[b] = enc_ring(ss[b], ss[b]->ek, l);
                 er.Vc[b] = enc_ring(ss[b], ss[b]->ev, l);
@@ -2313,7 +2356,7 @@
     return RowsScratch{x, s->qkvd, s->xnd, s->attd, s->gated, s->dpa, s->dpc};
 }
 
-static int run_decoder_rows(vox_hip_stream_t* s, float* x, int n, int pos0, const float* rope) {
+static int run_decoder_rows(vox_hip_stream_t* s, float* x, int n, int pos0, const float* rope, bool kv_tail = false) {
     vox_hip_model_t* m = s->m;
     const vox_hip_config_t& c = m->c;
     const int H = c.dec_heads, KVH = c.dec_kv_heads, hd = c.dec_head_dim;
@@ -2328,14 +2371,20 @@
         (void)hipGetLastError();
         gf = false;
     }
-    return rows_layers(m, dec_rows_stack(c), dec_rows_scratch(s, x), stream_gemmfq(s), gf, n, [&](int l, uint16_t* planes) -> int {
+    RowsRope rr;
+    if (gf && gemmf_rope_on() && gemmf_rope_ok(DQ, DKV, hd, s->kvt)) {
+        rr.s = s;
+        rr.r = GemmfRope{DQ, DKV, hd, rope, pos0, s->qd_, nullptr, nullptr, s->dcap, s->kvt};
+    }
+    return rows_layers(m, dec_rows_stack(c), dec_rows_scratch(s, x), stream_gemmfq(s), gf, n, [&](int l, uint16_t* planes, bool kv_only, bool roped) -> int {
         float* Kc = dec_ring(s, s->dk, l);
         float* Vc = dec_ring(s, s->dv, l);
-        CK(launch_rope_kv(s->qkvd, n, DQ, DKV, hd, rope, pos0, s->qd_, Kc, Vc, s->dcap, st, s->kvt));
+        if (!roped) CK(launch_rope_kv(s->qkvd, n, DQ, DKV, hd, rope, pos0, s->qd_, Kc, Vc, s->dcap, st, s->kvt));
+        if (kv_only) return 0;
         CK(launch_attn_rows_mf(hd, s->qd_, DQ, Kc, Vc, s->dcap, s->attd, DQ, n, H, KVH, pos0, 0, c.dec_window, scale, st,
                                s->gws, s->gws_n, planes, s->kvt));
         return 0;
-    }, RowsAda{s->delay < 0 ? nullptr : stream_ada(s), nullptr});
+    }, RowsAda{s->delay < 0 ? nullptr : stream_ada(s), nullptr}, kv_tail && !prefill_tail_on(), rr);
 }
 
 enum { T_QKV, T_WO, T_W13, T_W2 };
@@ -2537,7 +2586,7 @@
     if (ensure_rope(s, np + 2)) return -1;
     CK(launch_embed_rows(s->adapter, m->tok_emb, m->tok_emb_s, 0, np, TOKEN_BOS, TOKEN_STREAMING_PAD, m->c.dec_dim,
                          s->xd, s->st));
-    if (run_decoder_rows(s, s->xd, np, 0, m->rope_dec)) return -1;
+    if (run_decoder_rows(s, s->xd, np, 0, m->rope_dec, true)) return -1;
     return stream_prefilled(s, s->st);
 }
 
@@ -3112,6 +3161,132 @@
     };
     const int rc = run();
     dfree(dW); dfree(dF); dfree(dx); dfree(dxs); dfree(dy); dfree(ds); dfree(dws); dfree(dflags);
+    return rc ? -1 : 0;
+}
+
+namespace {
+struct GemmfRowsBufs {
+    uint8_t *dW = nullptr, *dF = nullptr;
+    float *dx = nullptr, *dws = nullptr, *db = nullptr;
+    uint16_t* dxs = nullptr;
+    int* dflags = nullptr;
+    size_t ws_n = 0;
+    ~GemmfRowsBufs() { dfree(dW); dfree(dF); dfree(dx); dfree(dws); dfree(db); dfree(dxs); dfree(dflags); }
+    int make(int M, int N, int K, const float* x, const uint16_t* W, const float* bias) {
+        const size_t rows = (size_t)(M + 127) / 128 * 128;
+        ws_n = gemmf_ws_floats(gemmf_grid());
+        CK(dalloc(&dW, (size_t)N * K * 2));
+        if (upload(dW, W, (size_t)N * K * 2) || frag_copy(&dF, dW, N, K, 0)) return -1;
+        CK(dalloc(&dx, (size_t)M * K));
+        CK(dalloc(&dxs, rows * 3 * K));
+        CK(dalloc(&dws, ws_n));
+        CK(dalloc(&dflags, gemmf_flag_ints()));
+        if (upload(dx, x, (size_t)M * K * 4)) return -1;
+        if (bias) {
+            CK(dalloc(&db, (size_t)N));
+            if (upload(db, bias, (size_t)N * 4)) return -1;
+        }
+        CK(launch_split_fplanes(dx, M, K, dxs, g_twin_st));
+        return 0;
+    }
+};
+}
+
+extern "C" int vox_hip_gemmf_rows(int M, int N, int K, const float* x, const uint16_t* W, const float* bias, int epi,
+                                  float* y, long long* recomputes) {
+    std::lock_guard<std::mutex> lk(g_twin_mu);
+    if (!x || !W || !y) return set_err("gemmf_rows: null argument");
+    if (epi != EPI_STORE && epi != EPI_RESID && epi != EPI_SWIGLU) return set_err("gemmf_rows: epi is 0 (store), 1 (residual) or 4 (SwiGLU)");
+    if (!gemmf_ok(M, N, K) || M > PLANE_MAX_ROWS || (epi == EPI_SWIGLU && (bias || N % 256)))
+        return set_err("gemmf_rows: k_gemmf does not take M %d N %d K %d (M 1..1024, N %% 128, K %% 64)", M, N, K);
+    if (twin_init()) return -1;
+    GemmfRowsBufs B;
+    float* dy = nullptr;
+    uint16_t* dxo = nullptr;
+    const int NO = epi == EPI_SWIGLU ? N / 2 : N;
+    const size_t rows = (size_t)(M + 127) / 128 * 128;
+    std::vector<uint16_t> xo;
+    auto run = [&]() -> int {
+        if (B.make(M, N, K, x, W, bias)) return -1;
+        if (epi == EPI_SWIGLU) {
+            CK(dalloc(&dxo, rows * 3 * NO));
+            xo.resize(rows * 3 * NO);
+        } else {
+            CK(dalloc(&dy, (size_t)M * N));
+            if (epi == EPI_RESID && upload(dy, y, (size_t)M * N * 4)) return -1;
+        }
+        CK(launch_gemmf(epi, 3, B.dxs, K, M, B.dF, N, B.db, dy, NO, dxo, B.dws, B.ws_n, B.dflags, 1, g_twin_st));
+        CK(hipStreamSynchronize(g_twin_st));
+        if (epi == EPI_SWIGLU) CK(hipMemcpy(xo.data(), dxo, xo.size() * 2, hipMemcpyDeviceToHost));
+        else CK(hipMemcpy(y, dy, (size_t)M * N * 4, hipMemcpyDeviceToHost));
+        if (recomputes) {
+            int rc = 0;
+            CK(hipMemcpy(&rc, B.dflags + gemmf_grid(), 4, hipMemcpyDeviceToHost));
+            *recomputes = rc;
+        }
+        return 0;
+    };
+    const int rc = run();
+    dfree(dy);
+    dfree(dxo);
+    if (rc) return -1;
+    if (epi == EPI_SWIGLU) {
+        auto bf = [](uint16_t b) {
+            const uint32_t u = (uint32_t)b << 16;
+            float f;
+            memcpy(&f, &u, 4);
+            return (double)f;
+        };
+        for (int j = 0; j < M; j++)
+            for (int k = 0; k < NO; k++) {
+                const int b = k >> 6, r = k & 63;
+                const size_t off = ((size_t)(b * 2 + ((r >> 3) & 1)) * 64 + (r >> 4) * 16 + (j & 15)) * 8 + (r & 7);
+                double v = 0;
+                for (int p = 0; p < 3; p++) v += bf(xo[((size_t)(j >> 4) * 3 + p) * SK_ROWS * NO + off]);
+                y[(size_t)j * NO + k] = (float)v;
+            }
+    }
+    return 0;
+}
+
+extern "C" int vox_hip_gemmf_rope_rows(int M, int qd, int kvd, int hd, int K, const float* x, const uint16_t* W,
+                                       const float* bias, const float* rope, int pos0, int cap, int kvt, int fused,
+                                       float* q_out, void* k_out, void* v_out) {
+    std::lock_guard<std::mutex> lk(g_twin_mu);
+    if (!x || !W || !rope || !q_out || !k_out || !v_out) return set_err("gemmf_rope_rows: null argument");
+    const int N = qd + 2 * kvd;
+    if (!gemmf_rope_ok(qd, kvd, hd, kvt) || cap < 1 || pos0 < 0 || !gemmf_ok(M, N, K) || M > PLANE_MAX_ROWS)
+        return set_err("gemmf_rope_rows: k_gemmf's RoPE epilogue does not take M %d qd %d kvd %d hd %d K %d ring type %d", M, qd,
+                       kvd, hd, K, kvt);
+    if (twin_init()) return -1;
+    GemmfRowsBufs B;
+    float *dqkv = nullptr, *dq = nullptr, *dK = nullptr, *dV = nullptr, *drope = nullptr;
+    const size_t esz = kvt == KV_FP8 ? 1 : kvt == KV_F16 ? 2 : 4;
+    const size_t ring_f = ((size_t)cap * kvd * esz + 3) / 4;
+    auto run = [&]() -> int {
+        if (B.make(M, N, K, x, W, bias)) return -1;
+        CK(dalloc(&dqkv, (size_t)M * N));
+        CK(dalloc(&dq, (size_t)M * qd));
+        CK(dalloc(&dK, ring_f));
+        CK(dalloc(&dV, ring_f));
+        CK(dalloc(&drope, (size_t)M * hd));
+        if (upload(drope, rope, (size_t)M * hd * 4)) return -1;
+        if (fused) {
+            const GemmfRope r{qd, kvd, hd, drope, pos0, dq, dK, dV, cap, kvt};
+            CK(launch_gemmf(EPI_QKV_ROPE, 3, B.dxs, K, M, B.dF, N, B.db, nullptr, N, nullptr, B.dws, B.ws_n, B.dflags, 1,
+                            g_twin_st, nullptr, 0, nullptr, &r));
+        } else {
+            CK(launch_gemmf(EPI_STORE, 3, B.dxs, K, M, B.dF, N, B.db, dqkv, N, nullptr, B.dws, B.ws_n, B.dflags, 1, g_twin_st));
+            CK(launch_rope_kv(dqkv, M, qd, kvd, hd, drope, pos0, dq, dK, dV, cap, g_twin_st, kvt));
+        }
+        CK(hipStreamSynchronize(g_twin_st));
+        CK(hipMemcpy(q_out, dq, (size_t)M * qd * 4, hipMemcpyDeviceToHost));
+        CK(hipMemcpy(k_out, dK, (size_t)cap * kvd * esz, hipMemcpyDeviceToHost));
+        CK(hipMemcpy(v_out, dV, (size_t)cap * kvd * esz, hipMemcpyDeviceToHost));
+        return 0;
+    };
+    const int rc = run();
+    dfree(dqkv); dfree(dq); dfree(dK); dfree(dV); dfree(drope);
     return rc ? -1 : 0;
 }
 
@@ -3817,7 +3992,7 @@
     AttnFuse af;
     af.qkv = b->wqkv; af.S = 1; af.N = QKV; af.rope = m->rope_dec; af.xs = b->wpa;
     if (rows_layers(m, dec_rows_stack(c), RowsScratch{b->x, b->wqkv, b->wxn, b->att, b->whid, b->wpa, b->wpc}, q, gf, nb,
-                    [&](int l, uint16_t*) -> int {
+                    [&](int l, uint16_t*, bool, bool) -> int {
                         ap.ring_off = (size_t)l * ring_layer;
                         ap.layer = l;
                         if (ragged) CK(launch_attn_batch_wide_rag(hd, ap, af, nb, c.dec_window, scale, H, KVH, splits, st, kvt));
@@ -3956,7 +4131,7 @@
     }
     if (rows_layers(m, dec_rows_stack(c), dec_rows_scratch(lead, X),
                     GemmfQ{st, gws, gws_n, b->gflags, &b->gepoch, &m->n_gemmf_q8, nullptr, nullptr}, gf, N,
-                    [&](int l, uint16_t* planes) -> int {
+                    [&](int l, uint16_t* planes, bool, bool) -> int {
                         for (int i = 0; i < B; i++) {
                             er.Kc[i] = dec_ring(ss[i], ss[i]->dk, l);
                             er.Vc[i] = dec_ring(ss[i], ss[i]->dv, l);
diff --git a/voxtral.c_amd/csrc/vox_hip_dev.h b/voxtral.c_amd/csrc/vox_hip_dev.h
--- a/voxtral.c_amd/csrc/vox_hip_dev.h
+++ b/voxtral.c_amd/csrc/vox_hip_dev.h
@@ -223,4 +223,67 @@
     return __builtin_bit_cast(bf16x8, make_uint4(h[0] | (h[1] << 16), h[2] | (h[3] << 16), h[4] | (h[5] << 16), h[6] | (h[7] << 16)));
 }
 
-}
+typedef _Float16 kvh_t;
+typedef _Float16 h16x4 __attribute__((ext_vector_type(4)));
+typedef _Float16 h16x2 __attribute__((ext_vector_type(2)));
+__device__ __forceinline__ float kv8_clamp(float v) { return v > 448.f ? 448.f : v < -448.f ? -448.f : v; }
+__device__ __forceinline__ unsigned kv8_fix_nan(float v, unsigned code) {
+    return v != v ? (0x7fu | ((__float_as_uint(v) >> 24) & 0x80u)) : code;
+}
+__device__ __forceinline__ unsigned kv8_enc2(float a, float b) {
+    const unsigned w = (unsigned)__builtin_amdgcn_cvt_pk_fp8_f32(kv8_clamp(a), kv8_clamp(b), 0, false);
+    return kv8_fix_nan(a, w & 0xffu) | (kv8_fix_nan(b, (w >> 8) & 0xffu) << 8);
+}
+struct kv8_t {
+    uint8_t b;
+    kv8_t() = default;
+    __device__ __forceinline__ explicit kv8_t(float v) : b((uint8_t)(kv8_enc2(v, v) & 0xffu)) {}
+    __device__ __forceinline__ explicit operator float() const {
+        return __builtin_amdgcn_cvt_pk_f32_fp8((int)b, false)[0];
+    }
+};
+static_assert(sizeof(kv8_t) == 1, "kv8_t: one byte per ring element");
+template <class T> __device__ __forceinline__ float4 kv_ld4(const T* p) {
+    if constexpr (sizeof(T) == 4) {
+        return *reinterpret_cast<const float4*>(p);
+    } else if constexpr (sizeof(T) == 2) {
+        const h16x4 h = *reinterpret_cast<const h16x4*>(p);
+        return make_float4((float)h[0], (float)h[1], (float)h[2], (float)h[3]);
+    } else {
+        const int w = *reinterpret_cast<const int*>(p);
+        const auto lo = __builtin_amdgcn_cvt_pk_f32_fp8(w, false), hi = __builtin_amdgcn_cvt_pk_f32_fp8(w, true);
+        return make_float4(lo[0], lo[1], hi[0], hi[1]);
+    }
+}
+template <class T> __device__ __forceinline__ float2 kv_ld2(const T* p) {
+    if constexpr (sizeof(T) == 4) {
+        return *reinterpret_cast<const float2*>(p);
+    } else if constexpr (sizeof(T) == 2) {
+        const h16x2 h = *reinterpret_cast<const h16x2*>(p);
+        return make_float2((float)h[0], (float)h[1]);
+    } else {
+        const auto v = __builtin_amdgcn_cvt_pk_f32_fp8((int)*reinterpret_cast<const uint16_t*>(p), false);
+        return make_float2(v[0], v[1]);
+    }
+}
+template <class T> __device__ __forceinline__ float kv_round(float v) { return (float)(T)v; }
+template <class T> __device__ __forceinline__ void kv_st2(T* p, float a, float b) {
+    if constexpr (sizeof(T) == 4) {
+        *reinterpret_cast<float2*>(p) = make_float2(a, b);
+    } else if constexpr (sizeof(T) == 2) {
+        *reinterpret_cast<h16x2*>(p) = h16x2{(T)a, (T)b};
+    } else {
+        *reinterpret_cast<uint16_t*>(p) = (uint16_t)kv8_enc2(a, b);
+    }
+}
+__device__ __forceinline__ float kv_f32(float v) {
+    asm volatile("" : "+v"(v));
+    return v;
+}
+__device__ __forceinline__ void kv_st2_rt(float* base, size_t e, float a, float b, int kvt) {
+    if (kvt == KV_FP8) kv_st2(reinterpret_cast<kv8_t*>(base) + e, a, b);
+    else if (kvt == KV_F16) kv_st2(reinterpret_cast<kvh_t*>(base) + e, a, b);
+    else kv_st2(base + e, a, b);
+}
+
+}
diff --git a/voxtral.c_amd/csrc/vox_hip_gemmf.hip b/voxtral.c_amd/csrc/vox_hip_gemmf.hip
--- a/voxtral.c_amd/csrc/vox_hip_gemmf.hip
+++ b/voxtral.c_amd/csrc/vox_hip_gemmf.hip
@@ -42,6 +42,7 @@
     long long U;
     int MT;
     int colmajor;
+    GemmfRope r;
 };
 
 
@@ -214,6 +215,37 @@
     return r;
 }
 
+__device__ __forceinline__ float gf_rot0(float x0, float x1, float c, float s) { return __builtin_fmaf(x0, c, -(x1 * s)); }
+__device__ __forceinline__ float gf_rot1(float x0, float x1, float c, float s) { return __builtin_fmaf(x0, s, x1 * c); }
+
+template <class KT>
+__device__ __forceinline__ void gf_rope_kv(const GemmfRope& r, int m, int n, const float4& v) {
+    int slot = r.pos0 % r.cap + m;
+    if (slot >= r.cap) {
+        slot -= r.cap;
+        if (slot >= r.cap) slot %= r.cap;
+    }
+    if (n >= r.qd + r.kvd) {
+        KT* vr = reinterpret_cast<KT*>(r.Vc) + (size_t)slot * r.kvd + (n - r.qd - r.kvd);
+        kv_st2(vr, v.x, v.y);
+        kv_st2(vr + 2, v.z, v.w);
+        return;
+    }
+    const bool isq = n < r.qd;
+    const int cn = isq ? n : n - r.qd;
+    const int hm = r.hd - 1;
+    const float* rp = r.rope + (size_t)m * r.hd + ((r.hd & hm) ? cn % r.hd : cn & hm);
+    const float c0 = rp[0], s0 = rp[1], c1 = rp[2], s1 = rp[3];
+    if (isq) {
+        *reinterpret_cast<float4*>(r.q + (size_t)m * r.qd + cn) =
+            make_float4(gf_rot0(v.x, v.y, c0, s0), gf_rot1(v.x, v.y, c0, s0), gf_rot0(v.z, v.w, c1, s1), gf_rot1(v.z, v.w, c1, s1));
+        return;
+    }
+    KT* kr = reinterpret_cast<KT*>(r.Kc) + (size_t)slot * r.kvd + cn;
+    kv_st2(kr, gf_rot0(v.x, v.y, c0, s0), gf_rot1(v.x, v.y, c0, s0));
+    kv_st2(kr + 2, gf_rot0(v.z, v.w, c1, s1), gf_rot1(v.z, v.w, c1, s1));
+}
+
 template <int EPI, int WF = WF_BF16>
 __device__ __forceinline__ void gf_out(const GemmfArgs& a, int m, int gg, int lane, const f32x4& w0, const f32x4& w1) {
     const int nq = gg * 16 + (lane >> 4) * 4;
@@ -249,6 +281,13 @@
     if (a.bias) {
         const float4 bb = *reinterpret_cast<const float4*>(a.bias + n);
         v.x += bb.x; v.y += bb.y; v.z += bb.z; v.w += bb.w;
+    }
+    if (EPI == EPI_QKV_ROPE) {
+        asm volatile("" : "+v"(v.x), "+v"(v.y), "+v"(v.z), "+v"(v.w));
+        if (a.r.kvt == KV_FP8) gf_rope_kv<kv8_t>(a.r, m, n, v);
+        else if (a.r.kvt == KV_F16) gf_rope_kv<kvh_t>(a.r, m, n, v);
+        else gf_rope_kv<float>(a.r, m, n, v);
+        return;
     }
     float4* cp = reinterpret_cast<float4*>(a.C + (size_t)m * a.ldc + n);
     if (EPI == EPI_RESID) {
@@ -421,9 +460,14 @@
 
 bool gemmf_ok(int M, int N, int K) { return M > 0 && M <= 1024 && K % 64 == 0 && N % 128 == 0; }
 
+bool gemmf_rope_ok(int qd, int kvd, int hd, int kvt) {
+    return qd > 0 && kvd > 0 && hd > 0 && qd % 4 == 0 && kvd % 4 == 0 && hd % 4 == 0 && qd % hd == 0 && kvd % hd == 0 &&
+           kvt >= KV_F32 && kvt <= KV_FP8 && !(kvt == KV_F16 && hd == 64);
+}
+
 hipError_t launch_gemmf(int epi, int np, const uint16_t* xs, int K, int M, const void* Wf, int N, const float* bias,
                         float* C, int ldc, uint16_t* xo, float* ws, size_t ws_floats, int* flags, int epoch,
-                        hipStream_t st, const int* epoch_dev, int rb, const float* wscale) {
+                        hipStream_t st, const int* epoch_dev, int rb, const float* wscale, const GemmfRope* rope) {
     constexpr int NG = 2, WR = 2;
     if (g_gemmf_rb < 0) {
         const char* e = getenv("VOX_HIP_GEMMF_RB");
@@ -432,6 +476,10 @@
     }
     if (!gemmf_ok(M, N, K) || (np != 2 && np != 3) || !ws || !flags || (g_gemmf_rb && g_gemmf_rb != 4 && g_gemmf_rb != 8) ||
         (rb && rb != 4 && rb != 8))
+        return hipErrorInvalidValue;
+    if ((epi == EPI_QKV_ROPE) != (rope != nullptr)) return hipErrorInvalidValue;
+    if (rope && (!gemmf_rope_ok(rope->qd, rope->kvd, rope->hd, rope->kvt) || N != rope->qd + 2 * rope->kvd || !rope->rope ||
+                 !rope->q || !rope->Kc || !rope->Vc || rope->cap < 1 || rope->pos0 < 0))
         return hipErrorInvalidValue;
     const int NGx = NG;
     const int t8 = ((M + 127) / 128) * (N / (64 * NG));
@@ -439,6 +487,7 @@
     GemmfArgs a;
     a.xs = xs; a.K = K; a.M = M; a.W = static_cast<const uint8_t*>(Wf); a.N = N; a.wscale = wscale; a.bias = bias; a.C = C; a.ldc = ldc;
     a.xo = xo; a.ws = ws; a.flags = flags; a.epoch = epoch; a.epoch_dev = epoch_dev;
+    a.r = rope ? *rope : GemmfRope{};
     a.recomputes = flags + gemmf_grid();
     a.wait_ticks = g_gemmf_wait;
     a.S = K / 64;
@@ -474,6 +523,8 @@
 
     GF_EPI(EPI_STORE) GF_EPI(EPI_RESID) GF_EPI(EPI_GELU) GF_EPI(EPI_GELU_ERF) GF_EPI(EPI_SWIGLU)
 #undef GF_EPI
+    if (epi == EPI_QKV_ROPE && np == 3)
+        return wscale ? gemmf_launch<EPI_QKV_ROPE, 3, 4, NG, WR, WF_Q8>(a, G, st) : gemmf_launch<EPI_QKV_ROPE, 3, 4, NG, WR>(a, G, st);
     return hipErrorInvalidValue;
 }
 
diff --git a/voxtral.c_amd/csrc/vox_hip_internal.h b/voxtral.c_amd/csrc/vox_hip_internal.h
--- a/voxtral.c_amd/csrc/vox_hip_internal.h
+++ b/voxtral.c_amd/csrc/vox_hip_internal.h
@@ -7,7 +7,8 @@
 enum { EPI_STORE = 0, EPI_RESID = 1, EPI_GELU = 2, EPI_GELU_ERF = 3, EPI_SWIGLU = 4, EPI_QKV = 5, EPI_LOGITS = 6,
        EPI_LOGITS_ALT = 7,
        EPI_PARTIAL = 8,
-       EPI_QKV_BIAS = 9 };
+       EPI_QKV_BIAS = 9,
+       EPI_QKV_ROPE = 10 };
 constexpr int ALT_TEXT_MIN = 1000;
 constexpr int ALT_PART = 10;
 constexpr int ALT_REC = 8;
@@ -258,9 +259,19 @@
 size_t gemmf_flag_ints();
 int set_gemmf_wait(int ticks);
 size_t gemmf_ws_floats(int blocks);
+struct GemmfRope {
+    int qd, kvd, hd;
+    const float* rope;
+    int pos0;
+    float* q;
+    float *Kc, *Vc;
+    int cap, kvt;
+};
+bool gemmf_rope_ok(int qd, int kvd, int hd, int kvt);
 hipError_t launch_gemmf(int epi, int np, const uint16_t* xs, int K, int M, const void* Wf, int N, const float* bias,
                         float* C, int ldc, uint16_t* xo, float* ws, size_t ws_floats, int* flags, int epoch,
-                        hipStream_t st, const int* epoch_dev = nullptr, int rb = 0, const float* wscale = nullptr);
+                        hipStream_t st, const int* epoch_dev = nullptr, int rb = 0, const float* wscale = nullptr,
+                        const GemmfRope* rope = nullptr);
 hipError_t launch_gemmf_epoch_bump(int* epoch_dev, int by, hipStream_t st);
 int gemmf_wide_rb(int M, int N, int K);
 int gemm_planes_np();
diff --git a/voxtral.c_amd/csrc/vox_hip_kernels.hip b/voxtral.c_amd/csrc/vox_hip_kernels.hip
--- a/voxtral.c_amd/csrc/vox_hip_kernels.hip
+++ b/voxtral.c_amd/csrc/vox_hip_kernels.hip
@@ -10,69 +10,6 @@
 #include <stdlib.h>
 
 namespace vox {
-
-typedef _Float16 kvh_t;
-typedef _Float16 h16x4 __attribute__((ext_vector_type(4)));
-typedef _Float16 h16x2 __attribute__((ext_vector_type(2)));
-__device__ __forceinline__ float kv8_clamp(float v) { return v > 448.f ? 448.f : v < -448.f ? -448.f : v; }
-__device__ __forceinline__ unsigned kv8_fix_nan(float v, unsigned code) {
-    return v != v ? (0x7fu | ((__float_as_uint(v) >> 24) & 0x80u)) : code;
-}
-__device__ __forceinline__ unsigned kv8_enc2(float a, float b) {
-    const unsigned w = (unsigned)__builtin_amdgcn_cvt_pk_fp8_f32(kv8_clamp(a), kv8_clamp(b), 0, false);
-    return kv8_fix_nan(a, w & 0xffu) | (kv8_fix_nan(b, (w >> 8) & 0xffu) << 8);
-}
-struct kv8_t {
-    uint8_t b;
-    kv8_t() = default;
-    __device__ __forceinline__ explicit kv8_t(float v) : b((uint8_t)(kv8_enc2(v, v) & 0xffu)) {}
-    __device__ __forceinline__ explicit operator float() const {
-        return __builtin_amdgcn_cvt_pk_f32_fp8((int)b, false)[0];
-    }
-};
-static_assert(sizeof(kv8_t) == 1, "kv8_t: one byte per ring element");
-template <class T> __device__ __forceinline__ float4 kv_ld4(const T* p) {
-    if constexpr (sizeof(T) == 4) {
-        return *reinterpret_cast<const float4*>(p);
-    } else if constexpr (sizeof(T) == 2) {
-        const h16x4 h = *reinterpret_cast<const h16x4*>(p);
-        return make_float4((float)h[0], (float)h[1], (float)h[2], (float)h[3]);
-    } else {
-        const int w = *reinterpret_cast<const int*>(p);
-        const auto lo = __builtin_amdgcn_cvt_pk_f32_fp8(w, false), hi = __builtin_amdgcn_cvt_pk_f32_fp8(w, true);
-        return make_float4(lo[0], lo[1], hi[0], hi[1]);
-    }
-}
-template <class T> __device__ __forceinline__ float2 kv_ld2(const T* p) {
-    if constexpr (sizeof(T) == 4) {
-        return *reinterpret_cast<const float2*>(p);
-    } else if constexpr (sizeof(T) == 2) {
-        const h16x2 h = *reinterpret_cast<const h16x2*>(p);
-        return make_float2((float)h[0], (float)h[1]);
-    } else {
-        const auto v = __builtin_amdgcn_cvt_pk_f32_fp8((int)*reinterpret_cast<const uint16_t*>(p), false);
-        return make_float2(v[0], v[1]);
-    }
-}
-template <class T> __device__ __forceinline__ float kv_round(float v) { return (float)(T)v; }
-template <class T> __device__ __forceinline__ void kv_st2(T* p, float a, float b) {
-    if constexpr (sizeof(T) == 4) {
-        *reinterpret_cast<float2*>(p) = make_float2(a, b);
-    } else if constexpr (sizeof(T) == 2) {
-        *reinterpret_cast<h16x2*>(p) = h16x2{(T)a, (T)b};
-    } else {
-        *reinterpret_cast<uint16_t*>(p) = (uint16_t)kv8_enc2(a, b);
-    }
-}
-__device__ __forceinline__ float kv_f32(float v) {
-    asm volatile("" : "+v"(v));
-    return v;
-}
-__device__ __forceinline__ void kv_st2_rt(float* base, size_t e, float a, float b, int kvt) {
-    if (kvt == KV_FP8) kv_st2(reinterpret_cast<kv8_t*>(base) + e, a, b);
-    else if (kvt == KV_F16) kv_st2(reinterpret_cast<kvh_t*>(base) + e, a, b);
-    else kv_st2(base + e, a, b);
-}
 
 __global__ __launch_bounds__(256) void k_rmsnorm_rows(const float* __restrict__ x, int ldx,
                                                       float* __restrict__ y, int ldy,
diff --git a/voxtral.c_amd/vox_hip.py b/voxtral.c_amd/vox_hip.py
--- a/voxtral.c_amd/vox_hip.py
+++ b/voxtral.c_amd/vox_hip.py
@@ -106,6 +106,7 @@
     "vox_hip_skinny_wmx4",
     "vox_hip_set_gemm_planes", "vox_hip_gemm_planes", "vox_hip_set_gemmf_wait",
     "vox_hip_set_gemmf_q8", "vox_hip_gemmf_q8", "vox_hip_model_gemmf_q8_stats", "vox_hip_gemmf_q8_rows",
+    "vox_hip_set_gemmf_rope", "vox_hip_set_prefill_tail", "vox_hip_gemmf_rows", "vox_hip_gemmf_rope_rows",
     "vox_hip_stream_create", "vox_hip_stream_free",
     "vox_hip_stream_reset", "vox_hip_stream_reset_decoder", "vox_hip_stream_encode_mel",
     "vox_hip_stream_set_delay", "vox_hip_stream_delay", "vox_hip_stream_ada_scale",
@@ -172,6 +173,9 @@
         "vox_hip_set_gemmf_q8": (I, [I]), "vox_hip_gemmf_q8": (I, []),
         "vox_hip_model_gemmf_q8_stats": (I, [P, ctypes.POINTER(ctypes.c_longlong)]),
         "vox_hip_gemmf_q8_rows": (I, [I, I, I, fp, P, fp, fp, I]),
+        "vox_hip_set_gemmf_rope": (I, [I]), "vox_hip_set_prefill_tail": (I, [I]),
+        "vox_hip_gemmf_rows": (I, [I, I, I, fp, P, fp, I, fp, ctypes.POINTER(ctypes.c_longlong)]),
+        "vox_hip_gemmf_rope_rows": (I, [I, I, I, I, I, fp, P, fp, fp, I, I, I, I, fp, P, P]),
         "vox_hip_stream_create": (P, [P]), "vox_hip_stream_free": (None, [P]),
         "vox_hip_stream_reset": (I, [P]), "vox_hip_stream_reset_decoder": (I, [P]),
         "vox_hip_stream_set_delay": (I, [P, I]), "vox_hip_stream_delay": (I, [P]),
@@ -327,6 +331,55 @@
     return y
 
 
+def set_gemmf_rope(on: bool) -> int:
+    return lib().vox_hip_set_gemmf_rope(int(bool(on)))
+
+
+def set_prefill_tail(on: bool) -> int:
+    return lib().vox_hip_set_prefill_tail(int(bool(on)))
+
+
+GEMMF_STORE, GEMMF_RESID, GEMMF_SWIGLU = 0, 1, 4
+
+
+def gemmf_rows(x, W_bf16, bias=None, epi: int = GEMMF_STORE, y0=None):
+    init()
+    W = np.ascontiguousarray(W_bf16, np.uint16)
+    xv = np.ascontiguousarray(x, np.float32)
+    N, K = W.shape
+    assert xv.ndim == 2 and xv.shape[1] == K
+    M = xv.shape[0]
+    b = None if bias is None else np.ascontiguousarray(bias, np.float32)
+    y = np.zeros((M, N // 2 if epi == GEMMF_SWIGLU else N), np.float32)
+    if epi == GEMMF_RESID:
+        y[:] = y0
+    rec = ctypes.c_longlong(0)
+    if lib().vox_hip_gemmf_rows(M, N, K, fptr(xv), W.ctypes.data, fptr(b) if b is not None else None, int(epi), fptr(y),
+                                ctypes.byref(rec)) != 0:
+        _err("gemmf_rows")
+    return y, rec.value
+
+
+def gemmf_rope_rows(x, W_bf16, bias, rope, qd: int, kvd: int, hd: int, pos0: int, cap: int, kvt: int, fused: bool):
+    init()
+    W = np.ascontiguousarray(W_bf16, np.uint16)
+    xv = np.ascontiguousarray(x, np.float32)
+    N, K = W.shape
+    M = xv.shape[0]
+    assert N == qd + 2 * kvd and xv.shape[1] == K
+    b = None if bias is None else np.ascontiguousarray(bias, np.float32)
+    rp = np.ascontiguousarray(rope, np.float32)
+    assert rp.shape == (M, hd)
+    q = np.empty((M, qd), np.float32)
+    k = np.empty((cap, kvd), KV_NP_DTYPE[kvt])
+    v = np.empty((cap, kvd), KV_NP_DTYPE[kvt])
+    if lib().vox_hip_gemmf_rope_rows(M, qd, kvd, hd, K, fptr(xv), W.ctypes.data, fptr(b) if b is not None else None,
+                                     fptr(rp), int(pos0), int(cap), int(kvt), int(bool(fused)), fptr(q),
+                                     k.ctypes.data, v.ctypes.data) != 0:
+        _err("gemmf_rope_rows")
+    return q, k, v
+
+
 def set_adapter_rows0(rows: int):
     if lib().vox_hip_set_adapter_rows0(int(rows)) != 0:
         _err("set_adapter_rows0")
```

Result: no change. 748.0 (-0.3%).
